# RWAlgorithms/ConjugateGradientOptim.jl

Hardware: AMD Instinct MI355X
Metric: CG iterations/sec at n=1e8 (outer iterations of minimizeobjective, PR-CG) (higher is better)
Workload: dtype f64

## Files before the change

conjugategradientoptim.jl_amd/_lib.py:

```python
from __future__ import annotations

import ctypes as C
import os
import subprocess

_PKG = os.path.dirname(os.path.abspath(__file__))
LIB_PATH = os.environ.get("CGO_LIB_PATH") or os.path.join(_PKG, "lib", "libcgo_hip.so")
CSRC = os.path.join(_PKG, "csrc")

dp = C.POINTER(C.c_double)
i64p = C.POINTER(C.c_int64)


class BetaConfig(C.Structure):
    _fields_ = [("kind", C.c_int32), ("lbfgs_m", C.c_int32), ("mu", C.c_double)]


class CGConfigC(C.Structure):
    _fields_ = [("eps", C.c_double), ("beta", BetaConfig), ("max_iters", C.c_int64),
                ("verbose", C.c_int32), ("trace_enabled", C.c_int32)]


class LSConfigC(C.Structure):
    _fields_ = [("kind", C.c_int32), ("cond_kind", C.c_int32), ("c1", C.c_double),
# ... 123 lines not shown
    "cgo_ctx_set_default_policy": (C.c_int, [_vp, C.POINTER(SolverPolicyC)]),
    "cgo_solver_get_policy": (C.c_int, [_vp, C.POINTER(SolverPolicyC)]),
    "cgo_solver_create_ex": (C.c_int, [_vp, _vp, C.POINTER(CGConfigC), C.POINTER(LSConfigC), C.POINTER(SolverPolicyC), _pp]),
    "cgo_solver_create_sys_ex": (C.c_int, [_vp, _vp, C.POINTER(CGConfigC), C.POINTER(LSSConfigC), C.POINTER(SolverPolicyC), _pp]),
    "cgo_ctx_destroy": (C.c_int, [_vp]),
    "cgo_comm_unique_id": (C.c_int, [_vp]),
    "cgo_ctx_set_comm_rccl": (C.c_int, [_vp, C.c_int32, C.c_int32, _vp]),
    "cgo_ctx_set_comm_callback": (C.c_int, [_vp, C.c_int32, C.c_int32, ALLGATHER_FN, _vp]),
    "cgo_ctx_set_comm_shm": (C.c_int, [_vp, C.c_int32, C.c_int32, C.c_char_p, C.c_int32]),
    "cgo_shm_unlink": (C.c_int, [C.c_char_p]),
    "cgo_ctx_comm_info": (C.c_int, [_vp, C.POINTER(C.c_int32), C.POINTER(C.c_int32), C.POINTER(C.c_int32), C.POINTER(C.c_int32)]),
    "cgo_ctx_exchange_stats": (C.c_int, [_vp, i64p, dp, dp, C.c_int32]),
    "cgo_ctx_comm_connect_devices": (C.c_int, [_vp, C.POINTER(C.c_int32)]),
    "cgo_rccl_available": (C.c_int, []),
    "cgo_objective_create": (C.c_int, [_vp, C.c_int32, C.c_int64, C.c_int64, C.c_int64, _pp]),
    "cgo_objective_create_from_source": (C.c_int, [_vp, C.c_char_p, C.c_int32, C.c_int64, C.c_int64, C.c_int64, _pp]),
    "cgo_objective_create_callback": (C.c_int, [_vp, FDF_FN, _vp, C.c_int64, C.c_int64, C.c_int64, _pp]),
    "cgo_objective_destroy": (C.c_int, [_vp]),
    "cgo_objective_create_from_source_ex": (C.c_int, [_vp, C.c_char_p, C.c_int32, C.c_int64, C.c_int64, C.c_int64, _pp]),
    "cgo_objective_num_params": (C.c_int, [_vp, C.POINTER(C.c_int32)]),
    "cgo_objective_set_param_host": (C.c_int, [_vp, C.c_int32, dp]),
    "cgo_objective_set_param_device": (C.c_int, [_vp, C.c_int32, _vp]),
    "cgo_objective_fill_param": (C.c_int, [_vp, C.c_int32, C.c_int32, C.c_uint64, C.c_double, C.c_double]),
    "cgo_objective_set_scalar": (C.c_int, [_vp, C.c_int32, C.c_double]),
    "cgo_objective_set_cost_class": (C.c_int, [_vp, C.c_int32]),
    "cgo_objective_eval_host": (C.c_int, [_vp, dp, dp, dp]),
    "cgo_solver_create": (C.c_int, [_vp, _vp, C.POINTER(CGConfigC), C.POINTER(LSConfigC), _pp]),
    "cgo_solver_destroy": (C.c_int, [_vp]),
    "cgo_solver_set_x0_host": (C.c_int, [_vp, dp]),
    "cgo_solver_set_x0_fill": (C.c_int, [_vp, C.c_int32, C.c_uint64, C.c_double, C.c_double]),
    "cgo_solver_set_x0_device": (C.c_int, [_vp, _vp]),
    "cgo_solver_results_device": (C.c_int, [_vp, _vp, _vp]),
    "cgo_solver_start": (C.c_int, [_vp]),
    "cgo_solver_iterate": (C.c_int, [_vp, C.c_int64, C.POINTER(C.c_int32)]),
    "cgo_solver_results": (C.c_int, [_vp, C.POINTER(ResultsC)]),
    "cgo_solver_trial_log": (C.c_int, [_vp, C.c_int64, dp, dp, dp, i64p]),
    "cgo_solver_profile_enable": (C.c_int, [_vp, C.c_int32]),
    "cgo_solver_profile_reset": (C.c_int, [_vp]),
    "cgo_solver_profile_get": (C.c_int, [_vp, C.c_int32, i64p, dp, dp]),
    "cgo_kernel_kind_name": (C.c_char_p, [C.c_int32]),
    "cgo_solver_kernel_family": (C.c_char_p, [_vp]),
    "cgo_solver_controller_launches": (C.c_int64, [_vp]),
    "cgo_solver_resident_stats": (C.c_int, [_vp, i64p, i64p, i64p]),
    "cgo_solver_lbfgs_stats": (C.c_int, [_vp, i64p, i64p, i64p]),
    "cgo_num_kernel_kinds": (C.c_int, []),
    "cgo_solver_set_lazy_direction": (C.c_int, [_vp, C.c_int32]),
    "cgo_solver_probe_set_beta_prev": (C.c_int, [_vp, C.c_double]),
    "cgo_solver_set_replay_depth": (C.c_int, [_vp, C.c_int32]),
    "cgo_solver_set_lean_sums": (C.c_int, [_vp, C.c_int32]),
    "cgo_solver_set_path_prediction": (C.c_int, [_vp, C.c_int32]),
    "cgo_solver_path_stats": (C.c_int, [_vp, i64p, i64p, i64p, i64p]),
    "cgo_solver_probe_set_path": (C.c_int, [_vp, C.c_int32]),
    "cgo_solver_debug_set_path_skew": (C.c_int, [_vp, C.c_double]),
    "cgo_solver_probe_set_replay": (C.c_int, [_vp, C.c_int32, dp, dp]),
    "cgo_solver_probe_set_deep_trial": (C.c_int, [_vp, C.c_int32]),
    "cgo_solver_replay_stats": (C.c_int, [_vp, i64p, i64p, i64p, i64p, i64p, i64p, C.POINTER(C.c_int32)]),
    "cgo_solver_kernel_symbol": (C.c_int, [_vp, C.c_int32, C.c_char_p, C.c_int32]),
    "cgo_evalwolfeconditions": (C.c_int, [C.POINTER(LSConfigC), C.c_double, C.c_double, C.c_double, C.c_double,
                                          C.c_double, C.c_double, C.POINTER(C.c_int32), C.POINTER(C.c_int32)]),
    "cgo_evalbacktrackcondition": (C.c_int, [C.POINTER(LSConfigC), C.c_double, C.c_double, C.c_double, C.c_double,
                                             C.POINTER(C.c_int32)]),
    "cgo_check_lss_config": (C.c_int, [C.POINTER(LSSConfigC)]),
    "cgo_lss_default_max_iters": (C.c_int64, [C.c_double]),
    "cgo_solver_create_sys": (C.c_int, [_vp, _vp, C.POINTER(CGConfigC), C.POINTER(LSSConfigC), _pp]),
    "cgo_solvesystem": (C.c_int, [_vp, _vp, dp, C.POINTER(CGConfigC), C.POINTER(LSSConfigC), C.POINTER(ResultsC)]),
    "cgo_minimize": (C.c_int, [_vp, _vp, dp, C.POINTER(CGConfigC), C.POINTER(LSConfigC), C.POINTER(ResultsC)]),
    "cgo_minimize_rerun": (C.c_int, [_vp, _vp, dp, C.POINTER(CGConfigC), C.POINTER(LSConfigC),
                                     C.POINTER(CGConfigC), C.POINTER(LSConfigC), C.c_int32,
                                     C.POINTER(ResultsC), C.POINTER(C.c_int32)]),
    "cgo_minimize_batch": (C.c_int, [_vp, C.c_int32, C.c_int64, C.c_int64, dp, dp, C.POINTER(CGConfigC), C.POINTER(LSConfigC),
                                     C.c_int64, C.POINTER(BatchResultsC)]),
    "cgo_batch_max_n": (C.c_int64, [_vp, C.c_int32]),
    "cgo_minimize_batch_obj": (C.c_int, [_vp, _vp, C.c_int64, dp, C.POINTER(dp), C.c_int32, C.POINTER(CGConfigC), C.POINTER(LSConfigC),
                                         C.c_int64, C.POINTER(BatchResultsC)]),
    "cgo_batch_max_n_obj": (C.c_int64, [_vp]),
    "cgo_batch_open": (C.c_int, [_vp, _vp, C.c_int64, C.POINTER(dp), C.c_int32, C.POINTER(_vp)]),
    "cgo_batch_solve": (C.c_int, [_vp, dp, dp, C.POINTER(C.c_uint8), C.POINTER(CGConfigC), C.POINTER(LSConfigC), C.c_int64,
                                  C.POINTER(BatchResultsC)]),
    "cgo_batch_close": (C.c_int, [_vp]),
    "cgo_batch_policy_init": (None, [C.POINTER(BatchPolicyC)]),
    "cgo_minimize_batch_ex": (C.c_int, [_vp, C.c_int32, C.c_int64, C.c_int64, dp, dp, C.POINTER(CGConfigC), C.POINTER(LSConfigC),
                                        C.c_int64, C.POINTER(BatchPolicyC), C.POINTER(BatchResultsC), C.POINTER(C.c_int32)]),
    "cgo_minimize_batch_obj_ex": (C.c_int, [_vp, _vp, C.c_int64, dp, C.POINTER(dp), C.c_int32, C.POINTER(CGConfigC), C.POINTER(LSConfigC),
                                            C.c_int64, C.POINTER(BatchPolicyC), C.POINTER(BatchResultsC), C.POINTER(C.c_int32)]),
    "cgo_batch_open_ex": (C.c_int, [_vp, _vp, C.c_int64, C.POINTER(dp), C.c_int32, C.POINTER(BatchPolicyC), C.POINTER(_vp)]),
    "cgo_batch_rows": (C.c_int, [_vp, C.POINTER(C.c_int32)]),
    "cgo_batch_max_n_ex": (C.c_int64, [_vp, C.c_int32, C.POINTER(BatchPolicyC)]),
    "cgo_batch_max_n_obj_ex": (C.c_int64, [_vp, C.POINTER(BatchPolicyC)]),
    "cgo_batch_rows_shape": (None, [C.POINTER(C.c_int32), C.POINTER(C.c_int32)]),
    "cgo_minimize_batch_lbfgs": (C.c_int, [_vp, C.c_int32, C.c_int64, C.c_int64, dp, dp, C.POINTER(CGConfigC), C.POINTER(LSConfigC),
                                           C.c_int64, C.POINTER(BatchResultsC)]),
    "cgo_batch_lbfgs_max_m": (C.c_int32, []),
    "cgo_batch_lbfgs_max_n": (C.c_int64, [_vp, C.c_int32]),
    "cgo_batch_lbfgs_shape": (None, [C.POINTER(C.c_int32), C.POINTER(C.c_int32)]),
    "cgo_minimize_batch_lbfgs_obj": (C.c_int, [_vp, _vp, C.c_int64, dp, C.POINTER(dp), C.c_int32, dp, C.POINTER(CGConfigC), C.POINTER(LSConfigC),
                                               C.c_int64, C.POINTER(BatchResultsC)]),
    "cgo_batch_lbfgs_max_n_obj": (C.c_int64, [_vp]),
    "cgo_batch_lbfgs_shape_obj": (None, [C.c_int32, C.POINTER(C.c_int32), C.POINTER(C.c_int32)]),
    "cgo_minimize_batch_lbfgs_ex": (C.c_int, [_vp, C.c_int32, C.c_int64, C.c_int64, dp, dp, C.POINTER(CGConfigC), C.POINTER(LSConfigC),
                                              C.c_int64, C.POINTER(BatchPolicyC), C.POINTER(BatchResultsC), C.POINTER(C.c_int32)]),
    "cgo_minimize_batch_lbfgs_obj_ex": (C.c_int, [_vp, _vp, C.c_int64, dp, C.POINTER(dp), C.c_int32, dp, C.POINTER(CGConfigC),
                                                  C.POINTER(LSConfigC), C.c_int64, C.POINTER(BatchPolicyC), C.POINTER(BatchResultsC),
                                                  C.POINTER(C.c_int32)]),
    "cgo_batch_lbfgs_max_n_ex": (C.c_int64, [_vp, C.c_int32, C.c_int32, C.POINTER(BatchPolicyC)]),
    "cgo_batch_lbfgs_max_n_obj_ex": (C.c_int64, [_vp, C.c_int32, C.POINTER(BatchPolicyC)]),
    "cgo_batch_lbfgs_lds_rows": (C.c_int32, [C.c_int32, C.c_int32]),
# ... 66 lines not shown
```

conjugategradientoptim.jl_amd/api.py:

```python
from __future__ import annotations

import ctypes as C
import math
import re
from dataclasses import dataclass, field
from typing import List, Optional, Sequence, Union

import numpy as np

from . import _lib
from ._lib import BetaConfig, CGConfigC, LSConfigC, LSSConfigC, ResultsC, check, dp, i64p



class TraceTrait:
    pass


class EnableTrace(TraceTrait):
    def __repr__(self):
        return "EnableTrace()"


class DisableTrace(TraceTrait):
# ... 606 lines not shown
        fin = C.c_int32(0)
        check(_lib.lib().cgo_solver_iterate(self._h, iters, C.byref(fin)))
        return bool(fin.value)

    def enable_trial_log(self):
        cnt = C.c_int64()
        check(_lib.lib().cgo_solver_trial_log(self._h, -1, None, None, None, C.byref(cnt)))

    def trial_log(self):
        cnt = C.c_int64()
        check(_lib.lib().cgo_solver_trial_log(self._h, 0, None, None, None, C.byref(cnt)))
        k = cnt.value
        a, p, d = np.zeros(max(k, 1)), np.zeros(max(k, 1)), np.zeros(max(k, 1))
        check(_lib.lib().cgo_solver_trial_log(self._h, k, a.ctypes.data_as(dp), p.ctypes.data_as(dp),
                                              d.ctypes.data_as(dp), C.byref(cnt)))
        return a[:k], p[:k], d[:k]

    def kernel_family(self) -> str:
        return _lib.lib().cgo_solver_kernel_family(self._h).decode()

    def kernel_symbol(self, kind_name: str) -> str:
        L = _lib.lib()
        buf = C.create_string_buffer(200)
        for k in range(L.cgo_num_kernel_kinds()):
            if L.cgo_kernel_kind_name(k).decode() == kind_name:
                check(L.cgo_solver_kernel_symbol(self._h, k, buf, 200))
                return buf.value.decode()
        return ""

    def set_lazy_direction(self, on: bool = True):
        check(_lib.lib().cgo_solver_set_lazy_direction(self._h, int(bool(on))))

    def set_replay_depth(self, d: int):
        check(_lib.lib().cgo_solver_set_replay_depth(self._h, int(d)))

    def replay_stats(self):
        v = [C.c_int64(0) for _ in range(6)]
        mx = C.c_int32(0)
        check(_lib.lib().cgo_solver_replay_stats(self._h, *[C.byref(q) for q in v], C.byref(mx)))
        return dict(zip(("n", "s", "t", "m", "t_deep", "m_deep"), (q.value for q in v)), max_list=mx.value)

    def set_lean_sums(self, on: bool):
        check(_lib.lib().cgo_solver_set_lean_sums(self._h, int(bool(on))))

    def set_path_prediction(self, on: bool):
        check(_lib.lib().cgo_solver_set_path_prediction(self._h, int(bool(on))))

    def path_stats(self):
        by = (C.c_int64 * 8)()
        p, t, m = C.c_int64(0), C.c_int64(0), C.c_int64(0)
        check(_lib.lib().cgo_solver_path_stats(self._h, by, C.byref(p), C.byref(t), C.byref(m)))
        return dict(by_nact={j: int(by[j]) for j in (1, 2, 3, 4, 5, 7)}, predicted=p.value, tree=t.value, misses=m.value)

    def debug_set_path_skew(self, factor: float):
        check(_lib.lib().cgo_solver_debug_set_path_skew(self._h, float(factor)))

    def probe_launch(self, kind_name: str, variant: int, a_acc: float, beta: float, a: Sequence[float], x, u=None, aux=None,
                     beta_prev: Optional[float] = None, replay: Optional[Sequence] = None, path_nact: Optional[int] = None,
                     deep_trial: bool = False):
        L = _lib.lib()
        kk = [L.cgo_kernel_kind_name(k).decode() for k in range(L.cgo_num_kernel_kinds())].index(kind_name)
        if beta_prev is not None:
            check(L.cgo_solver_probe_set_beta_prev(self._h, float(beta_prev)))
        if replay is not None:
            ra = np.ascontiguousarray([p[0] for p in replay], dtype=np.float64)
            rb = np.ascontiguousarray([p[1] for p in replay], dtype=np.float64)
            check(L.cgo_solver_probe_set_replay(self._h, len(replay), ra.ctypes.data_as(dp), rb.ctypes.data_as(dp)))
        if path_nact is not None:
            check(L.cgo_solver_probe_set_path(self._h, int(path_nact)))
        if deep_trial:
            check(L.cgo_solver_probe_set_deep_trial(self._h, 1))
        n = self.obj.n_local
        vec = lambda v: None if v is None else np.ascontiguousarray(v, dtype=np.float64)
        x, u, aux = vec(x), vec(u), vec(aux)
        for v in (x, u, aux):
            if v is not None and v.size != n:
                raise ValueError(f"probe vectors hold n_local = {n} elements")
        av = np.ascontiguousarray(a, dtype=np.float64) if len(a) else np.zeros(1)
        sums, ln = np.full(64, np.nan), C.c_int32(0)
        xo, uo, go = np.empty(n), np.empty(n), np.empty(n)
        sym = C.create_string_buffer(200)
        ptr = lambda v: None if v is None else v.ctypes.data_as(dp)
        check(L.cgo_solver_probe_launch(self._h, kk, int(variant), float(a_acc), float(beta), ptr(av), len(a), ptr(x), ptr(u),
                                        ptr(aux), ptr(sums), 64, C.byref(ln), ptr(xo), ptr(uo), ptr(go), sym, 200))
        return dict(sums=sums[:ln.value].copy(), x=xo, u=uo, g=go, symbol=sym.value.decode())

    LBFGS_PASSES = ("push", "push_gram", "direction_gram", "direction_trial", "push_lite", "loop")

    def probe_lbfgs(self, pass_name: str, x=None, u=None, g=None, gt=None, S=None, Y=None, **kw):
        n = self.obj.n_local
        P = self._cfg_c.beta.lbfgs_m + 1
        vec = lambda v: None if v is None else np.ascontiguousarray(v, dtype=np.float64)
        x, u, g, gt = vec(x), vec(u), vec(g), vec(gt)
        for v in (x, u, g, gt):
            if v is not None and v.size != n:
                raise ValueError(f"probe vectors hold n_local = {n} elements")
        S = None if S is None else np.ascontiguousarray(S, dtype=np.float64).reshape(P, n)
        Y = None if Y is None else np.ascontiguousarray(Y, dtype=np.float64).reshape(P, n)
        p = _lib.LbfgsProbeC()
        p.pass_ = self.LBFGS_PASSES.index(pass_name)
        dots = None
        for key, val in kw.items():
            if key in ("list", "spec_list"):
                getattr(p, key)[:len(val)] = [int(v) for v in val]
                setattr(p, "count" if key == "list" else "spec_count", len(val))
            elif key in ("cy", "cs", "alpha"):
                getattr(p, key)[:len(val)] = [float(v) for v in val]
            elif key == "stats":
                p.M, p.S = float(val[0]), float(val[1])
            elif key == "dots":
                dots = np.ascontiguousarray(val, dtype=np.float64).reshape(-1, 10)
                p.dots, p.dot_count = dots.ctypes.data_as(dp), dots.shape[0]
            else:
                if not hasattr(p, key):
                    raise TypeError(f"probe_lbfgs: no field {key}")
                setattr(p, key, val)
        outs = {k: np.full(n, np.nan) for k in ("x", "xo", "u", "g", "gt")}
        So, Yo = np.full((P, n), np.nan), np.full((P, n), np.nan)
        ptr = lambda v: None if v is None else v.ctypes.data_as(dp)
        check(_lib.lib().cgo_solver_probe_lbfgs(self._h, C.byref(p), ptr(x), ptr(u), ptr(g), ptr(gt), ptr(S), ptr(Y),
                                                *[ptr(outs[k]) for k in ("x", "xo", "u", "g", "gt")], ptr(So), ptr(Yo)))
        sym = p.symbol.decode()
        return dict(sums=np.array(p.sums[:p.sums_len]), S=So, Y=Yo, alpha=np.array(p.alpha[:]), symbols=sym.split(" + ") if sym else [],
                    new_in_list=p.new_in_list, spec_ok=bool(p.spec_ok),
                    gram=np.array(p.gram[:5 + 5 * p.spec_count]) if p.spec_ok else None, **outs)

    def probe_resident(self, script, x, u):
        n = self.obj.n_local
        x, u = np.ascontiguousarray(x, dtype=np.float64), np.ascontiguousarray(u, dtype=np.float64)
        if x.size != n or u.size != n:
            raise ValueError(f"probe vectors hold n_local = {n} elements")
        p = _lib.ResidentProbeC()
        if len(script) > 32:
            raise ValueError("probe_resident: at most 32 passes")
        p.npass = len(script)
        for q, item in enumerate(script):
            c = p.pass_[q]
            if item[0] == "trial":
# ... 1081 lines not shown
```

conjugategradientoptim.jl_amd/csrc/cgo_backend_cg.hip:

```cpp
#include "cgo_backend_internal.hpp"

#include "cgo_kernels.hip.hpp"
#include "cgo_kernels_cg.hip.hpp"
#include "cgo_kernels_cg_path.hip.hpp"
#include "cgo_kernels_chain.hip.hpp"
#include "cgo_kernels_lse.hip.hpp"
#include "cgo_kernels_resident.hip.hpp"

namespace cgo {

using namespace dev;

double bytes_r(int obj_kind, int mode, int64_t n, int n_params) {
    const int p = std::max(obj_kind == CGO_OBJ_QUAD_DIAG ? 1 : 0, n_params);
    return 8.0 * (double)n * (double)r_vectors(mode, p);
}

template <int N> using Pts = std::integral_constant<int, N>;
template <int MAXPTS, class F>
static inline void with_points(int npts, F f) {
    static_assert(MAXPTS == 1 || MAXPTS == 3 || MAXPTS == 5 || MAXPTS == 7, "a launch evaluates 1, 3, 5 or 7 trial points");
    if constexpr (MAXPTS >= 3) { if (npts == 3) return f(Pts<3>{}); }
    if constexpr (MAXPTS >= 5) { if (npts == 5) return f(Pts<5>{}); }
    if constexpr (MAXPTS >= 7) { if (npts != 1) return f(Pts<7>{}); }
    return f(Pts<1>{});
}

template <class Obj, bool BIG>
static int launch_cg(int mode, int npts, const RParams &P, int grid, hipStream_t st) {
#define ROW(MODE, MAXPTS) if (mode == (MODE) && P.tail.ctl) { with_points<MAXPTS>(npts, [&](auto n) { k_cg_armed<Obj, decltype(n)::value><<<grid, BLOCK, 0, st>>>(P); }); return 0; }
    CGO_CG_ARMED_ROWS(ROW)
#undef ROW
    switch (mode) {
#define ROW(MODE, MAXPTS) case (MODE): with_points<MAXPTS>(npts, [&](auto n) { k_cg<Obj, (MODE), decltype(n)::value, BIG><<<grid, BLOCK, 0, st>>>(P); }); return 0;
    CGO_CG_ROWS(ROW)
#undef ROW
    default: break;
    }
    if constexpr (BIG) {
        switch (mode) {
#define ROW(MODE, MAXPTS) case (MODE): with_points<MAXPTS>(npts, [&](auto n) { k_cg<Obj, (MODE), decltype(n)::value, true><<<grid, BLOCK, 0, st>>>(P); }); return 0;
        CGO_CG_LAG_ROWS(ROW)
        CGO_CG_REPLAY_ROWS(ROW)
        CGO_CG_LEAN_ROWS(ROW)
#undef ROW
        default: break;
        }
    }
    return -1;
}

template <class Obj>
static int launch_cg_path(int mode, int nact, const RParams &P, const RDeep &Q, int grid, hipStream_t st) {
#define ROW(MODE, NACT) if (mode == (MODE) && nact == (NACT)) { k_cg_path<Obj, (MODE), (NACT), true><<<grid, BLOCK, 0, st>>>(P, Q); return 0; }
    CGO_CG_PATH_ROWS(ROW)
#undef ROW
    return -1;
}
template <class Obj>
static int launch_cg_deep_t(int npts, const RParams &P, const RDeep &Q, int grid, hipStream_t st) {
#define ROW(NPTS) if (npts == (NPTS)) { k_cg_trial_deep<Obj, (NPTS), true><<<grid, BLOCK, 0, st>>>(P, Q); return 0; }
    CGO_CG_DEEP_T_ROWS(ROW)
#undef ROW
    return -1;
}
static inline bool path_row(int mode, int nact) {
#define ROW(MODE, NACT) if (mode == (MODE) && nact == (NACT)) return true;
    CGO_CG_PATH_ROWS(ROW)
#undef ROW
    return false;
}
static inline bool path_objective(int kind) {
#define ROW(KIND, T) if (kind == KIND) return true;
    CGO_OBJ_CURV_ROWS(ROW)
#undef ROW
    return false;
}
bool HipBackend::deep_trial(int mode) const {
    return mode == (R_REPLAY | R_TRIAL) && !path_nact_ && path_objective(obj_->kind) && (rep_n_ > RMAX || deep_t_);
}
bool HipBackend::path_rows() const {
    if (!path_on_ || !path_objective(obj_->kind) || replay_depth_ < 2 || !lazy_eligible()) return false;
    const int mode_n = r_mode_of(KK_ACCEPT_TRIAL_NOSTORE), mode_s = R_REPLAY | R_ADT;
    return path_row(mode_n | lean_for(mode_n), MAXP) && path_row(mode_s | lean_for(mode_s), MAXP);
}

static inline bool lean_row(int mode) {
#define ROW(MODE, MAXPTS) if (mode == (MODE)) return true;
    CGO_CG_LEAN_ROWS(ROW)
#undef ROW
    return false;
}
int HipBackend::lean_for(int mode) const { return (lean_bits_ && lean_row(mode | lean_bits_)) ? lean_bits_ : 0; }

void unpack_r(const double *s, int k, Scal *out, bool dir, int npts) {
    if (npts == 0) npts = npts_for(k);
    for (int j = 0; j < k; ++j) {
        const double *q = s + RS_PER_POINT * j;
        out[j].f = q[RS_F]; out[j].gtu = q[RS_GTU]; out[j].gtgt = q[RS_GTGT]; out[j].gtg = q[RS_GTG];
        out[j].yy = q[RS_YY]; out[j].uy = q[RS_UY]; out[j].ygt = q[RS_YGT];
    }
    if (dir) { out[0].gu = s[RS_PER_POINT * npts]; out[0].uu = s[RS_PER_POINT * npts + 1]; }
}

static inline int chain_npts(int mode, int npts) { return ((mode & R_TRIAL) && npts >= 3) ? 3 : 1; }

RPlan HipBackend::r_plan(int mode, int npts) const {
    const double bytes = bytes_r(obj_->kind, mode, obj_->n_local, obj_->nparams());
    const bool big = r_big_only(mode) || bytes > big_bytes(r_read_only(mode));
    return {big, big ? GRID_BIG : grid_cg(obj_->n_local, chain() ? 1 : npts), chain() ? chain_npts(mode, npts) : npts, bytes};
}
bool HipBackend::adt_is_big() const { return bytes_r(obj_->kind, R_ADT, obj_->n_local, obj_->nparams()) > big_bytes(false); }

int HipBackend::launch_r(int kk, int mode, double a_acc, double beta, const double *a, int k, bool fetch,
                         double *sums) {
    if (int rc = pipe_drain()) return rc;
    pipe_streak_ = 0;
    if (u_lag_ && !(mode & R_ULAG)) {
        if (r_reads_u(mode)) { if (int rc = materialize_u()) return rc; }
        else if (mode & (R_INIT | R_RESET)) u_lag_ = false;
    }
    if (rep_n_ > 0 && !(mode & R_REPLAY)) { if (int rc = materialize_lag()) return rc; }
    if (rep_n_ > RMAX && (mode & R_REPLAY) && r_base(mode) != R_REPLAY && !path_nact_ && !deep_trial(mode)) { if (int rc = materialize_lag()) return rc; }
    RPlan plan;
    const int npts = path_nact_ ? MAXP : npts_for(k);
    if (int rc = launch_r_kernel(kk, mode, a_acc, beta, a, k, npts, nullptr, &plan)) return rc;
    const int grid = plan.grid;
    total_launches_++;
    const bool has_sums = r_has_sums(mode);
    const bool fused = has_sums && tail_fused(grid);
    if (has_sums && chain()) {
        const bool three = plan.npts == 3;
        const int W = three ? NRC3 : NRC, edge = three ? RC3_EDGE : RC_EDGE, nsums = three ? NR : NR1;
        if (!fused) { if (int rc = finalize_rows(ctx_, grid, W, true)) return rc; }
        const int Wd = ctx_->world(), me = ctx_->rank();
        std::vector<double> raw((size_t)W * Wd);
        double all[NRC3];
        if (int rc = fetch_sums(ctx_, all, MERGE_SUM, W, raw.data())) return rc;
        if (sums) std::memcpy(sums, all, sizeof(double) * nsums);
        if (me > 0) {
            const double *e = raw.data() + (size_t)(me - 1) * W + edge + 4;
            halo_xl_[0] = e[0]; halo_xl_[1] = e[1]; halo_ul_[0] = e[2]; halo_ul_[1] = e[3];
        }
        if (me < Wd - 1) {
            const double *e = raw.data() + (size_t)(me + 1) * W + edge;
            halo_xr_[0] = e[0]; halo_xr_[1] = e[1]; halo_ur_[0] = e[2]; halo_ur_[1] = e[3];
        }
        if (probe_) { std::memcpy(probe_row_, all, sizeof(double) * W); probe_len_ = W; }
    } else if (has_sums) {
        if (!fused) { if (int rc = finalize_rows(ctx_, grid, rows_for(npts), true)) return rc; }
        if (fetch) {
            if (int rc = fetch_sums(ctx_, sums, MERGE_SUM, rows_for(npts))) return rc;
        }
        if (probe_ && fetch) { std::memcpy(probe_row_, sums, sizeof(double) * rows_for(npts)); probe_len_ = rows_for(npts); }
    }
    if (prof_on_) prof_commit(kk, plan.bytes);
    return CGO_OK;
}

bool HipBackend::lazy_eligible() const {
    if (!lazy_on_ || !rmode_ || chain() || sys_on_ || probe_ || pingpong_ == 1) return false;
    bool aot = false;
#define ROW(KIND, T) aot = aot || obj_->kind == KIND;
    CGO_OBJ_ROWS(ROW)
#undef ROW
    if (!aot) return false;
    if (const char *e = getenv("CGO_PINGPONG")) { if (e[0] == '1') return false; }
    if (ctl_depth() > 0) return false;
    return adt_is_big() && r_plan(R_TRIAL, 1).big;
}

int HipBackend::materialize_u() {
    if (!u_lag_) return CGO_OK;
    const int64_t asked = total_launches_;
    const int nact = path_nact_;
    path_nact_ = 0;
    const int rc = launch_rk(KK_MATERIALIZE_U, 0.0, 0.0, nullptr, 0, false, nullptr);
    path_nact_ = nact;
    total_launches_ = asked;
    if (rc) return rc;
    u_lag_ = false;
    return CGO_OK;
}

int HipBackend::materialize_lag() {
    if (int rc = materialize_u()) return rc;
    const int64_t asked = total_launches_;
    const int nact = path_nact_;
    path_nact_ = 0;
    int rc = CGO_OK;
    while (rep_n_ > 0 && rc == CGO_OK) {
        const int all = rep_n_, take = std::min(all, (int)RMAX);
        rep_n_ = take;
        rc = launch_rk(KK_MATERIALIZE_XU, 0.0, 0.0, nullptr, 0, false, nullptr);
        rep_n_ = all;
        if (rc) break;
        rstats_.m++;
        if (all > RMAX) rstats_.m_deep++;
        for (int j = take; j < all; ++j) { rep_a_[j - take] = rep_a_[j]; rep_b_[j - take] = rep_b_[j]; }
        rep_n_ = all - take;
    }
    path_nact_ = nact;
    total_launches_ = asked;
    return rc;
}

int HipBackend::set_replay_depth_now(int d) {
    if (d < 1 || d > RCAP + 1) { set_error("replay depth: 1 … 16"); return CGO_EINVAL; }
    if (d != replay_depth_) { if (int rc = materialize_lag()) return rc; }
    replay_depth_ = d;
    return CGO_OK;
}

void HipBackend::set_probe_replay(int nrep, const double *a, const double *beta) {
    probe_rep_n_ = std::max(0, std::min(nrep, (int)RCAP));
    for (int j = 0; j < probe_rep_n_; ++j) { probe_rep_a_[j] = a[j]; probe_rep_b_[j] = beta[j]; }
}

int HipBackend::accept_dir_trial_r(double a_acc, double beta, const double *a, int k, double *s) {
    if (!lazy_eligible()) return launch_rk(KK_ACCEPT_DIR_TRIAL, a_acc, beta, a, k, true, s);
    if (replay_depth_ >= 2) {
        if (int rc = materialize_u()) return rc;
        if (rep_n_ < replay_depth_ - 1 && rep_n_ < (path_nact_ ? RCAP : RMAX)) {
            const int mode_n = r_mode_of(KK_ACCEPT_TRIAL_NOSTORE);
            if (int rc = launch_r(KK_ACCEPT_TRIAL_NOSTORE, mode_n | lean_for(mode_n), a_acc, beta, a, k, true, s)) return rc;
            if (path_nact_) { path_last_n_ = path_nact_; path_count_[path_nact_]++; }
            rep_a_[rep_n_] = a_acc; rep_b_[rep_n_] = beta; rep_n_++;
            rstats_.n++;
            return CGO_OK;
        }
        const int mode_s = R_REPLAY | R_ADT;
        if (int rc = launch_r(KK_ACCEPT_DIR_TRIAL, mode_s | lean_for(mode_s), a_acc, beta, a, k, true, s)) return rc;
        if (path_nact_) { path_last_s_ = path_nact_; path_count_[path_nact_]++; }
        rep_n_ = 0;
        rstats_.s++;
        return CGO_OK;
    }
    if (!u_lag_) {
        if (int rc = launch_rk(KK_ACCEPT_TRIAL_LAZY, a_acc, beta, a, k, true, s)) return rc;
        u_lag_ = true; beta_lag_ = beta;
        return CGO_OK;
    }
    if (int rc = launch_r(KK_ACCEPT_DIR_TRIAL, R_ULAG | R_ADT, a_acc, beta, a, k, true, s)) return rc;
    u_lag_ = false;
    return CGO_OK;
}
int HipBackend::trial_r(const double *a, int k, double *s) {
    if (rep_n_ > 0 && lazy_eligible()) {
        rstats_.t++;
        if (rep_n_ > RMAX) rstats_.t_deep++;
        return launch_r(KK_TRIAL, R_REPLAY | R_TRIAL, 0, 0, a, k, true, s);
    }
    if (u_lag_ && lazy_eligible()) return launch_r(KK_TRIAL, R_ULAG | R_TRIAL, 0, 0, a, k, true, s);
    return launch_rk(KK_TRIAL, 0, 0, a, k, true, s);
}

bool HipBackend::pipe_fused(int grid) const {
    return tail_fused(grid) && obj_->kind != CGO_OBJ_USER && !chain() && ctl_fused_;
}
bool HipBackend::tail_fused(int grid) const {
    static const int cap = [] { const char *e = getenv("CGO_FUSED_TAIL_MAX_GRID"); int v = e ? atoi(e) : 0; return v > 0 ? v : 1024; }();
    return ctx_->fused_tail && grid <= cap && grid <= TAIL_GROUP * TAIL_GROUP;
}
Tail HipBackend::make_tail(bool on) {
    Tail t{};
    if (!on) return t;
    ctx_->seq++;
    t.partials2 = ctx_->partials2_f; t.tickets = ctx_->tickets; t.out = ctx_->out_dev;
    t.strict = ctx_->tail_strict ? 1 : 0;
    ctx_->pub_target(&t.host_out, &t.host_seq);
    ctx_->pub_checked = (t.host_out != nullptr) && !ctx_->tail_strict;
    t.seq = ctx_->seq;
    return t;
}

int HipBackend::launch_r_kernel(int kk, int mode, double a_acc, double beta, const double *a, int k, int npts,
                                const CtlArgs *ctl, RPlan *plan_out) {
    HIPCHK(hipSetDevice(ctx_->device));
    if (obj_->unset_slot() >= 0) return param_unset_error(obj_->unset_slot());
    const int64_t n = obj_->n_local;
    if (mode & (R_GRAD | R_GRADT)) { if (int rc = ensure_ga()) return rc; }
    const bool has_sums = r_has_sums(mode);
    const RPlan plan = *plan_out = r_plan(mode, npts);
    const bool big = plan.big; const int grid = plan.grid;
    const bool deep_t = deep_trial(mode);
    last_mode_ = mode; last_npts_ = plan.npts; last_big_ = big; last_nact_ = deep_t ? -1 : path_nact_;
    if (path_nact_ && (chain() || !big || ctl || !path_row(mode, path_nact_) || !path_objective(obj_->kind))) { set_error("internal: not a path row"); return CGO_EINVAL; }
    if (chain()) {
        if (int rc = prof_begin(kk)) return rc;
        if (int rc = launch_chain_kernel(mode, a_acc, beta, a, k, plan.npts, big, grid, make_tail(has_sums && !ctl && tail_fused(grid)))) return rc;
        return prof_end();
    }
    RParams P;
    P.x = xc_; P.u = uc_; P.gout = ga_.p; obj_->param_args(P); P.n = n;
    P.xo = xc_; P.uo = uc_;
    P.a_acc = a_acc; P.beta = beta; P.s0 = obj_->s0; P.partials = ctx_->partials;
    P.beta_prev = beta_lag_;
    const int nrep = (mode & R_REPLAY) ? rep_n_ : 0;
    if (nrep > RCAP || (nrep > RMAX && !path_nact_ && !deep_t)) { set_error("internal: more replayed steps than the launch takes"); return CGO_ESTATE; }
    P.nrep = std::min(nrep, (int)RMAX);
    for (int j = 0; j < RMAX; ++j) { P.ra[j] = j < P.nrep ? rep_a_[j] : 0.0; P.rb[j] = j < P.nrep ? rep_b_[j] : 0.0; }
    RDeep Q;
    Q.nrep2 = nrep - P.nrep;
    for (int j = 0; j < RDEEP; ++j) { Q.ra2[j] = j < Q.nrep2 ? rep_a_[RMAX + j] : 0.0; Q.rb2[j] = j < Q.nrep2 ? rep_b_[RMAX + j] : 0.0; }
    rstats_.max_list = std::max(rstats_.max_list, nrep);
    P.ctl = ctl;
    P.x2 = xn_;
    for (int j = 0; j < MAXP; ++j) P.a[j] = (a && j < k) ? a[j] : ((a && k > 0) ? a[k - 1] : 0.0);
    P.tail = make_tail(has_sums && !ctl && tail_fused(grid));
    if (ctl && pipe_fused(grid)) {
        P.tail.partials2 = ctx_->partials2_f; P.tail.tickets = ctx_->tickets; P.tail.out = ctx_->out_dev;
        P.tail.strict = ctx_->tail_strict ? 1 : 0;
        P.tail.ctl = ctl_dev_; P.tail.ctl_rec = ctl_rec_; P.tail.ctl_seq = ctl_seq_;
        if (!ctx_->single()) {
            P.tail.xw = ctx_->world(); P.tail.xme = ctx_->rank(); P.tail.xseq0 = epoch_ << 40;
            for (int r = 0; r < P.tail.xw && r < 8; ++r) P.tail.xmail[r] = ctx_->comm->dev_mailbox(r);
        }
    }
    if (P.tail.tickets) P.partials = ctx_->partials_f;
    const bool wr_x = r_writes_x(mode), wr_u = r_writes_u(mode);
    const bool pp = big && !ctl && (wr_x || wr_u) && !(mode & R_PROJ) && pingpong_ready();
    if (pp && wr_x) P.xo = xalt_;
    if (pp && wr_u) P.uo = ualt_;
    if (mode == R_PROJ && !xn_) { set_error("internal: no second iterate buffer"); return CGO_ESTATE; }
    hipStream_t st = ctx_->stream;
    if (int rc = prof_begin(kk)) return rc;
    int r = -2;
    if (path_nact_) {
        switch (obj_->kind) {
#define ROW(KIND, T) case KIND: r = launch_cg_path<T>(mode, path_nact_, P, Q, grid, st); break;
        CGO_OBJ_CURV_ROWS(ROW)
#undef ROW
        default: break;
        }
    } else if (deep_t) {
        if (!big) { set_error("internal: not a deep trial row"); return CGO_EINVAL; }
        switch (obj_->kind) {
#define ROW(KIND, T) case KIND: r = launch_cg_deep_t<T>(plan.npts, P, Q, grid, st); break;
        CGO_OBJ_CURV_ROWS(ROW)
#undef ROW
        default: break;
        }
    } else switch (obj_->kind) {
#define ROW(KIND, T) case KIND: r = big ? launch_cg<T, true>(mode, npts, P, grid, st) : launch_cg<T, false>(mode, npts, P, grid, st); break;
    CGO_OBJ_ROWS(ROW)
#undef ROW
    case CGO_OBJ_USER:
        if (!obj_->rtc) { set_error("user objective has no compiled module"); return CGO_EINVAL; }
        if (r_big_only(mode)) break;
        if (int rc = launch_module(obj_->rtc->cg(mode, npts, big), &P, grid, st)) return rc;
        r = 0;
        break;
    default: break;
    }
    if (r) { set_error("internal: CG kernel mode not instantiated"); return CGO_EINVAL; }
    HIPCHK(hipGetLastError());
    if (pp && wr_x) std::swap(xc_, xalt_);
    if (pp && wr_u) std::swap(uc_, ualt_);
    return prof_end();
}

template <bool BIG>
static int launch_chain(int mode, int npts, const ChainParams &P, int grid, hipStream_t st) {
    switch (mode) {
#define ROW(MODE, MAXPTS) case (MODE): with_points<MAXPTS>(npts, [&](auto n) { k_chain<(MODE), decltype(n)::value, BIG><<<grid, BLOCK, 0, st>>>(P); }); return 0;
    CGO_CHAIN_ROWS(ROW)
#undef ROW
    default: return -1;
    }
}

int HipBackend::launch_chain_kernel(int mode, double a_acc, double beta, const double *a, int k, int npts, bool big, int grid, const Tail &tail) {
    ChainParams P;
    P.tail = tail;
    for (int j = 0; j < 3; ++j) P.a[j] = (a && j < k) ? a[j] : ((a && k > 0) ? a[k - 1] : 0.0);
    P.x = xc_; P.u = uc_; P.xo = xc_; P.uo = uc_; P.gout = ga_.p;
    P.odd = (int)(obj_->n_local & 1);
    P.n = obj_->n_local + P.odd; P.a_acc = a_acc; P.beta = beta; P.partials = tail.tickets ? ctx_->partials_f : ctx_->partials;
    for (int j = 0; j < 2; ++j) { P.hxl[j] = halo_xl_[j]; P.hul[j] = halo_ul_[j]; P.hxr[j] = halo_xr_[j]; P.hur[j] = halo_ur_[j]; }
    P.has_left = obj_->offset > 0 ? 1 : 0;
    P.has_right = obj_->offset + obj_->n_local < obj_->n_global ? 1 : 0;
    const bool wr_x = r_writes_x(mode), wr_u = r_writes_u(mode);
    if (wr_x) P.xo = xalt_;
    if (wr_u) P.uo = ualt_;
    const int r = big ? launch_chain<true>(mode, npts, P, grid, ctx_->stream) : launch_chain<false>(mode, npts, P, grid, ctx_->stream);
    if (r) { set_error("internal: chain kernel mode not instantiated"); return CGO_EINVAL; }
    HIPCHK(hipGetLastError());
    if (wr_x) std::swap(xc_, xalt_);
    if (wr_u) std::swap(uc_, ualt_);
    return CGO_OK;
}

std::string HipBackend::r_symbol(int mode, int npts, bool big, int nact) const {
    char buf[160];
    if (chain()) snprintf(buf, sizeof buf, "k_chain<%d, %d, %s>", mode, npts, big ? "true" : "false");
    else if (nact < 0) snprintf(buf, sizeof buf, "k_cg_trial_deep<%s, %d, true>", obj_tname(), npts);
    else if (nact) snprintf(buf, sizeof buf, "k_cg_path<%s, %d, %d, true>", obj_tname(), mode, nact);
    else snprintf(buf, sizeof buf, "k_cg<%s, %d, %d, %s>", obj_tname(), mode, npts, big ? "true" : "false");
    return buf;
}

std::string HipBackend::kernel_symbol(int kk) const {
    if (!rmode_) {
        if (obj_->two_phase() || kk == KK_LBFGS_PUSH || kk == KK_LBFGS_LOOP || kk == KK_LBFGS_FINAL) return lbfgs_symbol(kk);
        const int mode = fused_mode(kk);
        return mode < 0 ? "" : fused_symbol(obj_tname(), mode, is_big(obj_->kind, mode, obj_->n_local, obj_->nparams(), pol_.hbm_stream_bytes));
    }
    const RKind *rk = r_kind(kk);
    if (!rk) return "";
    int mode = rk->mode;
    const bool lazy = lazy_eligible();
    switch (kk) {
    case KK_ACCEPT_DIR_TRIAL: if (lazy) mode |= replay_depth_ >= 2 ? R_REPLAY : R_ULAG; break;
    case KK_ACCEPT_TRIAL_LAZY: case KK_MATERIALIZE_U: if (!lazy || replay_depth_ >= 2) return ""; break;
    case KK_ACCEPT_TRIAL_NOSTORE: case KK_MATERIALIZE_XU: if (!lazy || replay_depth_ < 2) return ""; break;
    default: break;
    }
    if (kk == KK_TRIAL && lazy && rep_n_ > RMAX) mode |= R_REPLAY;
    const RPlan plan = r_plan(mode, rk->pts == PTS_ONE ? 1 : npts_for(rk->pts == PTS_MAX ? max_points() : std::min(max_points(), 3)));
    if ((mode & R_REPLAY) && (mode & R_ACCEPT)) mode |= lean_for(mode);
    if ((mode & R_REPLAY) && (mode & R_ACCEPT) && path_rows()) {
        const int last = kk == KK_ACCEPT_TRIAL_NOSTORE ? path_last_n_ : path_last_s_;
        return r_symbol(mode, plan.npts, plan.big, last ? last : MAXP);
    }
    if (kk == KK_TRIAL && deep_trial(mode)) return r_symbol(mode, plan.npts, plan.big, -1);
    return r_symbol(mode, plan.npts, plan.big);
}


__global__ void k_ctl_init(CtlDev *d, const CtlConfig cfg, const CtlState st, unsigned long long round) {
    d->cfg = cfg;
    d->st = st;
    d->round = round;
    d->args = ctl_args_of(st);
}



template <int N, int THREADS>
__global__ __launch_bounds__(THREADS) void k_finalize_ctl(const double *partials, int rows, double *out, CtlDev *d,
                                                          CtlRecord *rec_ring, unsigned long long *seq_ring) {
    constexpr int G = BLOCK / N;
    constexpr int WD = sizeof(CtlDev) / 8, WR = sizeof(CtlRecord) / 8;
    __shared__ double sm[G][N];
    __shared__ double fin[CTL_NSUMS];
    __shared__ CtlDev sd;
    __shared__ CtlRecord sr;
    const int tid = threadIdx.x;
    if (tid < WD) ((unsigned long long *)&sd)[tid] = ((const unsigned long long *)d)[tid];
    if (tid < CTL_NSUMS) fin[tid] = 0.0;
    __syncthreads();
    const bool go = sd.st.go != 0;
    const unsigned long long round = sd.round, seq = round + 1;
    CtlRecord *rec_host = rec_ring + (round % PIPE_RING);
    unsigned long long *seq_host = seq_ring + (round % PIPE_RING);
    if (go) {
        if (tid < G * N) {
            double t = 0.0;
            const long long total = (long long)rows * N;
            for (long long i = tid; i < total; i += G * N) t += partials[i];
            sm[tid / N][tid % N] = t;
        }
        __syncthreads();
        if (tid < N) {
            double v = 0.0;
#pragma unroll
            for (int g = 0; g < G; ++g) v += sm[g][tid];
            out[tid] = v;
            fin[tid] = v;
        }
        __syncthreads();
    }
    if (tid == 0) {
        if (go) {
            ctl_step(sd.cfg, sd.st, fin, sr);
            sd.args = ctl_args_of(sd.st);
// ... 242 lines not shown
        if (b == &x2_ || b == &u2_) { if (pingpong_ != 1) continue; }
        if (int rc = b->alloc(np)) return rc;
        HIPCHK(hipMemsetAsync(b->p, 0, na * sizeof(double), ctx_->stream));
        HIPCHK(hipMemsetD32Async((hipDeviceptr_t)(b->p + na), (int)PROBE_NAN32, (np - na) * 2, ctx_->stream));
    }
    for (int j = 0; j < obj_->nparams(); ++j) {
        if (!obj_->p_set[j]) continue;
        DevBuf p;
        if (int rc = p.alloc(np)) return rc;
        HIPCHK(hipMemcpyAsync(p.p, obj_->p[j].p, n * sizeof(double), hipMemcpyDeviceToDevice, ctx_->stream));
        HIPCHK(hipMemsetD32Async((hipDeviceptr_t)(p.p + n), (int)PROBE_NAN32, (np - n) * 2, ctx_->stream));
        HIPCHK(hipStreamSynchronize(ctx_->stream));
        std::swap(p.p, obj_->p[j].p); std::swap(p.n, obj_->p[j].n);
    }
    HIPCHK(hipStreamSynchronize(ctx_->stream));
    xc_ = x_.p; uc_ = u_.p; xalt_ = x2_.p; ualt_ = u2_.p;
    g_ = ga_.p; gt_ = gb_.p; xn_ = gb_.p;
    lse_have_ = false;
    probe_ = true;
    return CGO_OK;
}

int HipBackend::probe_slack_intact() {
    const size_t n = (size_t)obj_->n_local, na = n + (chain() ? (n & 1) : 0);
    struct { const DevBuf *b; const char *name; size_t used; int slot; } v[] = {
        {&x_, "x", na, -1}, {&u_, "u", na, -1}, {&x2_, "x (ping-pong)", na, -1}, {&u2_, "u (ping-pong)", na, -1},
        {&ga_, "gradient A", na, -1}, {&gb_, "gradient B / x2", na, -1}, {&obj_->p[0], "parameter vector", n, 0},
        {&obj_->p[1], "parameter vector 1", n, 1}, {&obj_->p[2], "parameter vector 2", n, 2}, {&obj_->p[3], "parameter vector 3", n, 3}};
    std::vector<unsigned> h;
    for (const auto &e : v) {
        if (!e.b->p || (e.slot >= 0 && !(e.slot < obj_->nparams() && obj_->p_set[e.slot]))) continue;
        const size_t words = (e.b->n - e.used) * 2;
        h.assign(words, 0u);
        HIPCHK(hipMemcpyAsync(h.data(), e.b->p + e.used, words * 4, hipMemcpyDeviceToHost, ctx_->stream));
        HIPCHK(hipStreamSynchronize(ctx_->stream));
        for (size_t w = 0; w < words; ++w)
            if (h[w] != PROBE_NAN32) {
                set_error(std::string("probe: the launch wrote past the ") + std::to_string(e.used) + " elements of " + e.name +
                          " (element " + std::to_string(e.used + w / 2) + ")");
                return CGO_ESTATE;
            }
    }
    return CGO_OK;
}

int HipBackend::probe_launch(int kk, int variant, double a_acc, double beta, const double *a, int k, const double *x,
                             const double *u, const double *aux, double *sums, int sums_cap, int *sums_len, double *x_out,
                             double *u_out, double *g_out, std::string &symbol) {
    *sums_len = 0;
    const int want_nact = probe_nact_;
    probe_nact_ = 0;
    const bool want_deep = probe_deep_t_;
    probe_deep_t_ = false;
    const bool lse = obj_->two_phase();
    if (k < 0 || k > MAXP || (k > 0 && !a)) { set_error("probe: 0 ≤ k ≤ 7 trial steps"); return CGO_EINVAL; }
    if (!rmode_ && !lse) return probe_launch_stored(kk, variant, a_acc, beta, a, k, x, u, aux, sums, sums_cap, sums_len, x_out, u_out, g_out, symbol);
    int mode = -1;
    if (lse) {
        if (kk == KK_LSE_STATS && (variant == 0 || variant == LM_NOU || variant == (LM_ACCEPT | LM_DIR))) mode = variant;
        if (kk == KK_LSE_GRAD && variant >= 0 && variant <= 2) mode = variant;
        if (kk == KK_LSE_STATS && mode != LM_NOU && k < 1) mode = -1;
        if (kk == KK_LSE_GRAD && mode != 2 && k < 1) mode = -1;
    } else {
        static constexpr RKind norm_passes{KK_SCALED_NORM, R_GRAD, PTS_ONE, {R_GRADT, 0}};
        const RKind *rk = kk == KK_SCALED_NORM ? &norm_passes : r_kind(kk);
        if (rk && (variant & R_LEAN)) {
            const int full = kk == KK_ACCEPT_DIR_TRIAL ? (R_REPLAY | R_ADT) : (kk == KK_ACCEPT_TRIAL_NOSTORE ? rk->mode : -1);
            if (lean_row(variant) && (variant & ~R_LEAN) == full) mode = variant;
        } else if (rk) {
            const int m = variant ? variant : rk->mode;
            if (r_kind_allows(*rk, m) || (kk == KK_INIT && chain() && m == R_EDGES)) mode = m;
        }
        if (mode > 0 && (mode & (R_TRIAL | R_GRADT | R_PROJ)) && k < 1) mode = -1;
        if (mode > 0 && chain() && k > 3) mode = -1;
        if (mode > 0 && r_big_only(mode) && (chain() || obj_->kind == CGO_OBJ_USER)) mode = -1;
    }
    if (mode < 0) { set_error("probe: kernel kind / variant / trial steps not a launch this solver's engine issues"); return CGO_EINVAL; }
    if (int rc = probe_prepare()) return rc;
    HIPCHK(hipSetDevice(ctx_->device));
    hipStream_t st = ctx_->stream;
    const size_t n = (size_t)obj_->n_local, nb = n * sizeof(double);
    double *ub = lse ? u_.p : uc_;
    double *gb = lse ? gt_ : ga_.p;
    double *auxb = lse ? g_ : xn_;
    auto put = [&](double *dst, const double *src) -> int {
        if (src) HIPCHK(hipMemcpyAsync(dst, src, nb, hipMemcpyHostToDevice, st));
        else HIPCHK(hipMemsetD32Async((hipDeviceptr_t)dst, (int)PROBE_NAN32, n * 2, st));
        return CGO_OK;
    };
    if (int rc = put(xc_, x)) return rc;
    if (int rc = put(ub, u)) return rc;
    if (int rc = put(auxb, aux)) return rc;
    if (gb != auxb) { if (int rc = put(gb, nullptr)) return rc; }
    if (!lse && pingpong_ == 1) {
        if (int rc = put(xalt_, nullptr)) return rc;
        if (int rc = put(ualt_, nullptr)) return rc;
    }
    HIPCHK(hipStreamSynchronize(st));
    probe_len_ = 0;
    last_mode_ = -1;
    beta_lag_ = probe_beta_prev_;
    rep_n_ = (!lse && (mode & R_REPLAY)) ? probe_rep_n_ : 0;
    for (int j = 0; j < rep_n_; ++j) { rep_a_[j] = probe_rep_a_[j]; rep_b_[j] = probe_rep_b_[j]; }
    int rc = CGO_OK;
    char buf[160];
    if (lse) {
        Scal o;
        if (kk == KK_LSE_STATS) {
            lse_have_ = false;
            rc = lse_stats(mode, a_acc, beta, k ? a[0] : 0.0, o, mode == (LM_ACCEPT | LM_DIR));
            snprintf(buf, sizeof buf, "k_lse_stats<%d, %s, %s>", last_mode_, last_big_ ? "true" : "false", last_npts_ ? "true" : "false");
        } else {
            const bool nb0 = need_beta_;
            need_beta_ = mode == 1;
            rc = lse_grad(mode == 2, k ? a[0] : 0.0, o);
            need_beta_ = nb0;
            snprintf(buf, sizeof buf, "k_lse_grad<%s, %s, %s>", last_mode_ == 1 ? "true" : "false", last_mode_ == 2 ? "true" : "false",
                     last_big_ ? "true" : "false");
        }
        if (rc) return rc;
        symbol = buf;
    } else {
        double s[64];
        if (want_deep && (mode != (R_REPLAY | R_TRIAL) || want_nact || !path_objective(obj_->kind))) { rep_n_ = 0; set_error("probe: not a deep trial launch of this solver"); return CGO_EINVAL; }
        if (rep_n_ > RMAX && !want_nact && !(mode == (R_REPLAY | R_TRIAL) && path_objective(obj_->kind))) {
            rep_n_ = 0; set_error("probe: more than 7 replayed steps: path rows and the deep trial launch only"); return CGO_EINVAL;
        }
        deep_t_ = want_deep;
        if (want_nact) {
            if (!path_row(mode, want_nact) || !path_objective(obj_->kind) || k > want_nact) { rep_n_ = 0; set_error("probe: not a path row of this solver, or more steps than it evaluates"); return CGO_EINVAL; }
            path_nact_ = want_nact;
        }
        rc = launch_r(kk, mode, a_acc, beta, a, k, true, s);
        path_nact_ = 0;
        deep_t_ = false;
        rep_n_ = 0;
        if (rc) return rc;
        symbol = r_symbol(last_mode_, last_npts_, last_big_, last_nact_);
    }
    HIPCHK(hipStreamSynchronize(st));
    if (x_out) HIPCHK(hipMemcpyAsync(x_out, xc_, nb, hipMemcpyDeviceToHost, st));
    if (u_out) HIPCHK(hipMemcpyAsync(u_out, lse ? u_.p : uc_, nb, hipMemcpyDeviceToHost, st));
    if (g_out) HIPCHK(hipMemcpyAsync(g_out, mode == R_PROJ && !lse ? xn_ : gb, nb, hipMemcpyDeviceToHost, st));
    HIPCHK(hipStreamSynchronize(st));
    if (int rc2 = probe_slack_intact()) return rc2;
    *sums_len = probe_len_;
    if (probe_len_ > sums_cap) { set_error("probe: sums_cap smaller than the launch's row"); return CGO_EINVAL; }
    if (probe_len_) std::memcpy(sums, probe_row_, sizeof(double) * probe_len_);
    return CGO_OK;
}

void HipBackend::probe_append(const double *row, int len) {
    if (probe_len_ + len > (int)(sizeof probe_row_ / sizeof probe_row_[0])) return;
    std::memcpy(probe_row_ + probe_len_, row, sizeof(double) * len);
    probe_len_ += len;
}

int HipBackend::probe_launch_stored(int kk, int variant, double a_acc, double beta, const double *a, int k, const double *x,
                                    const double *u, const double *aux, double *sums, int sums_cap, int *sums_len, double *x_out,
                                    double *u_out, double *g_out, std::string &symbol) {
    if (ctx_->world() != 1) { set_error("probe: a single-rank solver"); return CGO_EINVAL; }
    const bool host = obj_->host_closure();
    int mode = -1;
    if (const MKind *mk = m_kind(kk)) {
        const int m = variant ? variant : (host ? mk->host : fused_mode(kk));
        if (host ? m == mk->host : (m == mk->mode || (mk->alt && m == mk->alt))) mode = m;
    } else if (kk == KK_SCALED_NORM) {
        mode = (variant == 0 || variant == 1 || variant == 3 || variant == 4) ? variant : -1;
    }
    const bool trial_step = kk == KK_TRIAL || kk == KK_ACCEPT_DIR_TRIAL;
    if (mode >= 0 && trial_step && k != 1) mode = -1;
    if (mode < 0) { set_error("probe: kernel kind / variant / trial steps not a launch this solver's engine issues"); return CGO_EINVAL; }
    if (int rc = probe_prepare()) return rc;
    HIPCHK(hipSetDevice(ctx_->device));
    hipStream_t st = ctx_->stream;
    const size_t n = (size_t)obj_->n_local, nb = n * sizeof(double);
    auto put = [&](double *dst, const double *src) -> int {
        if (src) HIPCHK(hipMemcpyAsync(dst, src, nb, hipMemcpyHostToDevice, st));
        else HIPCHK(hipMemsetD32Async((hipDeviceptr_t)dst, (int)PROBE_NAN32, n * 2, st));
        return CGO_OK;
    };
    const bool norm = kk == KK_SCALED_NORM;
    const bool gt_in_x = norm && (mode == 1 || mode == 4);
    const bool swaps = kk == KK_ACCEPT_DIR_TRIAL || kk == KK_ACCEPT_DIR || kk == KK_ACCEPT_ONLY;
    if (int rc = put(xc_, gt_in_x ? nullptr : x)) return rc;
    if (int rc = put(u_.p, u)) return rc;
    if (int rc = put(swaps ? gt_ : g_, aux)) return rc;
    if (int rc = put(swaps ? g_ : gt_, gt_in_x ? x : nullptr)) return rc;
    HIPCHK(hipStreamSynchronize(st));
    probe_len_ = 0;
    probe_syms_.clear();
// ... 459 lines not shown
```

conjugategradientoptim.jl_amd/csrc/cgo_capi.hip:

```cpp
#include <sys/mman.h>

#include <cmath>
#include <cstdio>
#include <cstdlib>
#include <cstring>
#include <new>
#include <vector>

#include "cgo_capi_internal.hpp"
#include "cgo_build_id.inc"

using namespace cgo;

extern "C" {

int cgo_version(void) { return CGO_VERSION; }
const char *cgo_build_id(void) { return CGO_BUILD_ID; }
const char *cgo_last_error(void) { return get_error(); }
const char *cgo_status_name(int32_t s) { return status_name(s); }
const char *cgo_kernel_kind_name(int32_t k) {
    if (k == 100) return "dir";
    if (k == 101) return "beta_partials";
    return kernel_kind_name(k);
}
// ... 424 lines not shown
    int rc = s->be->alloc();
    if (rc) { delete s; obj_unref(obj); return rc; }
    const bool cheap = obj->o.kind == CGO_OBJ_QUAD_DIAG || obj->o.kind == CGO_OBJ_BOOTH ||
                       (obj->o.kind == CGO_OBJ_USER && obj->o.user_cheap);
    s->be->set_multi_min_n(0);
    s->be->set_multi5_min_n(cheap ? 0 : INT64_MAX);
    s->be->set_multi7_min_n(cheap ? 0 : INT64_MAX);
    s->be->set_three_point_band(0, 0);
    const char *mm = getenv("CGO_MULTI_MIN_N"), *m5 = getenv("CGO_MULTI5_MIN_N"), *m7 = getenv("CGO_MULTI7_MIN_N");
    if (chain) m5 = m7 = nullptr;
    if (mm || m5 || m7) s->be->set_three_point_band(0, 0);
    if (mm) s->be->set_multi_min_n(atoll(mm));
    if (m5) s->be->set_multi5_min_n(atoll(m5));
    if (m7) s->be->set_multi7_min_n(atoll(m7));
    if (pol.points) {
        const int pts = chain ? std::min(pol.points, 3) : pol.points;
        s->be->set_three_point_band(0, 0);
        s->be->set_multi_min_n(pts >= 3 ? 0 : INT64_MAX);
        s->be->set_multi5_min_n(pts >= 5 ? 0 : INT64_MAX);
        s->be->set_multi7_min_n(pts >= 7 ? 0 : INT64_MAX);
    }
    s->be->set_ctl_depth((ls && !cheap && !chain && s->be->policy_points() <= 3 && (ctx->c.world() == 1 || ctx->c.dev_exchange()) && obj->o.n_local <= 100000) ? 4 : 0);
    if (pol.controller_depth >= 0) s->be->set_ctl_depth(chain ? 0 : pol.controller_depth);
    s->be->set_ctl_graph(pol.controller_graph != 0);
    {
        bool lazy = obj->o.kind == CGO_OBJ_QUAD_DIAG;
        const int forced = env_tri("CGO_LAZY_DIR");
        if (forced >= 0) lazy = forced != 0;
        s->be->set_lazy_direction(lazy);
    }
    {
        int depth = 1;
        if (obj->o.kind == CGO_OBJ_QUAD_DIAG && 8.0 * (double)obj->o.n_local * 5.0 > 1.4e9) depth = kReplayDepth;
        if (const char *e = getenv("CGO_REPLAY_DEPTH")) { const int v = atoi(e); if (v >= 1 && v <= 16) depth = v; }
        s->be->set_replay_depth(depth);
    }
    {
        bool lean = kLeanSums && obj->o.kind == CGO_OBJ_QUAD_DIAG && 8.0 * (double)obj->o.n_local * 5.0 > 1.4e9;
        const int forced = env_tri("CGO_LEAN_SUMS");
        if (forced >= 0) lean = forced != 0;
        s->be->set_beta_unread(beta_unread_sums(cfg->beta.kind));
        s->be->set_lean_sums(lean);
    }
    {
        bool predict = kPathPredict && kLeanSums && obj->o.kind == CGO_OBJ_QUAD_DIAG && 8.0 * (double)obj->o.n_local * 5.0 > 1.4e9;
        const int forced = env_tri("CGO_PATH_PREDICT");
        if (forced >= 0) predict = forced != 0;
        s->be->set_path_prediction(predict && path_applies(obj, cfg, ls));
    }
    if (int prc = s->be->place()) { delete s; obj_unref(obj); return prc; }
    if (pol.resident >= 0) s->be->set_resident(pol.resident != 0);
    if (int prc = s->be->prepare_controller()) { delete s; obj_unref(obj); return prc; }
    s->sv = ls ? new Solver(s->be, *cfg, *ls) : new Solver(s->be, *cfg, *lss);
    *out = s;
    return CGO_OK;
}

int cgo_solver_create(cgo_ctx *ctx, cgo_objective *obj, const cgo_cg_config *cfg,
                      const cgo_ls_config *ls, cgo_solver **out) {
    API_GUARD_BEGIN
    REQUIRE(ctx && obj && cfg && ls && out, "null argument");
    return make_solver(ctx, obj, cfg, ls, nullptr, nullptr, out);
    API_GUARD_END
}

int cgo_solver_create_ex(cgo_ctx *ctx, cgo_objective *obj, const cgo_cg_config *cfg, const cgo_ls_config *ls,
                         const cgo_solver_policy *policy, cgo_solver **out) {
    API_GUARD_BEGIN
    REQUIRE(ctx && obj && cfg && ls && out, "null argument");
    return make_solver(ctx, obj, cfg, ls, nullptr, policy, out);
    API_GUARD_END
}

int cgo_solver_create_sys(cgo_ctx *ctx, cgo_objective *obj, const cgo_cg_config *cfg,
                          const cgo_lss_config *ls, cgo_solver **out) {
    API_GUARD_BEGIN
    REQUIRE(ctx && obj && cfg && ls && out, "null argument");
    return make_solver(ctx, obj, cfg, nullptr, ls, nullptr, out);
    API_GUARD_END
}

int cgo_solver_create_sys_ex(cgo_ctx *ctx, cgo_objective *obj, const cgo_cg_config *cfg, const cgo_lss_config *ls,
                             const cgo_solver_policy *policy, cgo_solver **out) {
    API_GUARD_BEGIN
    REQUIRE(ctx && obj && cfg && ls && out, "null argument");
    return make_solver(ctx, obj, cfg, nullptr, ls, policy, out);
    API_GUARD_END
}

int cgo_check_lss_config(const cgo_lss_config *ls) {
    API_GUARD_BEGIN
    std::string why;
    if (int rc = check_lss_config(ls, why)) { set_error(why); return rc; }
    return CGO_OK;
    API_GUARD_END
}

int64_t cgo_lss_default_max_iters(double rho) { return lss_default_max_iters(rho); }

int cgo_solver_destroy(cgo_solver *s) {
    API_GUARD_BEGIN
    if (s) {
        (void)hipSetDevice(s->ctx->c.device);
        cgo_objective *o = s->obj;
        delete s;
        obj_unref(o);
// ... 154 lines not shown
}

int cgo_solver_set_replay_depth(cgo_solver *s, int32_t d) {
    API_GUARD_BEGIN
    REQUIRE(s, "null argument");
    REQUIRE(d >= 1 && d <= 16, "replay depth: 1 … 16");
    return s->be->set_replay_depth_now(d);
    API_GUARD_END
}

int cgo_solver_replay_stats(cgo_solver *s, int64_t *n, int64_t *s_launches, int64_t *t, int64_t *m, int64_t *t_deep, int64_t *m_deep,
                            int32_t *max_list) {
    API_GUARD_BEGIN
    REQUIRE(s, "null argument");
    const auto &r = s->be->replay_stats();
    if (n) *n = r.n;
    if (s_launches) *s_launches = r.s;
    if (t) *t = r.t;
    if (m) *m = r.m;
    if (t_deep) *t_deep = r.t_deep;
    if (m_deep) *m_deep = r.m_deep;
    if (max_list) *max_list = r.max_list;
    return CGO_OK;
    API_GUARD_END
}

int cgo_solver_set_lean_sums(cgo_solver *s, int32_t on) {
    API_GUARD_BEGIN
    REQUIRE(s, "null argument");
    s->be->set_lean_sums(on != 0);
    return CGO_OK;
    API_GUARD_END
}

int cgo_solver_set_path_prediction(cgo_solver *s, int32_t on) {
    API_GUARD_BEGIN
    REQUIRE(s, "null argument");
    const bool applies = s->sv && !s->sv->is_sys() && path_applies(s->obj, &s->sv->config(), &s->sv->linesearch());
    s->be->set_path_prediction(on != 0 && applies);
    return CGO_OK;
    API_GUARD_END
}

int cgo_solver_path_stats(cgo_solver *s, int64_t *by_nact, int64_t *predicted, int64_t *tree, int64_t *misses) {
    API_GUARD_BEGIN
    REQUIRE(s && s->sv, "null argument");
    if (by_nact) for (int j = 0; j < 8; ++j) by_nact[j] = s->be->path_launches(j);
    int64_t p = 0, t = 0, m = 0;
    s->sv->path_stats(p, t, m);
    if (predicted) *predicted = p;
    if (tree) *tree = t;
    if (misses) *misses = m;
    return CGO_OK;
    API_GUARD_END
}

int cgo_solver_debug_set_path_skew(cgo_solver *s, double factor) {
    API_GUARD_BEGIN
    REQUIRE(s && s->sv, "null argument");
    REQUIRE(factor > 0.0 && std::isfinite(factor), "path skew: a positive factor");
    s->sv->set_path_skew(factor);
    return CGO_OK;
    API_GUARD_END
}

int cgo_solver_probe_set_path(cgo_solver *s, int32_t nact) {
    API_GUARD_BEGIN
    REQUIRE(s, "null argument");
    REQUIRE(nact >= 0 && nact <= 7, "probe path row: 0 … 7 active points");
    s->be->set_probe_path(nact);
    return CGO_OK;
    API_GUARD_END
}

int cgo_solver_probe_set_replay(cgo_solver *s, int32_t nrep, const double *a, const double *beta) {
    API_GUARD_BEGIN
    REQUIRE(s, "null argument");
    REQUIRE(nrep >= 0 && nrep <= 15 && (nrep == 0 || (a && beta)), "probe replay list: 0 … 15 (a*, β) pairs (more than 7: path rows and the deep trial launch)");
    s->be->set_probe_replay(nrep, a, beta);
    return CGO_OK;
    API_GUARD_END
}

int cgo_solver_probe_set_deep_trial(cgo_solver *s, int32_t on) {
    API_GUARD_BEGIN
    REQUIRE(s, "null argument");
    s->be->set_probe_deep_trial(on != 0);
    return CGO_OK;
    API_GUARD_END
}

int cgo_solver_probe_set_beta_prev(cgo_solver *s, double beta_prev) {
    API_GUARD_BEGIN
    REQUIRE(s, "null argument");
    s->be->set_probe_beta_prev(beta_prev);
    return CGO_OK;
    API_GUARD_END
}

int cgo_solver_profile_enable(cgo_solver *s, int32_t on) {
    API_GUARD_BEGIN
    REQUIRE(s, "null argument");
    s->be->profile_enable(on != 0);
    return CGO_OK;
    API_GUARD_END
}
// ... 247 lines not shown
```

conjugategradientoptim.jl_amd/csrc/cgo_engine.cpp:

```cpp
#include "cgo_engine.hpp"

#include <algorithm>
#include <cstring>

namespace cgo {

static const char *kStatusNames[CGO_NUM_STATUS] = {
    "incomplete",
    "success",
    "increasing_objective",
    "non_finite_objective_or_gradient_proposed",
    "max_iters_reached",
    "non_descent_search_direction",
    "linesearch_a_max_overflow",
    "linesearch_max_iters_reached",
    "zoom_max_iters_reached",
    "accepted_non_finite_iterate",
    "cannot_find_initial_feasible_step",
    "max_step_length_reached",
    "cannot_find_feasible_step",
    "step_bracket_precision_issue",
    "bisection_lower_bound_larger_than_proposed_step",
    "feasible",
    "infeasible",
    "non_finite_step_proposed",
    "proposed_step_same_as_current_step",
    "linesearch_failed",
};

const char *status_name(int s) {
    return (s >= 0 && s < CGO_NUM_STATUS) ? kStatusNames[s] : "unknown";
}

static const char *kKernelNames[KK_COUNT] = {
    "init", "trial", "accept_dir_trial", "accept_dir", "accept_only",
    "reset_dir", "upg_norm", "lbfgs_push", "lbfgs_loop", "lbfgs_final", "lse_stats", "lse_grad",
    "scaled_norm", "dir_trial", "sys_project", "resident", "accept_trial_nostore", "materialize_xu",
    "accept_trial_lazy", "materialize_u",
};

const char *kernel_kind_name(int k) { return (k >= 0 && k < KK_COUNT) ? kKernelNames[k] : "unknown"; }

int check_cg_config(const cgo_cg_config *c, std::string &why) {
    if (!c) { why = "null CGConfig"; return CGO_EINVAL; }
    if (!(0.0 < c->eps && c->eps < 1.0)) {
        why = "AssertionError: zero(T) < ϵ < one(T)  (types.jl:187)";
        return CGO_EINVAL;
    }
    if (c->beta.kind < 0 || c->beta.kind > CGO_BETA_BROYDEN_FAMILY) { why = "unknown β_config kind"; return CGO_EINVAL; }
    if (c->beta.kind == CGO_BETA_BROYDEN_FAMILY && !(0.0 <= c->beta.mu)) {
        why = "AssertionError: zero(T) <= θ  (qn_flavours.jl:57)"; return CGO_EINVAL;
    }
    if (c->beta.kind == CGO_BETA_LBFGS && (c->beta.lbfgs_m < 1 || c->beta.lbfgs_m > 64)) {
        why = "LBFGS history length m must be in 1..64"; return CGO_EINVAL;
    }
    if (c->max_iters < 0) { why = "max_iters must be ≥ 0"; return CGO_EINVAL; }
    return CGO_OK;
}

int check_ls_config(const cgo_ls_config *l, std::string &why) {
    if (!l) { why = "null LineSearchConfig"; return CGO_EINVAL; }
    if (l->kind == CGO_LS_STRONG_WOLFE_BISECTION) {
        if (!(0.0 < l->c1 && l->c1 < l->c2 && l->c2 < 1.0)) {
            why = "AssertionError: zero(T) < c1 < c2 < one(T)  (nocedal.jl:22)"; return CGO_EINVAL;
        }
        if (!(l->max_iters >= 0)) { why = "AssertionError: max_iters >= 0  (nocedal.jl:24)"; return CGO_EINVAL; }
        if (!(l->zoom_max_iters >= 0)) { why = "AssertionError: zoom_max_iters >= 0  (nocedal.jl:25)"; return CGO_EINVAL; }
        if (!(l->a_max_growth_factor > 1.0)) { why = "AssertionError: a_max_growth_factor > 1  (nocedal.jl:26)"; return CGO_EINVAL; }
        return CGO_OK;
    }
    if (l->kind == CGO_LS_WOLFE_BISECTION) {
        if (l->cond_kind == CGO_COND_WOLFE) {
            if (!(0.0 < l->c1 && l->c1 < l->c2 && l->c2 < 1.0)) {
                why = "AssertionError: zero(T) < c1 < c2 < one(T)  (wolfe.jl:278)"; return CGO_EINVAL;
            }
        } else if (l->cond_kind == CGO_COND_YUAN_WEI_LU) {
            if (!(0.0 < l->delta1 && l->delta1 < l->c1 && l->c1 < l->c2 && l->c2 < 1.0)) {
                why = "AssertionError: zero(T) < δ1 < c1 < c2 < one(T)  (wolfe.jl:233)"; return CGO_EINVAL;
            }
        } else { why = "unknown Wolfe condition kind"; return CGO_EINVAL; }
        return CGO_OK;
    }
    if (l->kind == CGO_LS_BACKTRACKING) {
        if (l->cond_kind != CGO_COND_ARMIJO) { why = "Backtracking needs the Armijo condition"; return CGO_EINVAL; }
        if (!(0.0 < l->c1 && l->c1 < 1.0)) {
            why = "AssertionError: zero(T) < c1 < one(T)  (geometric.jl:169)"; return CGO_EINVAL;
        }
        if (!(l->discount_factor > 0.0 && std::isfinite(l->discount_factor))) { why = "discount_factor must be positive"; return CGO_EINVAL; }
        return CGO_OK;
    }
    why = "unknown LineSearchConfig kind";
// ... 15 lines not shown
double beta_from_scalars(const cgo_beta_config &b, const Scal &t, double gu_old, double gg_old,
                         double uu_old) {
    const TrialSums ts = trial_sums(t);
    return beta_from_sums(b.kind, b.mu, ts, gu_old, gg_old, uu_old, beta_norms_fast(ts, uu_old));
}

int Solver::robust_norm(double sumsq, int which, double &out) {
    if (sumsq >= 1e-280 && sumsq <= 1e300) { out = std::sqrt(sumsq); return CGO_OK; }
    double m = 0, ss = 0;
    bool has_nan = false;
    if (int rc = be_->scaled_norm_parts(which, last_eval_a_, m, ss, has_nan)) return rc;
    if (has_nan) out = NAN;
    else if (m == 0.0 || std::isinf(m)) out = m;
    else out = m * std::sqrt(ss);
    return CGO_OK;
}

Solver::Solver(VecBackend *be, const cgo_cg_config &cfg, const cgo_ls_config &ls)
    : be_(be), cfg_(cfg), ls_(ls) {}

Solver::Solver(VecBackend *be, const cgo_cg_config &cfg, const cgo_lss_config &lss)
    : be_(be), cfg_(cfg), ls_{}, sys_(true), lss_(lss) {}

int Solver::start() {
    Scal s;
    if (cfg_.beta.kind == CGO_BETA_LBFGS) {
        const int P = cfg_.beta.lbfgs_m + 1;
        int rc = be_->lbfgs_alloc(P);
        if (rc) return rc;
        qn_rho_.assign(P, 0.0);
        qn_list_.clear(); qn_free_ = 0; qn_gamma_ = 1.0;
        qn_gram_ = be_->lbfgs_gram_max_pairs() >= cfg_.beta.lbfgs_m;
        qn_SY_.assign((size_t)P * P, 0.0); qn_YY_.assign((size_t)P * P, 0.0);
        qn_sg_.assign(P, 0.0); qn_yg_.assign(P, 0.0);
    }
    if (sys_ && (cfg_.beta.kind >= CGO_BETA_LBFGS || !be_->sys_supported())) return CGO_EINVAL;
    int rc = be_->init_eval(s);
    if (rc) return rc;
    if (sys_ && (rc = be_->sys_begin())) return rc;
    total_evals_ = 1;
    f_x_ = s.f;
    f_x0_ = f_x_;
    gg_ = s.gtgt;
    if ((rc = robust_norm(gg_, 0, norm_df_x_))) return rc;
    dphi0_ = -gg_;
    uu_ = gg_;
    dir_is_neg_grad_ = true;
    a_initial_ = NAN;
    it_ = 0; iters_ran_ = 0; status_ = CGO_INCOMPLETE;
    ncache_ = 0; finished_ = false; started_ = true;
    qn_trial_done_ = false;
    res_fail_streak_ = 0; res_backoff_ = 0;
    tr_f_.clear(); tr_g_.clear(); tr_a_.clear(); tr_e_.clear(); log_.clear();
    path_part_ = false; path_reset_ = false;
    path_pred_ = 0; path_tree_ = 0; path_miss_ = 0;
    return CGO_OK;
}

void Solver::finish(int64_t iters, int status) {
    iters_ran_ = iters;
    status_ = status;
    finished_ = true;
    ncache_ = 0;
    path_part_ = false;
    qn_trial_done_ = false;
    be_->discard_pending();
    if (cfg_.trace_enabled) {
        tr_f_.resize((size_t)iters); tr_g_.resize((size_t)iters);
        tr_a_.resize((size_t)iters); tr_e_.resize((size_t)iters);
    }
}

double Solver::first_step(double a_initial) const { return ls_first_step(ls_, a_initial); }

void Solver::first_hints(double a0, double (&h)[2]) const { ls_first_hints(ls_, a0, h[0], h[1]); }

int Solver::eval(double a, double &phi, double &dphi, double h1, double h2, double h3, double h4) {
    const double hs[4] = {h1, h2, h3, h4};
    return evaln(a, phi, dphi, hs, 4);
}

int Solver::evaln(double a, double &phi, double &dphi, const double *hs, int nh) {
    int hit = -1;
    for (int j = 0; j < ncache_; ++j)
        if (std::memcmp(&a, &cache_[j].a, sizeof(double)) == 0) { hit = j; break; }
    int in_tree = -1;
    if (hit < 0 && path_part_)
        for (int j = 0; j < ntree_; ++j)
            if (std::memcmp(&a, &tree_[j], sizeof(double)) == 0) { in_tree = j; break; }
    if (hit >= 0) {
        last_ = cache_[hit].s;
    } else if (in_tree >= 0) {
        Scal out[7];
        if (int rc = be_->trial(tree_, ntree_, out)) return rc;
        ncache_ = ntree_;
        for (int j = 0; j < ntree_; ++j) cache_[j] = {tree_[j], out[j]};
        last_ = out[in_tree];
        path_part_ = false;
        path_miss_++;
    } else {
        double pts[7] = {a, 0, 0, 0, 0, 0, 0};
        int k = 1;
        const int mp = sys_ ? be_->max_points() : std::min(be_->max_points(), 3);
        for (int q = 0; q < nh && k < mp; ++q) {
            const double h = hs[q];
            bool ok = std::isfinite(h) && h > 0.0;
            for (int j = 0; ok && j < k; ++j) ok = (h != pts[j]);
            if (ok) pts[k++] = h;
        }
        Scal out[7];
        if (int rc = be_->trial(pts, k, out)) return rc;
        ncache_ = k;
        for (int j = 0; j < k; ++j) cache_[j] = {pts[j], out[j]};
        last_ = out[0];
    }
    last_eval_a_ = a;
    total_evals_++;
    phi = last_.f;
    dphi = last_.gtu;
    if (log_on_) log_.push_back({a, phi, dphi});
    return CGO_OK;
}

int Solver::ls_strong_wolfe(double a_initial, LSOut &o) {
    auto ev = [this](double a, double &phi, double &dphi, double h1, double h2, double h3, double h4) {
        return eval(a, phi, dphi, h1, h2, h3, h4);
    };
    return ls_strong_wolfe_t(ls_, f_x_, dphi0_, a_initial, ev, o);
}

int Solver::find_feasible(double &a, double lb, int64_t &evals, double &phi, double &dphi,
                          int &flag, double h1, double h2, double h3, double h4) {
    auto ev = [this](double a_, double &phi_, double &dphi_, double g1, double g2, double g3, double g4) {
        return eval(a_, phi_, dphi_, g1, g2, g3, g4);
    };
    return ls_find_feasible_t(ls_, a, lb, evals, phi, dphi, flag, ev, h1, h2, h3, h4);
}

int Solver::ls_wolfe_bisection(double a_initial, LSOut &o) {
    auto ev = [this](double a, double &phi, double &dphi, double h1, double h2, double h3, double h4) {
        return eval(a, phi, dphi, h1, h2, h3, h4);
    };
    struct Bk {
        Solver *s;
        int is_neg_grad(bool &yes) {
            yes = s->dir_is_neg_grad_;
            if (!yes) {
                double ss = 0;
                if (int rc = s->be_->upg_sumsq(ss)) return rc;
                yes = (std::sqrt(ss) == 0.0);
            }
            return 0;
        }
        int reset_dir(double &uu) {
            Scal sc;
            if (int rc = s->be_->reset_dir(sc)) return rc;
            s->ncache_ = 0;
            uu = sc.uu;
            s->dphi0_ = sc.gu;
            s->dir_is_neg_grad_ = true;
            s->path_part_ = false; s->path_reset_ = true;
            return 0;
// ... 225 lines not shown
                        qn_SY_[(size_t)slot * P + pj] = G.yjsn[j];
                        qn_YY_[(size_t)pj * P + slot] = qn_YY_[(size_t)slot * P + pj] = G.yjyn[j];
                    }
                }
                if (sy > 0.0) {
                    qn_SY_[(size_t)slot * P + slot] = sy; qn_YY_[(size_t)slot * P + slot] = yy;
                    qn_sg_[slot] = G.sgn; qn_yg_[slot] = G.ygn;
                }
            } else {
                if ((rc = be_->lbfgs_push(a_xp, o.a, slot, sy, yy))) return rc;
            }
            if (sy > 0.0) {
                qn_rho_[slot] = 1.0 / sy;
                qn_gamma_ = sy / yy;
                qn_commit(slot);
            }
            if (!will_stop) {
                const double a0 = first_step(a_initial_);
                Scal t0;
                if ((rc = qn_direction(s, ls_.kind == CGO_LS_BACKTRACKING ? NAN : a0, &t0))) return rc;
                dphi0_ = s.gu; uu_ = s.uu;
                dir_is_neg_grad_ = qn_list_.empty();
                if (qn_trial_done_) { ncache_ = 1; cache_[0] = {a0, t0}; }
            }
        } else if (will_stop) {
            if ((rc = be_->accept_only(a_xp))) return rc;
        } else if (!std::isfinite(first_step(a_initial_))) {
            if ((rc = be_->accept_dir(a_xp, beta, s))) return rc;
            dphi0_ = s.gu; uu_ = s.uu;
            dir_is_neg_grad_ = (beta == 0.0);
        } else {
            double pts[7] = {0, 0, 0, 0, 0, 0, 0};
            int k;
            if (be_->max_points() >= 5) {
                k = ls_trial_points_n(ls_, first_step(a_initial_), be_->max_points() >= 7 ? 7 : 5, pts);
            } else {
                double p3[3];
                k = ls_trial_points(ls_, first_step(a_initial_), be_->max_points() >= 3, p3);
                for (int j = 0; j < 3; ++j) pts[j] = p3[j];
            }
            Scal out[7];
            if (be_->ctl_depth() > 0 && !be_->two_phase() && ls_.kind != CGO_LS_BACKTRACKING) {
                CtlConfig cc;
                cc.ls = ls_; cc.eps = cfg_.eps; cc.mu = cfg_.beta.mu;
                cc.beta_kind = cfg_.beta.kind; cc.maxp = be_->max_points();
                cc.max_iters = cfg_.max_iters;
                CtlState cs;
                cs.f_x = f_x_; cs.gg = gg_; cs.a_acc = a_xp; cs.beta = beta;
                for (int j = 0; j < CTL_MAXP; ++j) cs.a[j] = pts[j < k ? j : k - 1];
                cs.npts = k; cs.go = 1; cs.it = it_;
                rc = be_->accept_dir_trial_ctl(cc, cs, budget, out);
            } else if (be_->path_rows() && k >= 6) {
                k = path_points(a_xp, beta, pts, k);
                rc = be_->accept_dir_trial_path(a_xp, beta, pts, k, out);
            } else {
                rc = be_->accept_dir_trial(a_xp, beta, pts, k, out);
            }
            if (rc) return rc;
            dphi0_ = out[0].gu; uu_ = out[0].uu;
            dir_is_neg_grad_ = (beta == 0.0);
            ncache_ = k;
            for (int j = 0; j < k; ++j) cache_[j] = {pts[j], out[j]};
        }
    }
    finished = finished_;
    return CGO_OK;
}

int Solver::path_points(double a_xp, double beta, double (&pts)[7], int k) {
    ntree_ = k;
    for (int j = 0; j < 7; ++j) tree_[j] = pts[j];
    path_part_ = false;
    int kp = 0;
    double pp[7] = {0, 0, 0, 0, 0, 0, 0};
    if (cfg_.beta.kind == CGO_BETA_POLAK_RIBIERE && !path_reset_ && std::isfinite(last_.curv) && std::isfinite(beta) &&
        std::isfinite(a_xp) && a_xp > 0.0 && std::isfinite(dphi0_) && std::isfinite(last_.gtu) && std::isfinite(last_.gtgt) &&
        std::isfinite(last_.ygt) && std::isfinite(f_x_)) {
        const double c_k = (last_.gtu - dphi0_) / a_xp;
        const double d1 = -last_.gtgt + beta * last_.gtu;
        const double c1 = (last_.curv - 2.0 * beta * last_.ygt / a_xp + beta * beta * c_k) * path_skew_;
        kp = ls_predicted_path(ls_, f_x_, d1, c1, a_initial_, pp);
    }
    int ka = 0;
    for (int j = 0; j < kp; ++j) {
        bool held = false;
        for (int q = 0; q < k; ++q) held = held || std::memcmp(&pp[j], &tree_[q], sizeof(double)) == 0;
        if (!held) break;
        pp[ka++] = pp[j];
    }
    if (ka == 0 || std::memcmp(&pp[0], &tree_[0], sizeof(double)) != 0) { path_tree_++; return k; }
    for (int j = 0; j < 7; ++j) pts[j] = j < ka ? pp[j] : 0.0;
    path_part_ = ka < k;
    path_pred_++;
    return ka;
}

int check_batch_config(const cgo_cg_config &cfg, const cgo_ls_config &ls, std::string &why) {
    if (cfg.beta.kind == CGO_BETA_LBFGS) { why = "batched solves: β = L-BFGS is not supported (CG flavours only)"; return CGO_EINVAL; }
    if (cfg.beta.kind == CGO_BETA_BROYDEN_FAMILY) { why = "batched solves: β = Broyden family is not supported (CG flavours only)"; return CGO_EINVAL; }
    if (ls.kind == CGO_LS_BACKTRACKING) { why = "batched solves: the Backtracking line search is not supported (StrongWolfeBisection or WolfeBisection)"; return CGO_EINVAL; }
    return CGO_OK;
}

int run_batch(VecBackend *be, const cgo_cg_config &cfg, const cgo_ls_config &ls, int64_t batch, int64_t slice_iters, BatchRun &out) {
    ResConfig c{};
    c.ls = ls; c.eps = cfg.eps; c.mu = cfg.beta.mu; c.beta_kind = cfg.beta.kind;
    c.npts = 3; c.max_iters = cfg.max_iters; c.log_on = 0;
    const int64_t budget = slice_iters > 0 ? slice_iters : 64;
    out.evals.assign((size_t)batch, 0);
    out.launches = 0;
    std::vector<char> live((size_t)batch, 1);
    for (;;) {
        if (int rc = be->batch_launch(c, budget, out.st, out.f_x0)) return rc;
        out.launches++;
        if ((int64_t)out.st.size() != batch || (int64_t)out.f_x0.size() != batch) return CGO_ESTATE;
        bool any = false;
        for (int64_t b = 0; b < batch; ++b) {
            if (!live[(size_t)b]) continue;
            const ResState &s = out.st[(size_t)b];
            out.evals[(size_t)b] += s.evals;
            if (s.reason == RES_STOP || s.reason == RES_HOST) live[(size_t)b] = 0;
            else if (s.reason == RES_BUDGET && s.done > 0) any = true;
            else return CGO_ESTATE;
        }
        if (!any) break;
    }
    return CGO_OK;
}

int Solver::iterate_sys(int64_t iters, bool &finished) {
    for (int64_t budget = iters; budget > 0 && !finished_; --budget) {
        const int64_t n = it_ + 1;
        if (n > cfg_.max_iters) { finish(cfg_.max_iters, CGO_MAX_ITERS_REACHED); break; }
        if (norm_df_x_ < cfg_.eps) { finish(n - 1, CGO_SUCCESS); break; }
        const double s0 = lss_.s, rho = lss_.rho;
        double a = NAN, phi = NAN, dphi = NAN, nrm = NAN;
        int64_t hit = -1;
        int rc;
        for (int64_t i = 0; i < lss_.max_iters; ++i) {
            a = s0 * std::pow(rho, (double)i);
            double nxt[6];
            for (int q = 0; q < 6; ++q) nxt[q] = (i + 1 + q < lss_.max_iters) ? s0 * std::pow(rho, (double)(i + 1 + q)) : NAN;
            if ((rc = evaln(a, phi, dphi, nxt, 6))) return rc;
// ... 59 lines not shown
```

conjugategradientoptim.jl_amd/csrc/cgo_engine.hpp:

```cpp
#pragma once

#include <cmath>
#include <cstdint>
#include <memory>
#include <string>
#include <vector>

#include "../../include/cgo.h"
#include "cgo_ctl.hpp"
#include "cgo_path.hpp"
#include "cgo_resident.hpp"

namespace cgo {

struct Scal {
    double f = 0;
    double gtu = 0;
    double gtgt = 0;
    double gtg = 0;
    double yy = 0;
    double uy = 0;
    double ygt = 0;
    double gu = 0;
    double uu = 0;
    double curv = NAN;
};

enum KernelKind : int {
    KK_INIT = 0,
    KK_TRIAL,
    KK_ACCEPT_DIR_TRIAL,
    KK_ACCEPT_DIR,
    KK_ACCEPT_ONLY,
    KK_RESET_DIR,
    KK_UPG_NORM,
    KK_LBFGS_PUSH,
    KK_LBFGS_LOOP,
    KK_LBFGS_FINAL,
    KK_LSE_STATS,
    KK_LSE_GRAD,
    KK_SCALED_NORM,
    KK_DIR_TRIAL,
    KK_SYS_PROJECT,
    KK_RESIDENT,
    KK_ACCEPT_TRIAL_NOSTORE,
    KK_MATERIALIZE_XU,
    KK_ACCEPT_TRIAL_LAZY,
    KK_MATERIALIZE_U,
    KK_COUNT
};

struct Comm {
    int rank = 0, world = 1;
    virtual ~Comm() {}
    virtual int allgather_host(const double *send, double *recv, int count) = 0;
    virtual int allgather_device(const double *, double *, int, void * ) { return -1; }
    virtual int kind() const { return 3; }
    virtual int ranks_seen() { return world; }
    virtual double *shm_slot_host(int , int ) { return nullptr; }
    virtual double *shm_slot_dev(int , int ) { return nullptr; }
    virtual int connect_devices() { return 0; }
    virtual double *dev_mailbox(int ) { return nullptr; }
};

struct VecBackend {
    virtual ~VecBackend() {}
    virtual int64_t n_local() const = 0;
    virtual int set_x0_host(const double *x0) = 0;
    virtual int set_x0_fill(int kind, uint64_t seed, double lo, double hi) = 0;
    virtual int init_eval(Scal &out) = 0;
    virtual int max_points() const { return 1; }
    virtual int trial(const double *a, int k, Scal *out) = 0;
    virtual int accept_dir_trial(double a_acc, double beta, const double *a, int k, Scal *out) = 0;
    virtual bool path_rows() const { return false; }
    virtual int accept_dir_trial_path(double a_acc, double beta, const double *a, int k, Scal *out) { return accept_dir_trial(a_acc, beta, a, k, out); }
    virtual int ctl_depth() const { return 0; }
    virtual int accept_dir_trial_ctl(const CtlConfig &, const CtlState &s, int64_t , Scal *out) {
        return accept_dir_trial(s.a_acc, s.beta, s.a, s.npts, out);
    }
    virtual bool resident_ready(const cgo_cg_config &, const cgo_ls_config &) const { return false; }
    virtual int resident_run(const ResConfig &, ResState &, int64_t , std::vector<ResRecord> &, std::vector<ResLog> &) { return CGO_EINVAL; }
    virtual int batch_launch(const ResConfig &, int64_t , std::vector<ResState> & , std::vector<double> & ) { return CGO_EINVAL; }
    virtual bool sys_supported() const { return false; }
    virtual int sys_begin() { return CGO_EINVAL; }
    virtual int sys_project(double , double , Scal &) { return CGO_EINVAL; }
    virtual int sys_commit() { return CGO_EINVAL; }
    virtual int dir_trial(double , const double * , int , Scal *) { return CGO_EINVAL; }
    virtual int accept_dir(double a_acc, double beta, Scal &out) = 0;
    virtual int accept_only(double a_acc) = 0;
    virtual int reset_dir(Scal &out) = 0;
    virtual int upg_sumsq(double &out) = 0;
    virtual int lbfgs_push(double a_x, double a_s, int slot, double &sy, double &yy) = 0;
    virtual int lbfgs_direction(const int *slots, const double *rho, int count, double gamma,
                                Scal &out) = 0;
    virtual int lbfgs_alloc(int slots) = 0;
    virtual int lbfgs_gram_max_pairs() const { return 0; }
    struct GramOut {
        double sy, yy, sgn, ygn;
        double sjg[16], yjg[16], sjyn[16], yjsn[16], yjyn[16];
        bool materialized = false;
        bool y_based = false;
        double gtgt = 0.0;
    };
    virtual int lbfgs_push_gram(double, double, int, const int *, int, GramOut &) { return CGO_EINVAL; }
    virtual bool lbfgs_push_materializes(double ) { return false; }
    virtual int lbfgs_push_commit(bool ) { return CGO_OK; }
    virtual bool lbfgs_push_spec(double , double , int , const int * , int , GramOut &) { return false; }
    virtual int lbfgs_direction_gram(const int *, const double *, const double *, int, double, Scal &) { return CGO_EINVAL; }
    virtual bool lbfgs_direction_gram_can_fuse_trial() const { return false; }
    virtual int lbfgs_direction_gram_trial(const int *, const double *, const double *, int, double, double , Scal & , Scal & ) { return CGO_EINVAL; }
    virtual bool two_phase() const { return false; }
    virtual void discard_pending() {}
    virtual int materialize(Scal &) { return 0; }
    virtual int download(double *x, double *g) = 0;
    virtual int scaled_norm_parts(int which, double a_trial, double &maxabs, double &scaled_ss, bool &has_nan) = 0;
    virtual void profile_enable(bool) {}
    virtual void profile_reset() {}
    virtual void profile_get(int, int64_t *launches, double *ms, double *bytes) {
        *launches = 0; *ms = 0; *bytes = 0;
    }
    virtual int64_t launches() const { return 0; }
};

const char *status_name(int s);
const char *kernel_kind_name(int k);
int check_cg_config(const cgo_cg_config *c, std::string &why);
int check_ls_config(const cgo_ls_config *l, std::string &why);
int check_lss_config(const cgo_lss_config *l, std::string &why);
int64_t lss_default_max_iters(double rho);

double beta_from_scalars(const cgo_beta_config &b, const Scal &t, double gu_old, double gg_old,
                         double uu_old);

struct TrialRecord { double a, phi, dphi; };

class Solver {
  public:
    Solver(VecBackend *be, const cgo_cg_config &cfg, const cgo_ls_config &ls);
    Solver(VecBackend *be, const cgo_cg_config &cfg, const cgo_lss_config &lss);
    int start();
    int iterate(int64_t iters, bool &finished);
    double objective() const { return f_x_; }
    int64_t iters_ran() const { return iters_ran_; }
    int status() const { return status_; }
    bool finished() const { return finished_; }
    int64_t total_evals() const { return total_evals_; }
    const std::vector<double> &trace_objective() const { return tr_f_; }
    const std::vector<double> &trace_grad_norm() const { return tr_g_; }
    const std::vector<double> &trace_step_size() const { return tr_a_; }
    const std::vector<int64_t> &trace_evals() const { return tr_e_; }
    const std::vector<TrialRecord> &trial_log() const { return log_; }
    void set_log_enabled(bool on) { log_on_ = on; }
    VecBackend *backend() { return be_; }
    const cgo_cg_config &config() const { return cfg_; }
    const cgo_ls_config &linesearch() const { return ls_; }
    bool is_sys() const { return sys_; }
    void path_stats(int64_t &predicted, int64_t &tree, int64_t &misses) const { predicted = path_pred_; tree = path_tree_; misses = path_miss_; }
    void set_path_skew(double f) { path_skew_ = f; }
    void resume(double f_x0, int64_t evals, const ResState &s, const ResRecord *recs);

  private:
    void adopt(const ResState &s, const ResRecord *recs, const ResLog *log);
    int eval(double a, double &phi, double &dphi, double h1 = NAN, double h2 = NAN, double h3 = NAN, double h4 = NAN);
    int evaln(double a, double &phi, double &dphi, const double *hints, int nh);
    void first_hints(double a0, double (&h)[2]) const;
    int ls_strong_wolfe(double a_initial, LSOut &o);
    int ls_wolfe_bisection(double a_initial, LSOut &o);
    int ls_backtracking(double a_initial, LSOut &o);
    int find_feasible(double &a, double lb, int64_t &evals, double &phi, double &dphi,
                      int &flag, double h1 = NAN, double h2 = NAN, double h3 = NAN, double h4 = NAN);
    double first_step(double a_initial) const;
    int robust_norm(double sumsq, int which, double &out);
    void finish(int64_t iters, int status);
    int iterate_sys(int64_t iters, bool &finished);
    int run_resident(int64_t cap, int64_t &done, int &reason);
    std::vector<ResRecord> res_recs_;
    int res_fail_streak_ = 0;
    int64_t res_backoff_ = 0;
    std::vector<ResLog> res_log_;

    VecBackend *be_;
    cgo_cg_config cfg_;
    cgo_ls_config ls_;
    bool sys_ = false;
    cgo_lss_config lss_{};
    bool started_ = false, finished_ = false;
    double f_x_ = NAN, f_x0_ = NAN, norm_df_x_ = NAN, gg_ = NAN;
    double a_initial_ = NAN;
    int64_t it_ = 0;
    int64_t iters_ran_ = 0;
    int status_ = CGO_INCOMPLETE;
    double dphi0_ = NAN, uu_ = NAN;
    bool dir_is_neg_grad_ = true;
    struct Cached { double a; Scal s; };
    Cached cache_[7];
    int ncache_ = 0;
    Scal last_;
    double last_eval_a_ = NAN;
    int64_t total_evals_ = 0;
    std::vector<int> qn_list_;
    int qn_free_ = 0;
    std::vector<double> qn_rho_;
    double qn_gamma_ = 1.0;
    bool qn_gram_ = false;
    std::vector<double> qn_SY_, qn_YY_, qn_sg_, qn_yg_;
    int qn_direction(Scal &s, double a_trial = NAN, Scal *trial = nullptr);
    bool qn_trial_done_ = false;
    void qn_commit(int slot);
    std::vector<double> tr_f_, tr_g_, tr_a_;
    std::vector<int64_t> tr_e_;
    std::vector<TrialRecord> log_;
    bool log_on_ = false;
    double tree_[7] = {};
    int ntree_ = 0;
    bool path_part_ = false, path_reset_ = false;
    double path_skew_ = 1.0;
    int64_t path_pred_ = 0, path_tree_ = 0, path_miss_ = 0;
    int path_points(double a_xp, double beta, double (&pts)[7], int k);
};

struct BatchRun {
    std::vector<ResState> st;
    std::vector<double> f_x0;
    std::vector<int64_t> evals;
    int64_t launches = 0;
};
int check_batch_config(const cgo_cg_config &cfg, const cgo_ls_config &ls, std::string &why);
int run_batch(VecBackend *be, const cgo_cg_config &cfg, const cgo_ls_config &ls, int64_t batch, int64_t slice_iters, BatchRun &out);

}
```

conjugategradientoptim.jl_amd/csrc/cgo_hip_backend.hip:

```cpp
#include "cgo_backend_internal.hpp"

#include "cgo_kernels.hip.hpp"
#include "cgo_kernels_lse.hip.hpp"
#include "cgo_kernels_cg.hip.hpp"
#include "cgo_kernels_chain.hip.hpp"

namespace cgo {

using namespace dev;

static double wait_timeout_ns() {
    static const double t = [] { const char *e = getenv("CGO_WAIT_TIMEOUT_S"); double v = e ? atof(e) : 0.0; return (v > 0.0 ? v : 120.0) * 1e9; }();
    return t;
}

static thread_local std::string g_err;
void set_error(const std::string &msg) { g_err = msg; }
const char *get_error() { return g_err.c_str(); }


int DevBuf::alloc(size_t count) {
    release();
    if (count == 0) count = 1;
    HIPCHK(hipMalloc((void **)&p, count * sizeof(double)));
    n = count;
    return CGO_OK;
}
void DevBuf::release() {
    if (p) (void)hipFree(p);
    p = nullptr;
    n = 0;
}

HipObjective::~HipObjective() {
    if (host_x) (void)hipHostFree(host_x);
    if (host_g) (void)hipHostFree(host_g);
}

int HipCtx::init(int dev_id) {
    int count = 0;
    hipError_t e = hipGetDeviceCount(&count);
    if (e != hipSuccess || count <= 0) {
        set_error("no HIP device visible: this engine has no CPU fallback (needs an MI355X / gfx950)");
        return CGO_ENODEV;
    }
    if (dev_id < 0 || dev_id >= count) { set_error("device index out of range"); return CGO_EINVAL; }
    HIPCHK(hipSetDevice(dev_id));
    device = dev_id;
    hipDeviceProp_t prop;
    HIPCHK(hipGetDeviceProperties(&prop, dev_id));
    arch = prop.gcnArchName;
    num_cu = prop.multiProcessorCount;
    if (arch.find("gfx950") == std::string::npos) {
        set_error("device is " + arch + "; this library carries gfx950 code objects only");
        return CGO_ENODEV;
    }
    HIPCHK(hipStreamCreateWithFlags(&stream, hipStreamNonBlocking));
    HIPCHK(hipMalloc((void **)&partials, sizeof(double) * MAX_GRID * NG));
    HIPCHK(hipMalloc((void **)&partials2, sizeof(double) * (MAX_GRID / 64) * NG));
    HIPCHK(hipMalloc((void **)&out_dev, sizeof(double) * NG));
    HIPCHK(hipMalloc((void **)&tickets, sizeof(unsigned int) * (TAIL_GROUP + 2)));
    HIPCHK(hipMemset(tickets, 0, sizeof(unsigned int) * (TAIL_GROUP + 2)));
    HIPCHK(hipMalloc((void **)&partials_f, sizeof(double) * MAX_GRID * NR7));
    HIPCHK(hipMalloc((void **)&partials2_f, sizeof(double) * TAIL_GROUP * NG));
    static_assert((TAIL_EMPTY >> 32) == (TAIL_EMPTY & 0xFFFFFFFFull), "filled with a 32-bit pattern");
    HIPCHK(hipMemsetD32((hipDeviceptr_t)partials_f, (int)(TAIL_EMPTY & 0xFFFFFFFFull), (size_t)MAX_GRID * NR7 * 2));
    HIPCHK(hipMemsetD32((hipDeviceptr_t)partials2_f, (int)(TAIL_EMPTY & 0xFFFFFFFFull), (size_t)TAIL_GROUP * NG * 2));
    HIPCHK(hipDeviceSynchronize());
    if (const char *e = getenv("CGO_FUSED_TAIL")) fused_tail = (e[0] != '0');
    if (const char *e = getenv("CGO_TAIL_STRICT")) tail_strict = (e[0] == '1');
    HIPCHK(hipHostMalloc((void **)&host_pinned, sizeof(double) * NG * 64, hipHostMallocDefault));
    HIPCHK(hipHostMalloc((void **)&host_seq, 64, hipHostMallocDefault));
    *host_seq = 0;
    if (const char *e = getenv("CGO_HOST_PUBLISH")) host_publish = (e[0] != '0');
    if (const char *e = getenv("CGO_FORCE_GATHER")) force_gather = (e[0] == '1');
    HIPCHK(hipEventCreate(&ev0));
    HIPCHK(hipEventCreate(&ev1));
    return CGO_OK;
}

void HipCtx::xch_collect() {
    if (!xev_pending) return;
    float ms = 0;
    if (hipEventQuery(xev1) == hipSuccess && hipEventElapsedTime(&ms, xev0, xev1) == hipSuccess) {
        xch_dev_ms += ms; xch_dev_n++;
        xev_pending = false;
    }
}

int HipCtx::ensure_gather() {
    if (gather_dev) return CGO_OK;
    if (world() > 64) { set_error("world size > 64 unsupported"); return CGO_EINVAL; }
    HIPCHK(hipSetDevice(device));
    HIPCHK(hipMalloc((void **)&gather_dev, sizeof(double) * NG * world()));
    return CGO_OK;
}

HipCtx::~HipCtx() {
    if (device < 0) return;
    (void)hipSetDevice(device);
    comm.reset();
    if (stream) (void)hipStreamSynchronize(stream);
    if (partials) (void)hipFree(partials);
    if (partials2) (void)hipFree(partials2);
    if (out_dev) (void)hipFree(out_dev);
    if (tickets) (void)hipFree(tickets);
    if (partials_f) (void)hipFree(partials_f);
    if (partials2_f) (void)hipFree(partials2_f);
    if (gather_dev) (void)hipFree(gather_dev);
    if (host_pinned) (void)hipHostFree(host_pinned);
    if (host_seq) (void)hipHostFree(host_seq);
    if (ev0) (void)hipEventDestroy(ev0);
    if (ev1) (void)hipEventDestroy(ev1);
    if (xev0) (void)hipEventDestroy(xev0);
    if (xev1) (void)hipEventDestroy(xev1);
    if (stream) (void)hipStreamDestroy(stream);
}

double big_bytes_for(double forced, bool read_only) {
    if (forced > 0.0) return forced;
    return read_only ? 4.5e8 : 1.4e9;
}
double env_big_bytes() {
    static const double forced = [] { const char *e = getenv("CGO_BIG_BYTES"); double t = e ? atof(e) : 0.0; return t > 0.0 ? t : 0.0; }();
    return forced;
}
double HipBackend::big_bytes(bool read_only) const { return big_bytes_for(pol_.hbm_stream_bytes, read_only); }
int param_unset_error(int slot) {
    set_error("objective parameter vector (slot " + std::to_string(slot) + ") was never set");
    return CGO_ESTATE;
}
bool is_big(int obj_kind, int mode, int64_t n, int hp, double forced) {
    return bytes_for(obj_kind, mode, n, hp) > big_bytes_for(forced, m_read_only(mode));
}
std::string fused_symbol(const char *obj_tname, int mode, bool big) {
    char buf[160];
    snprintf(buf, sizeof buf, "k_fused<%s, %d, %s>", m_evaluates(mode) ? obj_tname : "ObjQuadDiag", mode, big ? "true" : "false");
    return buf;
}

static int grid_capped(int64_t n, int cap) {
    static const int forced = [] { const char *e = getenv("CGO_GRID_SMALL"); int v = e ? atoi(e) : 0; return (v >= 1 && v <= MAX_GRID) ? v : 0; }();
    static const int per = [] { const char *e = getenv("CGO_GROUPS_PER_LANE"); int v = e ? atoi(e) : 2; return (v >= 1 && v <= 64) ? v : 2; }();
    if (forced) cap = forced;
    const int64_t n2 = n >> 1;
    int64_t blocks = (n2 + (int64_t)BLOCK * per - 1) / ((int64_t)BLOCK * per);
    if (blocks < 1) blocks = 1;
    if (blocks > cap) blocks = cap;
    return (int)blocks;
}

int grid_for(int64_t n) { return grid_capped(n, GRID_SMALL); }

int grid_cg(int64_t n, int npts) {
    static const int cap57 = [] { const char *e = getenv("CGO_GRID_CG7"); int v = e ? atoi(e) : 0; return (v >= 1 && v <= MAX_GRID) ? v : 0; }();
    if (npts >= 5) return grid_capped(n, cap57 ? cap57 : (n <= 2000000 ? 256 : 512));
    return grid_capped(n, n <= 16000000 ? 256 : 512);
// ... 222 lines not shown
        if (timed_x) {
            if (!ctx->xev0) { HIPCHK(hipEventCreate(&ctx->xev0)); HIPCHK(hipEventCreate(&ctx->xev1)); }
            HIPCHK(hipEventRecord(ctx->xev0, ctx->stream));
        }
        dr = ctx->comm->allgather_device(ctx->out_dev, ctx->gather_dev, ns, (void *)ctx->stream);
        ctx->xch_count++;
    }
    if (dr == 2) {
    } else if (dr == 0 && ctx->host_publish) {
        ctx->seq++;
        k_publish<<<1, 64, 0, ctx->stream>>>(ctx->gather_dev, ns * W, h, ctx->host_seq, ctx->seq);
        HIPCHK(hipGetLastError());
        if (timed_x) { HIPCHK(hipEventRecord(ctx->xev1, ctx->stream)); ctx->xev_pending = true; }
        if (int rc = wait_seq(ctx, ctx->seq)) return rc;
    } else if (dr == 0) {
        HIPCHK(hipMemcpyAsync(h, ctx->gather_dev, sizeof(double) * ns * W, hipMemcpyDeviceToHost, ctx->stream));
        HIPCHK(hipStreamSynchronize(ctx->stream));
    } else if (dr < 0) {
        double local[NG];
        HIPCHK(hipMemcpyAsync(h, ctx->out_dev, sizeof(double) * ns, hipMemcpyDeviceToHost, ctx->stream));
        HIPCHK(hipStreamSynchronize(ctx->stream));
        std::memcpy(local, h, sizeof(double) * ns);
        if (ctx->comm->allgather_host(local, h, ns) != 0) {
            set_error("allgather callback failed");
            return CGO_ECOMM;
        }
    } else {
        return CGO_ECOMM;
    }
    if (raw) std::memcpy(raw, h, sizeof(double) * (size_t)ns * W);
    for (int s = 0; s < ns; ++s) {
        double t = 0.0;
        for (int r = 0; r < W; ++r) t += h[r * ns + s];
        sums[s] = t;
    }
    if (merge == MERGE_MAX0) {
        double m = h[0];
        for (int r = 1; r < W; ++r) if (h[r * ns] > m) m = h[r * ns];
        sums[0] = m;
    }
    if (merge == MERGE_LSE) {
        double m = h[L_M], S = h[L_S], T = h[L_T];
        for (int r = 1; r < W; ++r) lse_merge(m, S, T, h[r * ns + L_M], h[r * ns + L_S], h[r * ns + L_T]);
        sums[L_M] = m; sums[L_S] = S; sums[L_T] = T;
    }
    return CGO_OK;
}

static inline bool two_stage_rows(long long rows, int ns) {
    static const long long thr = [] { const char *e = getenv("CGO_FINALIZE_2STAGE_BYTES"); long long v = e ? atoll(e) : 0; return v > 0 ? v : 131072LL; }();
    return rows * ns * 8 > thr;
}

int finalize_rows(HipCtx *ctx, int rows, int ns, bool canon) {
    hipStream_t st = ctx->stream;
    ctx->seq++;
    double *hp; unsigned long long *hs;
    ctx->pub_target(&hp, &hs);
    if (ctx->fused_tail && rows > TAIL_GROUP && rows <= TAIL_GROUP * TAIL_GROUP && (canon || two_stage_rows(rows, ns))) {
        Tail t{};
        t.partials2 = ctx->partials2_f; t.tickets = ctx->tickets; t.out = ctx->out_dev;
        t.host_out = hp; t.host_seq = hs; t.seq = ctx->seq; t.strict = ctx->tail_strict ? 1 : 0;
        ctx->pub_checked = (hp != nullptr) && !ctx->tail_strict;
        const int nb = (rows + TAIL_GROUP - 1) / TAIL_GROUP;
        const bool ok = with_width<NG, NR, NR5, NR7, NRC3, NS>(ns, false, [&](auto w) { k_finalize_one<decltype(w)::value><<<nb, BLOCK, 0, st>>>(ctx->partials, rows, t); });
        if (!ok) { set_error("internal: no single-launch reduction for this row width"); return CGO_EINVAL; }
        HIPCHK(hipGetLastError());
        return CGO_OK;
    }
    const double *src = ctx->partials;
    int nrows = rows;
    if (canon) {
        if (rows > TAIL_GROUP * TAIL_GROUP) { set_error("internal: more partial rows than two levels of 64 reduce"); return CGO_EINVAL; }
        if (rows > TAIL_GROUP) {
            const int nb = (rows + TAIL_GROUP - 1) / TAIL_GROUP;
            with_width<NR, NR5, NR7, NRC3, NS>(ns, true, [&](auto w) { k_finalize_t<decltype(w)::value, BLOCK><<<nb, BLOCK, 0, st>>>(ctx->partials, TAIL_GROUP, rows, ctx->partials2, nullptr, nullptr, 0); });
            HIPCHK(hipGetLastError());
            src = ctx->partials2;
            nrows = nb;
        }
        with_width<NR, NR5, NR7, NRC3, NS>(ns, true, [&](auto w) { k_finalize_t<decltype(w)::value, BLOCK><<<1, BLOCK, 0, st>>>(src, nrows, nrows, ctx->out_dev, hp, hs, ctx->seq); });
        HIPCHK(hipGetLastError());
        return CGO_OK;
    }
    if (two_stage_rows(rows, ns)) {
        const int nb = (rows + 63) / 64;
        with_width<NG, NS>(ns, true, [&](auto w) { constexpr int N = decltype(w)::value, T = N == NG ? 768 : BLOCK; k_finalize_t<N, T><<<nb, T, 0, st>>>(ctx->partials, 64, rows, ctx->partials2, nullptr, nullptr, 0); });
        HIPCHK(hipGetLastError());
        src = ctx->partials2;
        nrows = nb;
    }
    with_width<NG, NS>(ns, true, [&](auto w) { constexpr int N = decltype(w)::value, T = N == NG ? 768 : BLOCK; k_finalize_t<N, T><<<1, T, 0, st>>>(src, nrows, nrows, ctx->out_dev, hp, hs, ctx->seq); });
    HIPCHK(hipGetLastError());
    return CGO_OK;
}

int finalize_launch(HipCtx *ctx, int grid, bool lse) {
    if (!lse) return finalize_rows(ctx, grid, NS);
    ctx->seq++;
    double *hp; unsigned long long *hs;
    ctx->pub_target(&hp, &hs);
    if (grid > 1024) {
        const int nb = (grid + 63) / 64;
        k_finalize_lse<<<nb, BLOCK, 0, ctx->stream>>>(ctx->partials, 64, grid, ctx->partials2, nullptr, nullptr, 0);
        k_finalize_lse<<<1, BLOCK, 0, ctx->stream>>>(ctx->partials2, nb, nb, ctx->out_dev, hp, hs, ctx->seq);
    } else {
        k_finalize_lse<<<1, BLOCK, 0, ctx->stream>>>(ctx->partials, grid, grid, ctx->out_dev, hp, hs, ctx->seq);
    }
    HIPCHK(hipGetLastError());
    return CGO_OK;
}

HipBackend::HipBackend(HipCtx *ctx, HipObjective *obj) : ctx_(ctx), obj_(obj) {
    cgo_solver_policy_init(&pol_);
    epoch_ = ++ctx->solver_epoch;
}
void HipBackend::set_policy(const cgo_solver_policy &p) {
    pol_ = p;
    ctl_fused_ = p.controller_fused != 0;
    if (p.fused_tail >= 0) ctx_->fused_tail = p.fused_tail != 0;
    if (p.strict_tail >= 0) ctx_->tail_strict = p.strict_tail != 0;
}
HipBackend::~HipBackend() {
    if (pipe_done_ < pipe_enq_ && ctx_->stream) (void)hipStreamSynchronize(ctx_->stream);
    if (placed_ && x_.p && u_.p && !ctx_->placed_x.p && !ctx_->placed_u.p) {
        if (ctx_->stream) (void)hipStreamSynchronize(ctx_->stream);
        std::swap(x_.p, ctx_->placed_x.p); std::swap(x_.n, ctx_->placed_x.n);
        std::swap(u_.p, ctx_->placed_u.p); std::swap(u_.n, ctx_->placed_u.n);
        ctx_->placed_n = obj_->n_local;
        ctx_->placed_first_us = place_first_us_; ctx_->placed_best_us = place_best_us_; ctx_->placed_candidates = place_candidates_;
    }
    for (auto &g : graphs_) if (g.exec) (void)hipGraphExecDestroy((hipGraphExec_t)g.exec);
    if (ctl_dev_) (void)hipFree(ctl_dev_);
    if (ctl_rec_) (void)hipHostFree(ctl_rec_);
    if (ctl_seq_) (void)hipHostFree(ctl_seq_);
    if (qn_alpha_dev_) (void)hipFree(qn_alpha_dev_);
    if (res_state_ || res_xbuf_) { if (ctx_->stream) (void)hipStreamSynchronize(ctx_->stream); }
    if (res_state_) (void)hipHostFree(res_state_);
    if (res_recs_) (void)hipHostFree(res_recs_);
    if (res_log_) (void)hipHostFree(res_log_);
// ... 10 lines not shown
    if (bat_fx0_) (void)hipFree(bat_fx0_);
    if (bat_S_) (void)hipFree(bat_S_);
    if (bat_Y_) (void)hipFree(bat_Y_);
    if (bat_qn_) (void)hipFree(bat_qn_);
    if (bat_s0v_) (void)hipFree(bat_s0v_);
    for (auto &r : ring_) { if (r.e0) (void)hipEventDestroy(r.e0); if (r.e1) (void)hipEventDestroy(r.e1); }
}

int HipBackend::alloc() {
    HIPCHK(hipSetDevice(ctx_->device));
    const size_t n = (size_t)obj_->n_local + (chain() ? (size_t)(obj_->n_local & 1) : 0);
    if (ctx_->placed_n != obj_->n_local && (ctx_->placed_x.p || ctx_->placed_u.p)) {
        ctx_->placed_x.release(); ctx_->placed_u.release(); ctx_->placed_n = 0;
    }
    if (int rc = x_.alloc(n)) return rc;
    if (int rc = u_.alloc(n)) return rc;
    if (chain()) {
        HIPCHK(hipMemsetAsync(x_.p, 0, n * sizeof(double), ctx_->stream));
        HIPCHK(hipMemsetAsync(u_.p, 0, n * sizeof(double), ctx_->stream));
    }
    xc_ = x_.p; uc_ = u_.p;
    if (chain()) {
        if (int rc = x2_.alloc(n)) return rc;
        if (int rc = u2_.alloc(n)) return rc;
        HIPCHK(hipMemsetAsync(x2_.p, 0, n * sizeof(double), ctx_->stream));
        HIPCHK(hipMemsetAsync(u2_.p, 0, n * sizeof(double), ctx_->stream));
        xalt_ = x2_.p; ualt_ = u2_.p;
        pingpong_ = 1;
    }
    if (!rmode_) {
        if (int rc = ensure_ga()) return rc;
        if (int rc = ensure_gb()) return rc;
    }
    return CGO_OK;
}

int HipBackend::ensure_ga() {
    if (!ga_.p) { if (int rc = ga_.alloc((size_t)obj_->n_local + (size_t)(obj_->n_local & 1))) return rc; }
    if (!g_) g_ = ga_.p;
    return CGO_OK;
}
int HipBackend::ensure_gb() {
    if (!gb_.p) { if (int rc = gb_.alloc((size_t)obj_->n_local)) return rc; }
    if (!gt_) gt_ = gb_.p;
    xn_ = (xc_ == gb_.p) ? x_.p : gb_.p;
    return CGO_OK;
}

int HipBackend::set_x0_host(const double *x0) {
    if (int rc = pipe_drain()) return rc;
    discard_pending();
    u_lag_ = false;
    rep_n_ = 0;
    HIPCHK(hipSetDevice(ctx_->device));
    xc_ = x_.p; xn_ = gb_.p;
    if (pingpong_ == 1) xalt_ = x2_.p;
    HIPCHK(hipMemcpyAsync(xc_, x0, sizeof(double) * (size_t)obj_->n_local, hipMemcpyHostToDevice, ctx_->stream));
    HIPCHK(hipStreamSynchronize(ctx_->stream));
    return CGO_OK;
}

int HipBackend::set_x0_device(const double *x0_dev) {
    if (int rc = pipe_drain()) return rc;
    discard_pending();
    u_lag_ = false;
    rep_n_ = 0;
    HIPCHK(hipSetDevice(ctx_->device));
    xc_ = x_.p; xn_ = gb_.p;
    if (pingpong_ == 1) xalt_ = x2_.p;
    HIPCHK(hipMemcpyAsync(xc_, x0_dev, sizeof(double) * (size_t)obj_->n_local, hipMemcpyDeviceToDevice, ctx_->stream));
    HIPCHK(hipStreamSynchronize(ctx_->stream));
    return CGO_OK;
}

int fill_device(HipCtx *ctx, double *v, int64_t n, int64_t offset, int kind, uint64_t seed, double lo,
                double hi) {
    HIPCHK(hipSetDevice(ctx->device));
    int grid = (int)std::min<int64_t>((n + BLOCK - 1) / BLOCK, GRID_SMALL);
    if (grid < 1) grid = 1;
    k_fill<<<grid, BLOCK, 0, ctx->stream>>>(v, n, offset, kind, seed, lo, hi);
    HIPCHK(hipGetLastError());
    return CGO_OK;
}

int HipBackend::set_x0_fill(int kind, uint64_t seed, double lo, double hi) {
    if (int rc = pipe_drain()) return rc;
    discard_pending();
    u_lag_ = false;
    rep_n_ = 0;
    xc_ = x_.p; xn_ = gb_.p;
    if (pingpong_ == 1) xalt_ = x2_.p;
    return fill_device(ctx_, xc_, obj_->n_local, obj_->offset, kind, seed, lo, hi);
}

int HipBackend::prof_slot(hipEvent_t *e0, hipEvent_t *e1) {
    if (ring_.empty()) {
        ring_.resize(1024);
        for (auto &r : ring_) { HIPCHK(hipEventCreate(&r.e0)); HIPCHK(hipEventCreate(&r.e1)); r.kk = -1; }
    }
    if (ring_used_ == (int)ring_.size()) prof_flush();
    ProfSlot &r = ring_[ring_used_++];
    r.kk = -1;
    *e0 = r.e0; *e1 = r.e1;
    return CGO_OK;
}
void HipBackend::profile_enable(bool on) {
    prof_on_ = on;
    if (on && ring_.empty() && hipSetDevice(ctx_->device) == hipSuccess) {
        ring_.resize(1024);
        for (auto &r : ring_) { if (hipEventCreate(&r.e0) != hipSuccess || hipEventCreate(&r.e1) != hipSuccess) { (void)hipGetLastError(); } r.kk = -1; }
    }
}

bool HipBackend::prof_pick(int kk) {
    const int every = obj_->n_local >= 30000000 ? 1 : prof_every_;
    if (capturing_) { prof_cur_ = false; return false; }
    prof_cur_ = prof_on_ && (prof_tick_[kk]++ % every) == 0;
    return prof_cur_;
}
int HipBackend::prof_begin(int kk) {
    if (!prof_pick(kk)) return CGO_OK;
    hipEvent_t e0, e1;
    if (int rc = prof_slot(&e0, &e1)) return rc;
    HIPCHK(hipEventRecord(e0, ctx_->stream));
    return CGO_OK;
}
int HipBackend::prof_end() {
    if (!prof_cur_ || ring_used_ == 0) return CGO_OK;
    HIPCHK(hipEventRecord(ring_[ring_used_ - 1].e1, ctx_->stream));
    return CGO_OK;
}
void HipBackend::prof_commit(int kk, double bytes) {
    prof_cnt_[kk]++;
    prof_bytes_[kk] = bytes;
    if (!prof_cur_ || ring_used_ == 0) return;
    ring_[ring_used_ - 1].kk = kk;
    ring_[ring_used_ - 1].bytes = bytes;
    prof_cur_ = false;
}
void HipBackend::prof_flush() {
    if (ring_used_ == 0) return;
    (void)hipStreamSynchronize(ctx_->stream);
// ... 39 lines not shown
    }
    if (probe_stored_) {
        probe_note(nullptr, 0, "%s", fused_symbol(obj_tname(), mode, is_big(obj_->kind, mode, obj_->n_local, obj_->nparams(), pol_.hbm_stream_bytes)).c_str());
        if (fetch) probe_append(sums, NS);
    }
    if (prof_on_) prof_commit(kk, bytes_for(obj_->kind, mode, obj_->n_local, obj_->nparams()));
    return CGO_OK;
}

static void unpack(const double *s, Scal &o, bool trial, bool dir) {
    if (trial) {
        o.f = s[S_F]; o.gtu = s[S_GTU]; o.gtgt = s[S_GTGT]; o.gtg = s[S_GTG];
        o.yy = s[S_YY]; o.uy = s[S_UY]; o.ygt = s[S_YGT];
    }
    if (dir) { o.gu = s[S_GU]; o.uu = s[S_UU]; }
}

int HipBackend::init_eval(Scal &out) {
    if (int rc = flush_lite()) return rc;
    if (rmode_) {
        double s[NR7];
        if (chain() && !ctx_->single()) {
            if (int rc = launch_r(KK_INIT, R_EDGES, 0, 0, nullptr, 0, true, s)) return rc;
        }
        if (int rc = launch_rk(KK_INIT, 0, 0, nullptr, 0, true, s)) return rc;
        out = Scal();
        out.f = s[RS_F]; out.gtgt = s[RS_GTGT];
        return CGO_OK;
    }
    if (obj_->host_closure()) return host_trial(0.0, true, out);
    if (obj_->two_phase()) {
        out = Scal();
        if (int rc = lse_stats(LM_NOU, 0, 0, 0, out, false)) return rc;
        const double f = out.f;
        if (int rc = lse_grad(true, 0.0, out)) return rc;
        out.f = f;
        std::swap(g_, gt_);
        return CGO_OK;
    }
    double s[NS];
    if (int rc = launch_k(KK_INIT, 0, 0, 0, true, s)) return rc;
    std::swap(g_, gt_);
    out = Scal();
    out.f = s[S_F];
    out.gtgt = s[S_GTGT];
    return CGO_OK;
}

int HipBackend::trial(const double *a, int k, Scal *out) {
    if (rmode_) {
        double s[NR7];
        if (int rc = trial_r(a, k, s)) return rc;
        unpack_r(s, k, out, false);
        return CGO_OK;
    }
    if (obj_->host_closure()) return host_trial(a[0], false, out[0]);
    if (obj_->two_phase()) return lse_stats(0, 0, 0, a[0], out[0], false);
    if (int rc = flush_lite()) return rc;
    spec_valid_ = false; spec_unmat_ = false;
    double s[NS];
    if (int rc = launch_k(KK_TRIAL, 0, 0, a[0], true, s)) return rc;
    unpack(s, out[0], true, false);
    return CGO_OK;
}

int HipBackend::accept_dir_trial(double a_acc, double beta, const double *a, int k, Scal *out) {
    if (rmode_) {
        double s[NR7];
        if (int rc = accept_dir_trial_r(a_acc, beta, a, k, s)) return rc;
        unpack_r(s, k, out, true);
        return CGO_OK;
    }
    double s[NS];
    if (obj_->host_closure()) {
        Scal d;
        if (int rc = accept_dir(a_acc, beta, d)) return rc;
        if (int rc = host_trial(a[0], false, out[0])) return rc;
        out[0].gu = d.gu; out[0].uu = d.uu;
        return CGO_OK;
    }
    std::swap(g_, gt_);
    if (obj_->two_phase()) return lse_stats(LM_ACCEPT | LM_DIR, a_acc, beta, a[0], out[0], true);
    if (int rc = launch_k(KK_ACCEPT_DIR_TRIAL, a_acc, beta, a[0], true, s)) return rc;
    unpack(s, out[0], true, true);
    return CGO_OK;
}

int HipBackend::accept_dir_trial_path(double a_acc, double beta, const double *a, int k, Scal *out) {
    if (!path_rows()) return accept_dir_trial(a_acc, beta, a, k, out);
    double s[NR7];
    path_nact_ = k <= 5 ? std::max(k, 1) : MAXP;
    const int rc = accept_dir_trial_r(a_acc, beta, a, k, s);
    path_nact_ = 0;
    if (rc) return rc;
    unpack_r(s, k, out, true, MAXP);
    for (int j = 0; j < k; ++j) { out[j].curv = out[j].yy; out[j].yy = 0.0; }
    return CGO_OK;
}

int HipBackend::accept_dir(double a_acc, double beta, Scal &out) {
    if (rmode_) {
        double s[NR7];
        if (int rc = launch_rk(KK_ACCEPT_DIR, a_acc, beta, nullptr, 0, true, s)) return rc;
        out.gu = s[RS_PER_POINT]; out.uu = s[RS_PER_POINT + 1];
        return CGO_OK;
    }
    double s[NS];
    std::swap(g_, gt_);
    if (int rc = launch_k(KK_ACCEPT_DIR, a_acc, beta, 0, true, s)) return rc;
    unpack(s, out, false, true);
    return CGO_OK;
}

int HipBackend::accept_only(double a_acc) {
    if (rmode_) return launch_rk(KK_ACCEPT_ONLY, a_acc, 0, nullptr, 0, false, nullptr);
    std::swap(g_, gt_);
    return launch_k(KK_ACCEPT_ONLY, a_acc, 0, 0, false, nullptr);
}

int HipBackend::reset_dir(Scal &out) {
    if (int rc = flush_lite()) return rc;
    if (rmode_) {
        double s[NR7];
        if (int rc = launch_rk(KK_RESET_DIR, 0, 0, nullptr, 0, true, s)) return rc;
        out.gu = s[RS_PER_POINT]; out.uu = s[RS_PER_POINT + 1];
        return CGO_OK;
    }
    double s[NS];
    if (int rc = launch_k(KK_RESET_DIR, 0, 0, 0, true, s)) return rc;
    unpack(s, out, false, true);
    return CGO_OK;
}

int HipBackend::upg_sumsq(double &out) {
    if (rmode_) {
        double s[NR7];
        if (int rc = launch_rk(KK_UPG_NORM, 0, 0, nullptr, 0, true, s)) return rc;
        out = s[RS_PER_POINT + 1];
        return CGO_OK;
    }
    double s[NS];
    if (int rc = launch_k(KK_UPG_NORM, 0, 0, 0, true, s)) return rc;
    out = s[S_UU];
    return CGO_OK;
}

int HipBackend::sys_begin() {
    if (!rmode_) { set_error("solvesystem needs an element-wise objective (k_cg kernel family)"); return CGO_EINVAL; }
    if (int rc = pipe_drain()) return rc;
// ... 344 lines not shown
```

conjugategradientoptim.jl_amd/csrc/cgo_hip_backend.hpp:

```cpp
#pragma once

#include <hip/hip_runtime.h>

#include <memory>
#include <string>
#include <vector>

#include "cgo_engine.hpp"
#include "cgo_launch_kinds.hpp"
#include "cgo_rtc.hpp"

namespace cgo {

enum class BatchTier : int { LDS = 0, ROWS = 1, LBFGS = 2, LBFGS_LDS = 3 };
constexpr int BATCH_TIERS = 4;
struct BatchTierRow;

namespace dev { struct CtlArgs; struct Tail; struct LoopParams; struct ResParams; struct BatchParams; struct BatchLbfgsParams; }

void set_error(const std::string &msg);
const char *get_error();

struct DevBuf {
    double *p = nullptr;
    size_t n = 0;
    DevBuf() {}
    DevBuf(const DevBuf &) = delete;
    DevBuf &operator=(const DevBuf &) = delete;
    ~DevBuf() { release(); }
    int alloc(size_t count);
    void release();
};

struct HipCtx {
    int device = -1;
    hipStream_t stream = nullptr;
    std::unique_ptr<Comm> comm;
    double *partials = nullptr;
    double *partials2 = nullptr;
    double *out_dev = nullptr;
    unsigned int *tickets = nullptr;
    double *partials_f = nullptr;
    double *partials2_f = nullptr;
    bool pub_checked = false;
    bool tail_strict = false;
    bool fused_tail = true;
    double *gather_dev = nullptr;
    double *host_pinned = nullptr;
    unsigned long long *host_seq = nullptr;
    unsigned long long seq = 0;
    bool host_publish = true;
    long long xch_count = 0;
    double xch_peer_wait_ns = 0;
    hipEvent_t xev0 = nullptr, xev1 = nullptr;
    bool xev_pending = false;
    double xch_dev_ms = 0; long long xch_dev_n = 0;
    void xch_collect();
    bool force_gather = false;
    unsigned long long solver_epoch = 0;
    bool dev_exchange() const { return comm && world() > 1 && comm->dev_mailbox(0) != nullptr; }
    bool single() const { return world() == 1 && !force_gather; }
    bool shm() const { return comm && comm->shm_slot_host(0, 0) != nullptr; }
    void pub_target(double **out, unsigned long long **seqw);
    hipEvent_t ev0 = nullptr, ev1 = nullptr;
    DevBuf placed_x, placed_u;
    int64_t placed_n = 0;
    double placed_first_us = 0.0, placed_best_us = 0.0;
    int placed_candidates = 0;
    std::string arch;
    int num_cu = 0;
    ~HipCtx();
    int init(int device);
    int ensure_gather();
    int rank() const { return comm ? comm->rank : 0; }
    int world() const { return comm ? comm->world : 1; }
};

struct HipObjective {
    HipCtx *ctx = nullptr;
    int kind = 0;
    int64_t n_global = 0, offset = 0, n_local = 0;
    DevBuf p[CGO_MAX_PARAM_SLOTS];
    bool p_set[CGO_MAX_PARAM_SLOTS] = {};
    double s0 = 0.0;
    std::shared_ptr<RtcModule> rtc;
    int user_nparams = 0;
    bool user_cheap = false;
    int users = 0;
    cgo_fdf_fn host_fn = nullptr;
    void *host_user = nullptr;
    double *host_x = nullptr, *host_g = nullptr;
    bool host_closure() const { return kind == CGO_OBJ_HOST; }
// ... 91 lines not shown
    int accept_only(double a_acc) override;
    int reset_dir(Scal &out) override;
    int upg_sumsq(double &out) override;
    int lbfgs_alloc(int slots) override;
    int lbfgs_gram_max_pairs() const override { return gram_on_ ? 12 : 0; }
    int lbfgs_push_gram(double a_x, double a_s, int slot, const int *prev, int count, GramOut &out) override;
    bool lbfgs_push_materializes(double a_x) override;
    bool lbfgs_push_spec(double a_x, double a_s, int slot, const int *prev, int count, GramOut &out) override;
    int lbfgs_push_commit(bool direction_follows) override;
    int lbfgs_direction_gram(const int *slots, const double *cy, const double *cs, int count, double cg,
                             Scal &out) override;
    bool lbfgs_direction_gram_can_fuse_trial() const override;
    int lbfgs_direction_gram_trial(const int *slots, const double *cy, const double *cs, int count, double cg, double a_trial,
                                   Scal &dir, Scal &trial) override;
    int lbfgs_push(double a_x, double a_s, int slot, double &sy, double &yy) override;
    int lbfgs_direction(const int *slots, const double *rho, int count, double gamma,
                        Scal &out) override;
    bool two_phase() const override { return obj_->two_phase(); }
    int materialize(Scal &out) override;
    void discard_pending() override { push_pending_ = false; push_lite_pending_ = false; lite_deferred_ = false; spec_valid_ = false; spec_unmat_ = false; }
    int download(double *x, double *g) override;
    int scaled_norm_parts(int which, double a_trial, double &maxabs, double &scaled_ss, bool &has_nan) override;
    void profile_enable(bool on) override;
    void profile_reset() override;
    void profile_get(int kind, int64_t *launches, double *ms, double *bytes) override;
    int64_t launches() const override { return total_launches_; }
    void set_need_beta(bool b) { need_beta_ = b; }
    void set_rmode(bool on) { rmode_ = on; }
    void set_multi_min_n(int64_t n) { multi_min_n_ = n; }
    void set_multi5_min_n(int64_t n) { multi5_min_n_ = n; }
    void set_multi7_min_n(int64_t n) { multi7_min_n_ = n; }
    void set_three_point_band(int64_t lo, int64_t hi) { band3_lo_ = lo; band3_hi_ = hi; }
    bool rmode() const { return rmode_; }
    void set_lazy_direction(bool on) { lazy_on_ = on; }
    bool lazy_direction() const { return lazy_on_; }
    int set_lazy_direction_now(bool on) { if (!on) { if (int rc = materialize_lag()) return rc; } lazy_on_ = on; return 0; }
    void set_probe_beta_prev(double b) { probe_beta_prev_ = b; }
    void set_replay_depth(int d) { replay_depth_ = d < 1 ? 1 : (d > 16 ? 16 : d); }
    int replay_depth() const { return replay_depth_; }
    int set_replay_depth_now(int d);
    void set_probe_replay(int nrep, const double *a, const double *beta);
    void set_probe_deep_trial(bool on) { probe_deep_t_ = on; }
    struct ReplayStats { int64_t n = 0, s = 0, t = 0, m = 0, t_deep = 0, m_deep = 0; int max_list = 0; };
    const ReplayStats &replay_stats() const { return rstats_; }
    void set_beta_unread(int bits) { lean_mask_ = bits; if (lean_bits_) lean_bits_ = bits; }
    void set_lean_sums(bool on) { lean_bits_ = on ? lean_mask_ : 0; }
    bool lean_sums() const { return lean_bits_ != 0; }
    void set_path_prediction(bool on) { path_on_ = on; }
    bool path_prediction() const { return path_on_; }
    bool path_rows() const override;
    int accept_dir_trial_path(double a_acc, double beta, const double *a, int k, Scal *out) override;
    int64_t path_launches(int nact) const { return (nact >= 1 && nact <= 7) ? path_count_[nact] : 0; }
    void set_probe_path(int nact) { probe_nact_ = nact; }
    std::string kernel_symbol(int kernel_kind) const;
    int probe_launch(int kernel_kind, int variant, double a_acc, double beta, const double *a, int k, const double *x,
                     const double *u, const double *aux, double *sums, int sums_cap, int *sums_len, double *x_out,
                     double *u_out, double *g_out, std::string &symbol);
    bool probed() const { return probe_; }
    int probe_launch_stored(int kernel_kind, int variant, double a_acc, double beta, const double *a, int k, const double *x,
                            const double *u, const double *aux, double *sums, int sums_cap, int *sums_len, double *x_out,
                            double *u_out, double *g_out, std::string &symbol);
    int probe_lbfgs(int m, cgo_lbfgs_probe &p, const double *x, const double *u, const double *g, const double *gt, const double *S,
                    const double *Y, double *x_out, double *xo_out, double *u_out, double *g_out, double *gt_out, double *S_out,
                    double *Y_out);

    int probe_resident(const cgo_cg_config &cfg, const cgo_ls_config &ls, cgo_resident_probe &p, const double *x, const double *u,
                       double *rows, int64_t rows_cap, double *x_out, double *u_out);

    int probe_armed(const cgo_cg_config &cfg, const cgo_ls_config &ls, cgo_armed_probe &p, const double *x, const double *u,
                    double *x_out, double *u_out);

    static int run_dir(HipCtx *ctx, double *u_host, const double *g_host, double beta, int64_t n,
                       double *out2);
    static int run_beta_partials(HipCtx *ctx, const double *gn, const double *g, const double *u,
                                 int64_t n, double *out9);
    static int run_trial(HipObjective *obj, const double *x, const double *u, double a,
                         double *gn_out, double *out2);
    static int run_eval(HipObjective *obj, const double *x, double *g_out, double *f);
    static int bench_kernel(HipCtx *ctx, HipObjective *obj, int kernel_kind, int64_t n, int reps,
                            double *ms, double *bytes);
    static int bench_stream_mix(HipCtx *ctx, int64_t n, int reps, double *median_us, double *best_us);

  private:
    int launch(int kk, int mode, double a_acc, double beta, double a_trial, bool fetch,
               double *sums );
    int launch_k(int kk, double a_acc, double beta, double a_trial, bool fetch, double *sums) { return launch(kk, fused_mode(kk), a_acc, beta, a_trial, fetch, sums); }
    HipCtx *ctx_;
    HipObjective *obj_;
    DevBuf x_, u_, ga_, gb_;
    DevBuf x2_, u2_;
    double *uc_ = nullptr;
    double *xalt_ = nullptr, *ualt_ = nullptr;
    int pingpong_ = -1;
    bool sys_on_ = false;
    bool chain() const { return obj_->kind == CGO_OBJ_ROSENBROCK_CHAINED; }
    bool probe_ = false;
    double probe_row_[64] = {};
    int probe_len_ = 0;
    int last_mode_ = -1, last_npts_ = 0;
    bool last_big_ = false;
    int probe_prepare();
    int probe_slack_intact();
    std::string r_symbol(int mode, int npts, bool big, int nact = 0) const;
    std::string probe_syms_;
    void probe_note(const double *row, int len, const char *fmt, ...);
    int probe_ring_slack_intact();
    bool probe_stored_ = false;
    void probe_append(const double *row, int len);
    const char *obj_tname() const;
    int launch_loop(const dev::LoopParams &P, int kk, double nvec, bool big, int grid);
    double halo_xl_[2] = {0, 0}, halo_ul_[2] = {0, 0}, halo_xr_[2] = {0, 0}, halo_ur_[2] = {0, 0};
    int launch_chain_kernel(int mode, double a_acc, double beta, const double *a, int k, int npts, bool big, int grid, const dev::Tail &tail);
    bool tail_fused(int grid) const;
    bool pipe_fused(int grid) const;
    dev::Tail make_tail(bool on);
    bool pingpong_ready();
    int tune_placement();
    double place_first_us_ = 0.0, place_best_us_ = 0.0;
    int place_candidates_ = 0;
    double place_cap_bytes_ = 0.0;
    bool placed_ = false;
    int ensure_ga();
    int ensure_gb();
    double *xc_ = nullptr, *xn_ = nullptr;
    double *g_ = nullptr, *gt_ = nullptr;
    bool need_beta_ = true;
    bool rmode_ = false;
    int64_t multi_min_n_ = 3000000;
    int64_t multi5_min_n_ = INT64_MAX;
    int64_t multi7_min_n_ = INT64_MAX;
    int64_t band3_lo_ = 0, band3_hi_ = 0;
    int launch_r(int kk, int mode, double a_acc, double beta, const double *a, int k, bool fetch, double *sums);
    int launch_rk(int kk, double a_acc, double beta, const double *a, int k, bool fetch, double *sums) { return launch_r(kk, r_mode_of(kk), a_acc, beta, a, k, fetch, sums); }
    RPlan r_plan(int mode, int npts) const;
    bool adt_is_big() const;
    int fused_mode(int kk) const { const MKind *mk = m_kind(kk); return !mk ? -1 : ((kk == KK_TRIAL && !need_beta_) ? mk->alt : mk->mode); }
    std::string lbfgs_symbol(int kk) const;
    bool lazy_on_ = false, u_lag_ = false;
    double beta_lag_ = 0.0, probe_beta_prev_ = 0.0;
    bool lazy_eligible() const;
    int materialize_u();
    int replay_depth_ = 1, rep_n_ = 0, probe_rep_n_ = 0;
    double rep_a_[15] = {}, rep_b_[15] = {}, probe_rep_a_[15] = {}, probe_rep_b_[15] = {};
    bool probe_deep_t_ = false, deep_t_ = false;
    bool deep_trial(int mode) const;
    ReplayStats rstats_;
    int materialize_lag();
    int lean_mask_ = 0, lean_bits_ = 0;
    int lean_for(int mode) const;
    bool path_on_ = false;
    int path_nact_ = 0, last_nact_ = 0, probe_nact_ = 0;
    int path_last_n_ = 0, path_last_s_ = 0;
    int64_t path_count_[8] = {};
    int accept_dir_trial_r(double a_acc, double beta, const double *a, int k, double *s);
    int trial_r(const double *a, int k, double *s);
    int launch_r_kernel(int kk, int mode, double a_acc, double beta, const double *a, int k, int npts,
                        const struct dev::CtlArgs *ctl, RPlan *plan_out);
    int ctl_depth_ = 0;
    unsigned long long epoch_ = 0;
    void *ctl_dev_ = nullptr;
    void *ctl_rec_ = nullptr;
    unsigned long long *ctl_seq_ = nullptr;
    unsigned long long pipe_enq_ = 0, pipe_done_ = 0;
    bool pipe_stopped_ = false;
    bool pipe_checked_ = false;
    bool ctl_fused_ = true;
    cgo_solver_policy pol_;
    int pipe_npts_ = 1;
    int64_t pipe_streak_ = 0;
    int64_t pipe_served_ = 0;
    std::vector<std::pair<int, unsigned>> pipe_prof_;
    unsigned prof_gen_ = 0;
    int pipe_alloc();
    int pipe_round_kernels();
    int pipe_finalize_ctl(const double *src, int nrows, int ns);
    int pipe_enqueue_round();
    int pipe_launch_graph(int rounds);
    int pipe_enqueue(int64_t count);
    struct PipeGraph { void *exec; int rounds, npts; double *x, *u; const double *p0; int64_t n; std::string syms; };
    std::vector<PipeGraph> graphs_;
    bool graph_on_ = false;
    bool capturing_ = false;
    unsigned long long pipe_batches_ = 0;
    int64_t graph_rounds_ = 0;
    int pipe_wait(unsigned long long id, CtlRecord &rec);
    int pipe_drain();
    int accept_dir_trial_keep_streak(const CtlState &s0, Scal *out);
    bool res_on_ = true;
    int res_grid_ = 0, res_npts_ = 3;
    int64_t res_chunk_ = 0;
    size_t res_lds_ = 0;
    int res_plan();
    int res_alloc();
    void res_out_buffers(double *&xo, double *&uo) const;
    void res_fill_params(dev::ResParams &P, double *xo, double *uo);
    void res_swap_in(double *xo, double *uo);
    int res_error_reset();
    ResState *res_state_ = nullptr;
    ResRecord *res_recs_ = nullptr;
    ResLog *res_log_ = nullptr;
    ResRecord *res_recs_dev_ = nullptr;
    ResLog *res_log_dev_ = nullptr;
    double *res_xbuf_ = nullptr;
    unsigned int *res_err_ = nullptr;
    DevBuf res_xo_, res_uo_;
    double *res_xin_ = nullptr, *res_uin_ = nullptr;
// ... 28 lines not shown
    struct ProfSlot { hipEvent_t e0 = nullptr, e1 = nullptr; int kk = -1; double bytes = 0; };
    std::vector<ProfSlot> ring_;
    int ring_used_ = 0;
    int prof_slot(hipEvent_t *e0, hipEvent_t *e1);
    int prof_begin(int kk);
    int prof_end();
    void prof_commit(int kk, double bytes);
    void prof_flush();
    bool prof_pick(int kk);
    int prof_every_ = 4;
    int64_t prof_tick_[KK_COUNT] = {};
    bool prof_cur_ = false;
    int64_t prof_cnt_[KK_COUNT] = {};
    int64_t prof_n_[KK_COUNT] = {};
    double prof_ms_[KK_COUNT] = {};
    double prof_bytes_[KK_COUNT] = {};
    int64_t total_launches_ = 0;
    int qn_m_ = 0;
    bool gram_on_ = true;
    DevBuf qn_S_, qn_Y_;
    double *qn_alpha_dev_ = nullptr;
    double qn_sgt_ = 0.0;
    int qn_sgt_slot_ = -1;
    bool push_pending_ = false, fuse_grad_ = true;
    double *push_xo_ = nullptr;
    bool spec_on_ = false, spec_valid_ = false, push_lite_pending_ = false;
    bool spec_fuse_push_ = true, lite_deferred_ = false, spec_unmat_ = false;
    int flush_lite();
    double spec_s_[64] = {}, spec_Mr_ = 0.0, spec_Sr_ = 1.0, spec_a_ = 0.0, spec_dphi_ = 0.0;
    int64_t spec_refreshed_ = 0;
    int spec_count_ = 0, spec_slots_[16] = {};
    double lite_a_ = 0.0, lite_as_ = 0.0, lite_M_ = 0.0, lite_S_ = 1.0;
    int lite_slot_ = 0;
    int64_t push_counts_[3] = {0, 0, 0};
    int lbfgs_direction_spec(const int *slots, const double *cy, const double *cs, int count, double cg, double a_trial, Scal &dir, Scal &trial);
    int lbfgs_push_lite();
    int chain_sums(int grid, int slot, const double **dot_ptr, int *dot_count, double *dot_host);
    double lse_a_ = 0.0, lse_M_ = 0.0, lse_S_ = 1.0;
    bool lse_have_ = false;
    int lse_stats(int mode, double a_acc, double beta, double a_trial, Scal &out, bool dir);
    int lse_grad(bool init, double a, Scal &out);
    int host_trial(double a, bool init, Scal &out);
};

int launch_fused(HipCtx *ctx, int obj_kind, int mode, const void *kparams, int64_t n,
                 bool timed = false, const HipObjective *obj = nullptr, hipEvent_t e0 = nullptr,
                 hipEvent_t e1 = nullptr, double big_forced = -1.0 );
int grid_for(int64_t n);
double bytes_for(int obj_kind, int mode, int64_t n, int n_params = 0);
int param_unset_error(int slot);
enum MergeKind { MERGE_SUM = 0, MERGE_LSE = 1, MERGE_MAX0 = 2 };
int fetch_sums(HipCtx *ctx, double *sums, int merge = MERGE_SUM, int ns = 10, double *raw = nullptr);
int finalize_launch(HipCtx *ctx, int grid, bool lse);
int finalize_rows(HipCtx *ctx, int rows, int ns, bool canon = false);
int fill_device(HipCtx *ctx, double *v, int64_t n, int64_t offset, int kind, uint64_t seed, double lo,
                double hi);

Comm *make_rccl_comm(HipCtx *ctx, int rank, int world, const void *unique_id128);
Comm *make_callback_comm(int rank, int world, cgo_allgather_fn fn, void *user);
Comm *make_shm_comm(HipCtx *ctx, int rank, int world, const char *name, int create);
int rccl_unique_id(void *out128);
bool rccl_available();

}
```

conjugategradientoptim.jl_amd/csrc/cgo_kernels_cg_path.hip.hpp:

```cpp
#pragma once

#include "cgo_kernels_cg.hip.hpp"

namespace cgo {
namespace dev {

template <class Obj> struct ObjCurv { static constexpr bool declared = false; };
template <> struct ObjCurv<ObjQuadDiag> {
    static constexpr bool declared = true;
    __device__ static inline d2 apply2(d2 v, const PV<ObjQuadDiag> &p) { return d2{p.v[0].x * v.x, p.v[0].y * v.y}; }
    __device__ static inline double apply1(double v, const PS<ObjQuadDiag> &p) { return p.v[0] * v; }
};

constexpr bool path_mode(int mode) {
    return (r_base(mode) == (R_REPLAY | R_ACCEPT | R_DIR | R_TRIAL | R_NOWU | R_NOWX) || r_base(mode) == (R_REPLAY | R_ACCEPT | R_DIR | R_TRIAL)) &&
           (mode & R_NOYY) != 0;
}

constexpr int RDEEP = 8;
constexpr int RCAP = RMAX + RDEEP;
struct RDeep {
    int nrep2;
    double ra2[RDEEP], rb2[RDEEP];
};
// ... 192 lines not shown
    static_assert(NPTS == 1 || NPTS == 3 || NPTS == 5 || NPTS == 7, "a launch evaluates 1, 3, 5 or 7 trial points");
    constexpr int W = RW<NPTS>::W;
    double acc[W];
#pragma unroll
    for (int s = 0; s < W; ++s) acc[s] = 0.0;
    __shared__ RDeepLds L;
    rdeep_stage(Q, L);
    const long long n2 = P.n >> 1;
    const long long per = big_chunk_pairs(n2, gridDim.x);
    long long i = per * blockIdx.x + threadIdx.x;
    const long long hi = (per * blockIdx.x + per < n2) ? per * blockIdx.x + per : n2;
    const long long step = BLOCK;
    for (; i + step < hi; i += 2 * step) {
        d2 xa = ldg2<true>(P.x, i), xb = ldg2<true>(P.x, i + step);
        d2 ua = ldg2<true>(P.u, i), ub = ldg2<true>(P.u, i + step);
        const PV<Obj> pa = pv_load<Obj, true>(P, i), pb = pv_load<Obj, true>(P, i + step);
        replay_pair<Obj>(P, Q, L, xa, ua, pa);
        cg_trial_points2<Obj, NPTS>(P, xa, ua, pa, acc);
        replay_pair<Obj>(P, Q, L, xb, ub, pb);
        cg_trial_points2<Obj, NPTS>(P, xb, ub, pb, acc);
    }
    if (i < hi) {
        d2 xa = ldg2<true>(P.x, i);
        d2 ua = ldg2<true>(P.u, i);
        const PV<Obj> pa = pv_load<Obj, true>(P, i);
        replay_pair<Obj>(P, Q, L, xa, ua, pa);
        cg_trial_points2<Obj, NPTS>(P, xa, ua, pa, acc);
    }
    if ((P.n & 1) && blockIdx.x == 0 && threadIdx.x == 0) {
        const long long e = P.n - 1;
        double x = P.x[e];
        double u = P.u[e];
        const PS<Obj> p = ps_load<Obj>(P, e);
        replay_single<Obj>(P, Q, L, x, u, p);
        double g = 0.0, f0 = 0.0;
        obj_eval1<Obj>(x, p, P.s0, f0, g);
#pragma unroll
        for (int j = 0; j < NPTS; ++j) {
            const int b = RS_PER_POINT * j;
            const double xp = x + P.a[j] * u;
            double gt;
            obj_term1<Obj, false>(xp, p, P.s0, acc[b + RS_F], gt);
            const double y = gt - g;
            acc[b + RS_GTU] = dsum(acc[b + RS_GTU], gt, u); acc[b + RS_GTGT] = dsum(acc[b + RS_GTGT], gt, gt);
            acc[b + RS_GTG] = dsum(acc[b + RS_GTG], gt, g);
            acc[b + RS_YY] = dsum(acc[b + RS_YY], y, y);
            acc[b + RS_UY] = dsum(acc[b + RS_UY], u, y);
            acc[b + RS_YGT] = dsum(acc[b + RS_YGT], y, gt);
        }
    }
    store_partials_n<W, false>(acc, P.partials, P.tail);
}

}
}
```

conjugategradientoptim.jl_amd/csrc/cgo_path.hpp:

```cpp
#pragma once

#include "cgo_ctl.hpp"

namespace cgo {

struct PathModelEval {
    double f, d0, c;
    double a[CTL_MAXP];
    int n; bool over;
    CGO_HD int operator()(double step, double &phi, double &dphi, double, double, double, double) {
        bool seen = false;
        for (int j = 0; j < CTL_MAXP; ++j) if (j < n && a[j] == step) seen = true;
        if (!seen) {
            if (n >= CTL_MAXP) { over = true; return 1; }
            for (int j = 0; j < CTL_MAXP; ++j) if (j == n) a[j] = step;
            ++n;
        }
        phi = f + step * d0 + 0.5 * (step * step) * c;
        dphi = d0 + step * c;
        return 0;
    }
};

CGO_HD inline int ls_predicted_path(const cgo_ls_config &ls, double f, double dphi0, double c, double a_initial, double (&pts)[7]) {
    for (int j = 0; j < 7; ++j) pts[j] = 0.0;
    if (!(hd_isfinite(f) && hd_isfinite(dphi0) && hd_isfinite(c))) return 0;
    if (!(c > 0.0) || !(dphi0 < 0.0)) return 0;
    if (ls.kind != CGO_LS_STRONG_WOLFE_BISECTION && ls.kind != CGO_LS_WOLFE_BISECTION) return 0;
    if (ls.kind == CGO_LS_WOLFE_BISECTION && ls.cond_kind != CGO_COND_WOLFE) return 0;
    PathModelEval ev;
    ev.f = f; ev.d0 = dphi0; ev.c = c; ev.n = 0; ev.over = false;
    for (int j = 0; j < CTL_MAXP; ++j) ev.a[j] = 0.0;
    LSOut o = ls_out(0.0, 0.0, 0, CGO_INCOMPLETE);
    if (ls.kind == CGO_LS_STRONG_WOLFE_BISECTION) {
        (void)ls_strong_wolfe_t(ls, f, dphi0, a_initial, ev, o);
    } else {
        CtlNoBackend bk;
        double uu = 0.0;
        (void)ls_wolfe_bisection_t(ls, f, dphi0, uu, a_initial, ev, bk, o);
    }
    for (int j = 0; j < 7; ++j) pts[j] = ev.a[j];
    for (int j = 0; j < 7; ++j) if (j < ev.n && !(hd_isfinite(pts[j]) && pts[j] > 0.0)) return 0;
    return ev.n;
}

}
```

include/cgo.h:

```cpp
#ifndef CGO_H
#define CGO_H

#include <stdint.h>

#ifdef __cplusplus
extern "C" {
#endif

#define CGO_VERSION 100

enum {
    CGO_OK = 0,
    CGO_EINVAL = 1,
    CGO_EHIP = 2,
    CGO_ECOMM = 3,
    CGO_ENODEV = 4,
    CGO_ESTATE = 5,
    CGO_ENOMEM = 6
};

enum {
    CGO_INCOMPLETE = 0,
    CGO_SUCCESS = 1,
    CGO_INCREASING_OBJECTIVE = 2,
// ... 300 lines not shown
                                    const cgo_cg_config *cfg, const cgo_ls_config *ls, int64_t slice_iters,
                                    const cgo_batch_policy *policy, cgo_batch_results *out, int32_t *rows_used);
int64_t cgo_batch_lbfgs_max_n_ex(cgo_ctx *ctx, int32_t obj_kind, int32_t m, const cgo_batch_policy *policy);
int64_t cgo_batch_lbfgs_max_n_obj_ex(cgo_objective *model, int32_t m, const cgo_batch_policy *policy);
int32_t cgo_batch_lbfgs_lds_rows(int32_t n_params, int32_t m);
void cgo_batch_lbfgs_lds_shape(int32_t n_params, int32_t *block, int32_t *pairs_per_trip);
int cgo_batch_lbfgs_open(cgo_ctx *ctx, cgo_objective *model, int64_t batch, const double *const *params, int32_t n_params,
                         int32_t m_max, const cgo_batch_policy *policy , cgo_batch **handle);
int cgo_batch_lbfgs_solve(cgo_batch *handle, const double *x0 , const double *scalars ,
                          const unsigned char *active , const cgo_cg_config *cfg, const cgo_ls_config *ls,
                          int64_t slice_iters , cgo_batch_results *out);
int cgo_batch_lbfgs_m(const cgo_batch *handle, int32_t *m_max);
#define CGO_BATCH_PROBE_MAX_PASSES 32
typedef struct cgo_batch_pass {
    int32_t kind, k;
    double a[7];
    double a_acc, beta;
    int32_t co_set, co_count;
    double co_gamma, co_cy[10], co_cs[10];
} cgo_batch_pass;
typedef struct cgo_batch_pass_out {
    double ts[7][7];
    double gu, uu;
    int64_t width, stored;
} cgo_batch_pass_out;
typedef struct cgo_batch_probe_args {
    int32_t tier, obj_kind, m, n_params;
    cgo_objective *model;
    int64_t n, batch;
    const double *x, *u;
    const double *params[4];
    const double *scalars;
    const unsigned char *skip;
    const double *S, *Y;
    const void *qn;
    int32_t npass, reserved;
    cgo_batch_pass pass[CGO_BATCH_PROBE_MAX_PASSES];
    double *rows;
    cgo_batch_pass_out *out;
    double *x_out, *u_out, *g_out, *S_out, *Y_out;
    void *qn_out;
    int32_t *reason;
    int64_t *done, *passes;
    int32_t points, reserved2;
    int64_t ld;
    char symbol[128];
} cgo_batch_probe_args;
int cgo_batch_probe(cgo_ctx *ctx, cgo_batch_probe_args *p);
int64_t cgo_batch_probe_qn_bytes(void);
int cgo_solver_set_path_prediction(cgo_solver *s, int32_t on);
int cgo_solver_path_stats(cgo_solver *s, int64_t *by_nact, int64_t *predicted, int64_t *tree, int64_t *misses);
int cgo_solver_probe_set_path(cgo_solver *s, int32_t nact);
int cgo_solver_debug_set_path_skew(cgo_solver *s, double factor);
int32_t cgo_stop_status(int64_t it, int64_t max_iters, double f_x, double grad_norm, double eps, double f_x0, int64_t *iters_ran);

int cgo_kernel_dir(cgo_ctx *ctx, double *u, const double *g, double beta, int64_t n,
                   double *out2);
int cgo_kernel_beta_partials(cgo_ctx *ctx, const double *g_next, const double *g,
                             const double *u, int64_t n, double *out9);
int cgo_getbeta(cgo_ctx *ctx, const cgo_beta_config *b, const double *g_next, const double *g,
                const double *u, int64_t n, double *beta);
int cgo_kernel_trial(cgo_objective *obj, const double *x, const double *u, double a,
                     double *g_next_out, double *out2);
int cgo_solver_probe_set_beta_prev(cgo_solver *s, double beta_prev);
int cgo_solver_probe_set_replay(cgo_solver *s, int32_t nrep, const double *a, const double *beta);
int cgo_solver_probe_set_deep_trial(cgo_solver *s, int32_t on);
int cgo_solver_probe_launch(cgo_solver *s, int32_t kernel_kind, int32_t variant, double a_acc, double beta,
                            const double *a, int32_t k,
                            const double *x, const double *u, const double *aux,
                            double *sums, int32_t sums_cap, int32_t *sums_len,
                            double *x_out, double *u_out, double *g_out,
                            char *symbol, int32_t symbol_cap);
typedef struct cgo_lbfgs_probe {
    int32_t pass, slot, count, list[16];
    double a, a_s, a_trial, cg, M, S;
    double cy[16], cs[16];
    int32_t deferred_push, lite_slot;
    double a_lite, a_s_lite, M_lite, S_lite;
    int32_t loop_mode, final_step, apply_scale, k, q_from_g, v_ring, v_slot, w_ring, w_slot, dot_count;
    double rho, scale, dot_host;
    const double *dots;
    double alpha[64];
    int32_t spec_check, spec_slot, spec_count, spec_list[16];
    double spec_a_x, spec_a_s;
    int32_t spec_ok, new_in_list, sums_len, reserved;
    double gram[85];
    double sums[64];
    char symbol[256];
} cgo_lbfgs_probe;
int cgo_solver_probe_lbfgs(cgo_solver *s, cgo_lbfgs_probe *p,
                           const double *x, const double *u, const double *g, const double *gt, const double *S, const double *Y,
                           double *x_out, double *xo_out, double *u_out, double *g_out, double *gt_out, double *S_out, double *Y_out);
#define CGO_RESIDENT_PROBE_MAX_PASSES 32
typedef struct cgo_resident_pass {
    int32_t kind, k;
    double a[7];
    double a_acc, beta;
} cgo_resident_pass;
typedef struct cgo_resident_pass_out {
    double ts[7][7];
    double gu, uu;
    int64_t width;
} cgo_resident_pass_out;
typedef struct cgo_resident_probe {
    int32_t npass, reserved;
    cgo_resident_pass pass[CGO_RESIDENT_PROBE_MAX_PASSES];
// ... 50 lines not shown
```

Baseline: 2358.

## Carry predicted next-iteration trial sums inside path launches

Adds a 'path carry' mode. The fused accept/trial path kernel also evaluates the curvature sums for the next iteration's predicted line-search trial points and stores per-block partials. A later trial with matching step sizes is then served by a small finalize/reduction instead of a full HBM streaming pass over x, u and the parameters. It is on by default and can be disabled with the CGO_PATH_CARRY env var. In exchange the path kernel does extra per-element arithmetic and uses more registers, and a misprediction leaves the carried work unused.

```diff
diff --git a/conjugategradientoptim.jl_amd/_lib.py b/conjugategradientoptim.jl_amd/_lib.py
--- a/conjugategradientoptim.jl_amd/_lib.py
+++ b/conjugategradientoptim.jl_amd/_lib.py
@@ -199,6 +199,10 @@
     "cgo_solver_path_stats": (C.c_int, [_vp, i64p, i64p, i64p, i64p]),
     "cgo_solver_probe_set_path": (C.c_int, [_vp, C.c_int32]),
     "cgo_solver_debug_set_path_skew": (C.c_int, [_vp, C.c_double]),
+    "cgo_solver_set_path_carry": (C.c_int, [_vp, C.c_int32]),
+    "cgo_solver_path_carry_stats": (C.c_int, [_vp, i64p, i64p, i64p]),
+    "cgo_solver_probe_set_carry": (C.c_int, [_vp, C.c_int32, dp]),
+    "cgo_solver_probe_carried": (C.c_int, [_vp, dp, C.c_int32, dp, C.c_int32, C.POINTER(C.c_int32)]),
     "cgo_solver_probe_set_replay": (C.c_int, [_vp, C.c_int32, dp, dp]),
     "cgo_solver_probe_set_deep_trial": (C.c_int, [_vp, C.c_int32]),
     "cgo_solver_replay_stats": (C.c_int, [_vp, i64p, i64p, i64p, i64p, i64p, i64p, C.POINTER(C.c_int32)]),
diff --git a/conjugategradientoptim.jl_amd/api.py b/conjugategradientoptim.jl_amd/api.py
--- a/conjugategradientoptim.jl_amd/api.py
+++ b/conjugategradientoptim.jl_amd/api.py
@@ -682,12 +682,20 @@
         check(_lib.lib().cgo_solver_path_stats(self._h, by, C.byref(p), C.byref(t), C.byref(m)))
         return dict(by_nact={j: int(by[j]) for j in (1, 2, 3, 4, 5, 7)}, predicted=p.value, tree=t.value, misses=m.value)
 
+    def set_path_carry(self, on: bool):
+        check(_lib.lib().cgo_solver_set_path_carry(self._h, int(bool(on))))
+
+    def path_carry_stats(self):
+        v = [C.c_int64(0) for _ in range(3)]
+        check(_lib.lib().cgo_solver_path_carry_stats(self._h, *[C.byref(q) for q in v]))
+        return dict(zip(("launches", "served", "unused"), (q.value for q in v)))
+
     def debug_set_path_skew(self, factor: float):
         check(_lib.lib().cgo_solver_debug_set_path_skew(self._h, float(factor)))
 
     def probe_launch(self, kind_name: str, variant: int, a_acc: float, beta: float, a: Sequence[float], x, u=None, aux=None,
                      beta_prev: Optional[float] = None, replay: Optional[Sequence] = None, path_nact: Optional[int] = None,
-                     deep_trial: bool = False):
+                     deep_trial: bool = False, carry: Optional[Sequence[float]] = None):
         L = _lib.lib()
         kk = [L.cgo_kernel_kind_name(k).decode() for k in range(L.cgo_num_kernel_kinds())].index(kind_name)
         if beta_prev is not None:
@@ -698,6 +706,9 @@
             check(L.cgo_solver_probe_set_replay(self._h, len(replay), ra.ctypes.data_as(dp), rb.ctypes.data_as(dp)))
         if path_nact is not None:
             check(L.cgo_solver_probe_set_path(self._h, int(path_nact)))
+        if carry is not None:
+            cv = np.ascontiguousarray(carry, dtype=np.float64)
+            check(L.cgo_solver_probe_set_carry(self._h, len(cv), cv.ctypes.data_as(dp)))
         if deep_trial:
             check(L.cgo_solver_probe_set_deep_trial(self._h, 1))
         n = self.obj.n_local
@@ -713,7 +724,12 @@
         ptr = lambda v: None if v is None else v.ctypes.data_as(dp)
         check(L.cgo_solver_probe_launch(self._h, kk, int(variant), float(a_acc), float(beta), ptr(av), len(a), ptr(x), ptr(u),
                                         ptr(aux), ptr(sums), 64, C.byref(ln), ptr(xo), ptr(uo), ptr(go), sym, 200))
-        return dict(sums=sums[:ln.value].copy(), x=xo, u=uo, g=go, symbol=sym.value.decode())
+        out = dict(sums=sums[:ln.value].copy(), x=xo, u=uo, g=go, symbol=sym.value.decode())
+        if carry is not None:
+            row, rl = np.full(64, np.nan), C.c_int32(0)
+            check(L.cgo_solver_probe_carried(self._h, cv.ctypes.data_as(dp), len(cv), ptr(row), 64, C.byref(rl)))
+            out["carried"] = row[:rl.value].copy()
+        return out
 
     LBFGS_PASSES = ("push", "push_gram", "direction_gram", "direction_trial", "push_lite", "loop")
 
diff --git a/conjugategradientoptim.jl_amd/csrc/cgo_backend_cg.hip b/conjugategradientoptim.jl_amd/csrc/cgo_backend_cg.hip
--- a/conjugategradientoptim.jl_amd/csrc/cgo_backend_cg.hip
+++ b/conjugategradientoptim.jl_amd/csrc/cgo_backend_cg.hip
@@ -58,6 +58,19 @@
     return -1;
 }
 template <class Obj>
+static int launch_cg_carry(int mode, int nact, int ncarry, const RParams &P, const RDeep &Q, const RCarry &C, int grid, hipStream_t st) {
+#define ROW(MODE, NACT, NCARRY) if (mode == (MODE) && nact == (NACT) && ncarry == (NCARRY)) { k_cg_path<Obj, (MODE), (NACT), true, (NCARRY)><<<grid, BLOCK, 0, st>>>(P, Q, C); return 0; }
+    CGO_CG_CARRY_ROWS(ROW)
+#undef ROW
+    return -1;
+}
+static inline bool carry_row(int mode, int nact, int ncarry) {
+#define ROW(MODE, NACT, NCARRY) if (mode == (MODE) && nact == (NACT) && ncarry == (NCARRY)) return true;
+    CGO_CG_CARRY_ROWS(ROW)
+#undef ROW
+    return false;
+}
+template <class Obj>
 static int launch_cg_deep_t(int npts, const RParams &P, const RDeep &Q, int grid, hipStream_t st) {
 #define ROW(NPTS) if (npts == (NPTS)) { k_cg_trial_deep<Obj, (NPTS), true><<<grid, BLOCK, 0, st>>>(P, Q); return 0; }
     CGO_CG_DEEP_T_ROWS(ROW)
@@ -83,6 +96,11 @@
     if (!path_on_ || !path_objective(obj_->kind) || replay_depth_ < 2 || !lazy_eligible()) return false;
     const int mode_n = r_mode_of(KK_ACCEPT_TRIAL_NOSTORE), mode_s = R_REPLAY | R_ADT;
     return path_row(mode_n | lean_for(mode_n), MAXP) && path_row(mode_s | lean_for(mode_s), MAXP);
+}
+
+bool HipBackend::carry_row_for(int nact, int kc) const {
+    const int mode_n = r_mode_of(KK_ACCEPT_TRIAL_NOSTORE), mode_s = R_REPLAY | R_ADT;
+    return carry_row(mode_n | lean_for(mode_n), nact, kc) && carry_row(mode_s | lean_for(mode_s), nact, kc);
 }
 
 static inline bool lean_row(int mode) {
@@ -116,6 +134,7 @@
                          double *sums) {
     if (int rc = pipe_drain()) return rc;
     pipe_streak_ = 0;
+    carry_drop();
     if (u_lag_ && !(mode & R_ULAG)) {
         if (r_reads_u(mode)) { if (int rc = materialize_u()) return rc; }
         else if (mode & (R_INIT | R_RESET)) u_lag_ = false;
@@ -154,6 +173,11 @@
         }
         if (probe_ && fetch) { std::memcpy(probe_row_, sums, sizeof(double) * rows_for(npts)); probe_len_ = rows_for(npts); }
     }
+    if (carry_n_ && path_nact_) {
+        carry_valid_ = true; carry_k_ = carry_n_; carry_grid_ = grid;
+        for (int j = 0; j < carry_n_; ++j) carry_a_[j] = carry_req_[j];
+        cstats_.launches++;
+    }
     if (prof_on_) prof_commit(kk, plan.bytes);
     return CGO_OK;
 }
@@ -224,14 +248,14 @@
         if (rep_n_ < replay_depth_ - 1 && rep_n_ < (path_nact_ ? RCAP : RMAX)) {
             const int mode_n = r_mode_of(KK_ACCEPT_TRIAL_NOSTORE);
             if (int rc = launch_r(KK_ACCEPT_TRIAL_NOSTORE, mode_n | lean_for(mode_n), a_acc, beta, a, k, true, s)) return rc;
-            if (path_nact_) { path_last_n_ = path_nact_; path_count_[path_nact_]++; }
+            if (path_nact_) { path_last_n_ = path_nact_; path_last_n_carry_ = carry_n_; path_count_[path_nact_]++; }
             rep_a_[rep_n_] = a_acc; rep_b_[rep_n_] = beta; rep_n_++;
             rstats_.n++;
             return CGO_OK;
         }
         const int mode_s = R_REPLAY | R_ADT;
         if (int rc = launch_r(KK_ACCEPT_DIR_TRIAL, mode_s | lean_for(mode_s), a_acc, beta, a, k, true, s)) return rc;
-        if (path_nact_) { path_last_s_ = path_nact_; path_count_[path_nact_]++; }
+        if (path_nact_) { path_last_s_ = path_nact_; path_last_s_carry_ = carry_n_; path_count_[path_nact_]++; }
         rep_n_ = 0;
         rstats_.s++;
         return CGO_OK;
@@ -245,7 +269,37 @@
     u_lag_ = false;
     return CGO_OK;
 }
+int HipBackend::trial_carried(int k, double *s) {
+    if (int rc = pipe_drain()) return rc;
+    pipe_streak_ = 0;
+    if (rep_n_ > 0 && lazy_eligible()) { rstats_.t++; if (rep_n_ > RMAX) rstats_.t_deep++; }
+    HIPCHK(hipSetDevice(ctx_->device));
+    const int ns = rows_for(npts_for(k));
+    total_launches_++;
+    if (int rc = prof_begin(KK_TRIAL_CARRIED)) return rc;
+    if (int rc = finalize_rows(ctx_, carry_grid_, ns, true, ctx_->carry_partials)) return rc;
+    if (int rc = prof_end()) return rc;
+    if (int rc = fetch_sums(ctx_, s, MERGE_SUM, ns)) return rc;
+    if (prof_on_) prof_commit(KK_TRIAL_CARRIED, 0.0);
+    carry_valid_ = false; carry_hit_ = true;
+    cstats_.served++;
+    return CGO_OK;
+}
+int HipBackend::probe_carried(const double *a, int k, double *row, int cap, int *len) {
+    *len = 0;
+    if (!probe_ || !carry_valid_ || k != carry_k_ || std::memcmp(a, carry_a_, sizeof(double) * k) != 0) { set_error("probe: no carried row for these points"); return CGO_EINVAL; }
+    double s[NR7];
+    if (int rc = trial_carried(k, s)) return rc;
+    carry_hit_ = false;
+    const int ns = rows_for(npts_for(k));
+    if (ns > cap) { set_error("probe: cap smaller than the carried row"); return CGO_EINVAL; }
+    std::memcpy(row, s, sizeof(double) * ns);
+    *len = ns;
+    return CGO_OK;
+}
+
 int HipBackend::trial_r(const double *a, int k, double *s) {
+    if (carry_valid_ && k == carry_k_ && std::memcmp(a, carry_a_, sizeof(double) * k) == 0) return trial_carried(k, s);
     if (rep_n_ > 0 && lazy_eligible()) {
         rstats_.t++;
         if (rep_n_ > RMAX) rstats_.t_deep++;
@@ -285,6 +339,9 @@
     const bool big = plan.big; const int grid = plan.grid;
     const bool deep_t = deep_trial(mode);
     last_mode_ = mode; last_npts_ = plan.npts; last_big_ = big; last_nact_ = deep_t ? -1 : path_nact_;
+    const int ncarry = path_nact_ ? carry_n_ : 0;
+    last_ncarry_ = ncarry;
+    if (ncarry && (!carry_row(mode, path_nact_, ncarry) || grid > GRID_BIG || tail_fused(grid) || !ctx_->carry_partials)) { set_error("internal: not a carrying path row"); return CGO_EINVAL; }
     if (path_nact_ && (chain() || !big || ctl || !path_row(mode, path_nact_) || !path_objective(obj_->kind))) { set_error("internal: not a path row"); return CGO_EINVAL; }
     if (chain()) {
         if (int rc = prof_begin(kk)) return rc;
@@ -326,7 +383,17 @@
     hipStream_t st = ctx_->stream;
     if (int rc = prof_begin(kk)) return rc;
     int r = -2;
-    if (path_nact_) {
+    if (ncarry) {
+        RCarry C;
+        C.partials = ctx_->carry_partials;
+        for (int j = 0; j < NCARRY_MAX; ++j) C.a[j] = j < ncarry ? carry_req_[j] : 0.0;
+        switch (obj_->kind) {
+#define ROW(KIND, T) case KIND: r = launch_cg_carry<T>(mode, path_nact_, ncarry, P, Q, C, grid, st); break;
+        CGO_OBJ_CURV_ROWS(ROW)
+#undef ROW
+        default: break;
+        }
+    } else if (path_nact_) {
         switch (obj_->kind) {
 #define ROW(KIND, T) case KIND: r = launch_cg_path<T>(mode, path_nact_, P, Q, grid, st); break;
         CGO_OBJ_CURV_ROWS(ROW)
@@ -391,10 +458,11 @@
     return CGO_OK;
 }
 
-std::string HipBackend::r_symbol(int mode, int npts, bool big, int nact) const {
+std::string HipBackend::r_symbol(int mode, int npts, bool big, int nact, int ncarry) const {
     char buf[160];
     if (chain()) snprintf(buf, sizeof buf, "k_chain<%d, %d, %s>", mode, npts, big ? "true" : "false");
     else if (nact < 0) snprintf(buf, sizeof buf, "k_cg_trial_deep<%s, %d, true>", obj_tname(), npts);
+    else if (nact && ncarry) snprintf(buf, sizeof buf, "k_cg_path<%s, %d, %d, true, %d>", obj_tname(), mode, nact, ncarry);
     else if (nact) snprintf(buf, sizeof buf, "k_cg_path<%s, %d, %d, true>", obj_tname(), mode, nact);
     else snprintf(buf, sizeof buf, "k_cg<%s, %d, %d, %s>", obj_tname(), mode, npts, big ? "true" : "false");
     return buf;
@@ -421,7 +489,7 @@
     if ((mode & R_REPLAY) && (mode & R_ACCEPT)) mode |= lean_for(mode);
     if ((mode & R_REPLAY) && (mode & R_ACCEPT) && path_rows()) {
         const int last = kk == KK_ACCEPT_TRIAL_NOSTORE ? path_last_n_ : path_last_s_;
-        return r_symbol(mode, plan.npts, plan.big, last ? last : MAXP);
+        return r_symbol(mode, plan.npts, plan.big, last ? last : MAXP, kk == KK_ACCEPT_TRIAL_NOSTORE ? path_last_n_carry_ : path_last_s_carry_);
     }
     if (kk == KK_TRIAL && deep_trial(mode)) return r_symbol(mode, plan.npts, plan.big, -1);
     return r_symbol(mode, plan.npts, plan.big);
@@ -770,6 +838,9 @@
     probe_nact_ = 0;
     const bool want_deep = probe_deep_t_;
     probe_deep_t_ = false;
+    const int want_carry = probe_carry_n_;
+    probe_carry_n_ = 0;
+    carry_drop();
     const bool lse = obj_->two_phase();
     if (k < 0 || k > MAXP || (k > 0 && !a)) { set_error("probe: 0 ≤ k ≤ 7 trial steps"); return CGO_EINVAL; }
     if (!rmode_ && !lse) return probe_launch_stored(kk, variant, a_acc, beta, a, k, x, u, aux, sums, sums_cap, sums_len, x_out, u_out, g_out, symbol);
@@ -849,12 +920,18 @@
             if (!path_row(mode, want_nact) || !path_objective(obj_->kind) || k > want_nact) { rep_n_ = 0; set_error("probe: not a path row of this solver, or more steps than it evaluates"); return CGO_EINVAL; }
             path_nact_ = want_nact;
         }
+        if (want_carry) {
+            if (!want_nact || !carry_row(mode, want_nact, want_carry)) { path_nact_ = 0; rep_n_ = 0; set_error("probe: not a carrying path row of this solver"); return CGO_EINVAL; }
+            carry_n_ = want_carry;
+            for (int j = 0; j < want_carry; ++j) carry_req_[j] = probe_carry_a_[j];
+        }
         rc = launch_r(kk, mode, a_acc, beta, a, k, true, s);
+        carry_n_ = 0;
         path_nact_ = 0;
         deep_t_ = false;
         rep_n_ = 0;
         if (rc) return rc;
-        symbol = r_symbol(last_mode_, last_npts_, last_big_, last_nact_);
+        symbol = r_symbol(last_mode_, last_npts_, last_big_, last_nact_, last_ncarry_);
     }
     HIPCHK(hipStreamSynchronize(st));
     if (x_out) HIPCHK(hipMemcpyAsync(x_out, xc_, nb, hipMemcpyDeviceToHost, st));
diff --git a/conjugategradientoptim.jl_amd/csrc/cgo_capi.hip b/conjugategradientoptim.jl_amd/csrc/cgo_capi.hip
--- a/conjugategradientoptim.jl_amd/csrc/cgo_capi.hip
+++ b/conjugategradientoptim.jl_amd/csrc/cgo_capi.hip
@@ -500,6 +500,12 @@
     if (pol.resident >= 0) s->be->set_resident(pol.resident != 0);
     if (int prc = s->be->prepare_controller()) { delete s; obj_unref(obj); return prc; }
     s->sv = ls ? new Solver(s->be, *cfg, *ls) : new Solver(s->be, *cfg, *lss);
+    {
+        const int forced = env_tri("CGO_PATH_CARRY");
+        const bool carry = forced >= 0 ? forced != 0 : true;
+        s->be->set_path_carry(carry);
+        s->sv->set_path_carry(carry);
+    }
     *out = s;
     return CGO_OK;
 }
@@ -760,6 +766,45 @@
     if (tree) *tree = t;
     if (misses) *misses = m;
     return CGO_OK;
+    API_GUARD_END
+}
+
+int cgo_solver_set_path_carry(cgo_solver *s, int32_t on) {
+    API_GUARD_BEGIN
+    REQUIRE(s && s->sv, "null argument");
+    s->be->set_path_carry(on != 0);
+    s->sv->set_path_carry(on != 0);
+    return CGO_OK;
+    API_GUARD_END
+}
+
+int cgo_solver_path_carry_stats(cgo_solver *s, int64_t *launches, int64_t *served, int64_t *unused) {
+    API_GUARD_BEGIN
+    REQUIRE(s, "null argument");
+    const HipBackend::CarryStats &c = s->be->carry_stats();
+    if (launches) *launches = c.launches;
+    if (served) *served = c.served;
+    if (unused) *unused = c.unused;
+    return CGO_OK;
+    API_GUARD_END
+}
+
+int cgo_solver_probe_set_carry(cgo_solver *s, int32_t kc, const double *a) {
+    API_GUARD_BEGIN
+    REQUIRE(s, "null argument");
+    REQUIRE(kc >= 0 && kc <= 3 && (kc == 0 || a), "probe carried request: 0 … 3 steps");
+    s->be->set_probe_carry(kc, a);
+    return CGO_OK;
+    API_GUARD_END
+}
+
+int cgo_solver_probe_carried(cgo_solver *s, const double *a, int32_t k, double *row, int32_t cap, int32_t *len) {
+    API_GUARD_BEGIN
+    REQUIRE(s && a && row && len && k >= 1 && k <= 3, "null argument, or not 1 … 3 steps");
+    int n = 0;
+    const int rc = s->be->probe_carried(a, k, row, cap, &n);
+    *len = n;
+    return rc;
     API_GUARD_END
 }
 
diff --git a/conjugategradientoptim.jl_amd/csrc/cgo_engine.cpp b/conjugategradientoptim.jl_amd/csrc/cgo_engine.cpp
--- a/conjugategradientoptim.jl_amd/csrc/cgo_engine.cpp
+++ b/conjugategradientoptim.jl_amd/csrc/cgo_engine.cpp
@@ -36,7 +36,7 @@
     "init", "trial", "accept_dir_trial", "accept_dir", "accept_only",
     "reset_dir", "upg_norm", "lbfgs_push", "lbfgs_loop", "lbfgs_final", "lse_stats", "lse_grad",
     "scaled_norm", "dir_trial", "sys_project", "resident", "accept_trial_nostore", "materialize_xu",
-    "accept_trial_lazy", "materialize_u",
+    "trial_carried", "accept_trial_lazy", "materialize_u",
 };
 
 const char *kernel_kind_name(int k) { return (k >= 0 && k < KK_COUNT) ? kKernelNames[k] : "unknown"; }
@@ -158,7 +158,7 @@
     qn_trial_done_ = false;
     res_fail_streak_ = 0; res_backoff_ = 0;
     tr_f_.clear(); tr_g_.clear(); tr_a_.clear(); tr_e_.clear(); log_.clear();
-    path_part_ = false; path_reset_ = false;
+    path_part_ = false; path_reset_ = false; ncarry_ = 0;
     path_pred_ = 0; path_tree_ = 0; path_miss_ = 0;
     return CGO_OK;
 }
@@ -205,15 +205,9 @@
         path_part_ = false;
         path_miss_++;
     } else {
-        double pts[7] = {a, 0, 0, 0, 0, 0, 0};
-        int k = 1;
         const int mp = sys_ ? be_->max_points() : std::min(be_->max_points(), 3);
-        for (int q = 0; q < nh && k < mp; ++q) {
-            const double h = hs[q];
-            bool ok = std::isfinite(h) && h > 0.0;
-            for (int j = 0; ok && j < k; ++j) ok = (h != pts[j]);
-            if (ok) pts[k++] = h;
-        }
+        double pts[7];
+        const int k = ls_trial_request(a, hs, nh, mp, pts);
         Scal out[7];
         if (int rc = be_->trial(pts, k, out)) return rc;
         ncache_ = k;
@@ -545,7 +539,8 @@
                 rc = be_->accept_dir_trial_ctl(cc, cs, budget, out);
             } else if (be_->path_rows() && k >= 6) {
                 k = path_points(a_xp, beta, pts, k);
-                rc = be_->accept_dir_trial_path(a_xp, beta, pts, k, out);
+                rc = ncarry_ ? be_->accept_dir_trial_path_carry(a_xp, beta, pts, k, carry_, ncarry_, out)
+                             : be_->accept_dir_trial_path(a_xp, beta, pts, k, out);
             } else {
                 rc = be_->accept_dir_trial(a_xp, beta, pts, k, out);
             }
@@ -564,15 +559,16 @@
     ntree_ = k;
     for (int j = 0; j < 7; ++j) tree_[j] = pts[j];
     path_part_ = false;
+    ncarry_ = 0;
     int kp = 0;
-    double pp[7] = {0, 0, 0, 0, 0, 0, 0};
+    double pp[7] = {0, 0, 0, 0, 0, 0, 0}, hh[7][4] = {};
     if (cfg_.beta.kind == CGO_BETA_POLAK_RIBIERE && !path_reset_ && std::isfinite(last_.curv) && std::isfinite(beta) &&
         std::isfinite(a_xp) && a_xp > 0.0 && std::isfinite(dphi0_) && std::isfinite(last_.gtu) && std::isfinite(last_.gtgt) &&
         std::isfinite(last_.ygt) && std::isfinite(f_x_)) {
         const double c_k = (last_.gtu - dphi0_) / a_xp;
         const double d1 = -last_.gtgt + beta * last_.gtu;
         const double c1 = (last_.curv - 2.0 * beta * last_.ygt / a_xp + beta * beta * c_k) * path_skew_;
-        kp = ls_predicted_path(ls_, f_x_, d1, c1, a_initial_, pp);
+        kp = ls_predicted_path_hints(ls_, f_x_, d1, c1, a_initial_, pp, hh);
     }
     int ka = 0;
     for (int j = 0; j < kp; ++j) {
@@ -582,6 +578,7 @@
         pp[ka++] = pp[j];
     }
     if (ka == 0 || std::memcmp(&pp[0], &tree_[0], sizeof(double)) != 0) { path_tree_++; return k; }
+    if (path_carry_ && !sys_) ncarry_ = ls_predicted_carry(pp, hh, kp, ka, std::min(be_->max_points(), 3), carry_);
     for (int j = 0; j < 7; ++j) pts[j] = j < ka ? pp[j] : 0.0;
     path_part_ = ka < k;
     path_pred_++;
diff --git a/conjugategradientoptim.jl_amd/csrc/cgo_engine.hpp b/conjugategradientoptim.jl_amd/csrc/cgo_engine.hpp
--- a/conjugategradientoptim.jl_amd/csrc/cgo_engine.hpp
+++ b/conjugategradientoptim.jl_amd/csrc/cgo_engine.hpp
@@ -45,6 +45,7 @@
     KK_RESIDENT,
     KK_ACCEPT_TRIAL_NOSTORE,
     KK_MATERIALIZE_XU,
+    KK_TRIAL_CARRIED,
     KK_ACCEPT_TRIAL_LAZY,
     KK_MATERIALIZE_U,
     KK_COUNT
@@ -74,6 +75,9 @@
     virtual int accept_dir_trial(double a_acc, double beta, const double *a, int k, Scal *out) = 0;
     virtual bool path_rows() const { return false; }
     virtual int accept_dir_trial_path(double a_acc, double beta, const double *a, int k, Scal *out) { return accept_dir_trial(a_acc, beta, a, k, out); }
+    virtual int accept_dir_trial_path_carry(double a_acc, double beta, const double *a, int k, const double * , int , Scal *out) {
+        return accept_dir_trial_path(a_acc, beta, a, k, out);
+    }
     virtual int ctl_depth() const { return 0; }
     virtual int accept_dir_trial_ctl(const CtlConfig &, const CtlState &s, int64_t , Scal *out) {
         return accept_dir_trial(s.a_acc, s.beta, s.a, s.npts, out);
@@ -156,6 +160,8 @@
     const cgo_ls_config &linesearch() const { return ls_; }
     bool is_sys() const { return sys_; }
     void path_stats(int64_t &predicted, int64_t &tree, int64_t &misses) const { predicted = path_pred_; tree = path_tree_; misses = path_miss_; }
+    void set_path_carry(bool on) { path_carry_ = on; }
+    bool path_carry() const { return path_carry_; }
     void set_path_skew(double f) { path_skew_ = f; }
     void resume(double f_x0, int64_t evals, const ResState &s, const ResRecord *recs);
 
@@ -217,6 +223,9 @@
     double path_skew_ = 1.0;
     int64_t path_pred_ = 0, path_tree_ = 0, path_miss_ = 0;
     int path_points(double a_xp, double beta, double (&pts)[7], int k);
+    bool path_carry_ = false;
+    double carry_[7] = {};
+    int ncarry_ = 0;
 };
 
 struct BatchRun {
diff --git a/conjugategradientoptim.jl_amd/csrc/cgo_hip_backend.hip b/conjugategradientoptim.jl_amd/csrc/cgo_hip_backend.hip
--- a/conjugategradientoptim.jl_amd/csrc/cgo_hip_backend.hip
+++ b/conjugategradientoptim.jl_amd/csrc/cgo_hip_backend.hip
@@ -58,6 +58,7 @@
     HIPCHK(hipStreamCreateWithFlags(&stream, hipStreamNonBlocking));
     HIPCHK(hipMalloc((void **)&partials, sizeof(double) * MAX_GRID * NG));
     HIPCHK(hipMalloc((void **)&partials2, sizeof(double) * (MAX_GRID / 64) * NG));
+    HIPCHK(hipMalloc((void **)&carry_partials, sizeof(double) * GRID_BIG * NR));
     HIPCHK(hipMalloc((void **)&out_dev, sizeof(double) * NG));
     HIPCHK(hipMalloc((void **)&tickets, sizeof(unsigned int) * (TAIL_GROUP + 2)));
     HIPCHK(hipMemset(tickets, 0, sizeof(unsigned int) * (TAIL_GROUP + 2)));
@@ -103,6 +104,7 @@
     if (stream) (void)hipStreamSynchronize(stream);
     if (partials) (void)hipFree(partials);
     if (partials2) (void)hipFree(partials2);
+    if (carry_partials) (void)hipFree(carry_partials);
     if (out_dev) (void)hipFree(out_dev);
     if (tickets) (void)hipFree(tickets);
     if (partials_f) (void)hipFree(partials_f);
@@ -431,8 +433,9 @@
     return rows * ns * 8 > thr;
 }
 
-int finalize_rows(HipCtx *ctx, int rows, int ns, bool canon) {
+int finalize_rows(HipCtx *ctx, int rows, int ns, bool canon, const double *partials) {
     hipStream_t st = ctx->stream;
+    if (!partials) partials = ctx->partials;
     ctx->seq++;
     double *hp; unsigned long long *hs;
     ctx->pub_target(&hp, &hs);
@@ -442,18 +445,18 @@
         t.host_out = hp; t.host_seq = hs; t.seq = ctx->seq; t.strict = ctx->tail_strict ? 1 : 0;
         ctx->pub_checked = (hp != nullptr) && !ctx->tail_strict;
         const int nb = (rows + TAIL_GROUP - 1) / TAIL_GROUP;
-        const bool ok = with_width<NG, NR, NR5, NR7, NRC3, NS>(ns, false, [&](auto w) { k_finalize_one<decltype(w)::value><<<nb, BLOCK, 0, st>>>(ctx->partials, rows, t); });
+        const bool ok = with_width<NG, NR, NR5, NR7, NRC3, NS>(ns, false, [&](auto w) { k_finalize_one<decltype(w)::value><<<nb, BLOCK, 0, st>>>(partials, rows, t); });
         if (!ok) { set_error("internal: no single-launch reduction for this row width"); return CGO_EINVAL; }
         HIPCHK(hipGetLastError());
         return CGO_OK;
     }
-    const double *src = ctx->partials;
+    const double *src = partials;
     int nrows = rows;
     if (canon) {
         if (rows > TAIL_GROUP * TAIL_GROUP) { set_error("internal: more partial rows than two levels of 64 reduce"); return CGO_EINVAL; }
         if (rows > TAIL_GROUP) {
             const int nb = (rows + TAIL_GROUP - 1) / TAIL_GROUP;
-            with_width<NR, NR5, NR7, NRC3, NS>(ns, true, [&](auto w) { k_finalize_t<decltype(w)::value, BLOCK><<<nb, BLOCK, 0, st>>>(ctx->partials, TAIL_GROUP, rows, ctx->partials2, nullptr, nullptr, 0); });
+            with_width<NR, NR5, NR7, NRC3, NS>(ns, true, [&](auto w) { k_finalize_t<decltype(w)::value, BLOCK><<<nb, BLOCK, 0, st>>>(partials, TAIL_GROUP, rows, ctx->partials2, nullptr, nullptr, 0); });
             HIPCHK(hipGetLastError());
             src = ctx->partials2;
             nrows = nb;
@@ -464,7 +467,7 @@
     }
     if (two_stage_rows(rows, ns)) {
         const int nb = (rows + 63) / 64;
-        with_width<NG, NS>(ns, true, [&](auto w) { constexpr int N = decltype(w)::value, T = N == NG ? 768 : BLOCK; k_finalize_t<N, T><<<nb, T, 0, st>>>(ctx->partials, 64, rows, ctx->partials2, nullptr, nullptr, 0); });
+        with_width<NG, NS>(ns, true, [&](auto w) { constexpr int N = decltype(w)::value, T = N == NG ? 768 : BLOCK; k_finalize_t<N, T><<<nb, T, 0, st>>>(partials, 64, rows, ctx->partials2, nullptr, nullptr, 0); });
         HIPCHK(hipGetLastError());
         src = ctx->partials2;
         nrows = nb;
@@ -581,6 +584,7 @@
     discard_pending();
     u_lag_ = false;
     rep_n_ = 0;
+    carry_drop();
     HIPCHK(hipSetDevice(ctx_->device));
     xc_ = x_.p; xn_ = gb_.p;
     if (pingpong_ == 1) xalt_ = x2_.p;
@@ -594,6 +598,7 @@
     discard_pending();
     u_lag_ = false;
     rep_n_ = 0;
+    carry_drop();
     HIPCHK(hipSetDevice(ctx_->device));
     xc_ = x_.p; xn_ = gb_.p;
     if (pingpong_ == 1) xalt_ = x2_.p;
@@ -617,6 +622,7 @@
     discard_pending();
     u_lag_ = false;
     rep_n_ = 0;
+    carry_drop();
     xc_ = x_.p; xn_ = gb_.p;
     if (pingpong_ == 1) xalt_ = x2_.p;
     return fill_device(ctx_, xc_, obj_->n_local, obj_->offset, kind, seed, lo, hi);
@@ -762,6 +768,8 @@
         double s[NR7];
         if (int rc = trial_r(a, k, s)) return rc;
         unpack_r(s, k, out, false);
+        if (carry_hit_) { for (int j = 0; j < k; ++j) out[j].curv = carry_curv_[j]; }
+        carry_hit_ = false;
         return CGO_OK;
     }
     if (obj_->host_closure()) return host_trial(a[0], false, out[0]);
@@ -805,6 +813,23 @@
     if (rc) return rc;
     unpack_r(s, k, out, true, MAXP);
     for (int j = 0; j < k; ++j) { out[j].curv = out[j].yy; out[j].yy = 0.0; }
+    return CGO_OK;
+}
+
+int HipBackend::accept_dir_trial_path_carry(double a_acc, double beta, const double *a, int k, const double *ca, int kc, Scal *out) {
+    const int nact = k <= 5 ? std::max(k, 1) : MAXP;
+    if (!carry_on_ || !path_rows() || !ctx_->single() || !carry_row_for(nact, kc)) return accept_dir_trial_path(a_acc, beta, a, k, out);
+    double s[NR7];
+    path_nact_ = nact;
+    carry_n_ = kc;
+    for (int j = 0; j < kc; ++j) carry_req_[j] = ca[j];
+    const int rc = accept_dir_trial_r(a_acc, beta, a, k, s);
+    path_nact_ = 0;
+    carry_n_ = 0;
+    if (rc) return rc;
+    unpack_r(s, k, out, true, MAXP);
+    for (int j = 0; j < k; ++j) { out[j].curv = out[j].yy; out[j].yy = 0.0; }
+    if (carry_valid_) for (int j = 0; j < kc; ++j) carry_curv_[j] = s[RS_PER_POINT * (nact + j) + RS_YY];
     return CGO_OK;
 }
 
diff --git a/conjugategradientoptim.jl_amd/csrc/cgo_hip_backend.hpp b/conjugategradientoptim.jl_amd/csrc/cgo_hip_backend.hpp
--- a/conjugategradientoptim.jl_amd/csrc/cgo_hip_backend.hpp
+++ b/conjugategradientoptim.jl_amd/csrc/cgo_hip_backend.hpp
@@ -38,6 +38,7 @@
     std::unique_ptr<Comm> comm;
     double *partials = nullptr;
     double *partials2 = nullptr;
+    double *carry_partials = nullptr;
     double *out_dev = nullptr;
     unsigned int *tickets = nullptr;
     double *partials_f = nullptr;
@@ -235,6 +236,13 @@
     int accept_dir_trial_path(double a_acc, double beta, const double *a, int k, Scal *out) override;
     int64_t path_launches(int nact) const { return (nact >= 1 && nact <= 7) ? path_count_[nact] : 0; }
     void set_probe_path(int nact) { probe_nact_ = nact; }
+    void set_path_carry(bool on) { carry_on_ = on; }
+    bool path_carry() const { return carry_on_; }
+    int accept_dir_trial_path_carry(double a_acc, double beta, const double *a, int k, const double *ca, int kc, Scal *out) override;
+    struct CarryStats { int64_t launches = 0, served = 0, unused = 0; };
+    const CarryStats &carry_stats() const { return cstats_; }
+    void set_probe_carry(int kc, const double *ca) { probe_carry_n_ = std::max(0, std::min(kc, 3)); for (int j = 0; j < probe_carry_n_; ++j) probe_carry_a_[j] = ca[j]; }
+    int probe_carried(const double *a, int k, double *row, int cap, int *len);
     std::string kernel_symbol(int kernel_kind) const;
     int probe_launch(int kernel_kind, int variant, double a_acc, double beta, const double *a, int k, const double *x,
                      const double *u, const double *aux, double *sums, int sums_cap, int *sums_len, double *x_out,
@@ -284,7 +292,7 @@
     bool last_big_ = false;
     int probe_prepare();
     int probe_slack_intact();
-    std::string r_symbol(int mode, int npts, bool big, int nact = 0) const;
+    std::string r_symbol(int mode, int npts, bool big, int nact = 0, int ncarry = 0) const;
     std::string probe_syms_;
     void probe_note(const double *row, int len, const char *fmt, ...);
     int probe_ring_slack_intact();
@@ -335,6 +343,15 @@
     int path_nact_ = 0, last_nact_ = 0, probe_nact_ = 0;
     int path_last_n_ = 0, path_last_s_ = 0;
     int64_t path_count_[8] = {};
+    bool carry_on_ = false, carry_valid_ = false, carry_hit_ = false;
+    int carry_n_ = 0, last_ncarry_ = 0, path_last_n_carry_ = 0, path_last_s_carry_ = 0, probe_carry_n_ = 0;
+    double carry_req_[3] = {}, probe_carry_a_[3] = {};
+    int carry_k_ = 0, carry_grid_ = 0;
+    double carry_a_[3] = {}, carry_curv_[3] = {};
+    CarryStats cstats_;
+    bool carry_row_for(int nact, int kc) const;
+    void carry_drop() { if (carry_valid_) { cstats_.unused++; carry_valid_ = false; } }
+    int trial_carried(int k, double *s);
     int accept_dir_trial_r(double a_acc, double beta, const double *a, int k, double *s);
     int trial_r(const double *a, int k, double *s);
     int launch_r_kernel(int kk, int mode, double a_acc, double beta, const double *a, int k, int npts,
@@ -469,7 +486,7 @@
 enum MergeKind { MERGE_SUM = 0, MERGE_LSE = 1, MERGE_MAX0 = 2 };
 int fetch_sums(HipCtx *ctx, double *sums, int merge = MERGE_SUM, int ns = 10, double *raw = nullptr);
 int finalize_launch(HipCtx *ctx, int grid, bool lse);
-int finalize_rows(HipCtx *ctx, int rows, int ns, bool canon = false);
+int finalize_rows(HipCtx *ctx, int rows, int ns, bool canon = false, const double *partials = nullptr);
 int fill_device(HipCtx *ctx, double *v, int64_t n, int64_t offset, int kind, uint64_t seed, double lo,
                 double hi);
 
diff --git a/conjugategradientoptim.jl_amd/csrc/cgo_kernels_cg_path.hip.hpp b/conjugategradientoptim.jl_amd/csrc/cgo_kernels_cg_path.hip.hpp
--- a/conjugategradientoptim.jl_amd/csrc/cgo_kernels_cg_path.hip.hpp
+++ b/conjugategradientoptim.jl_amd/csrc/cgo_kernels_cg_path.hip.hpp
@@ -268,5 +268,122 @@
     store_partials_n<W, false>(acc, P.partials, P.tail);
 }
 
-}
-}
+constexpr int NCARRY_MAX = 3;
+struct RCarry {
+    double *partials;
+    double a[NCARRY_MAX];
+};
+
+template <class Obj, int NACT, int NCARRY>
+__device__ inline void cg_carry_points2(const RParams &P, const RCarry &C, const d2 &x, const d2 &u, const PV<Obj> &p, double (&acc)[RW<MAXP>::W],
+                                        double (&car)[RW<NCARRY>::W]) {
+    d2 g;
+    double f0 = 0.0;
+    obj_eval2<Obj>(x, p, P.s0, f0, g);
+#pragma unroll
+    for (int j = 0; j < NCARRY; ++j) {
+        const int b = RS_PER_POINT * j;
+        d2 xp, gt;
+        xp.x = x.x + C.a[j] * u.x;
+        xp.y = x.y + C.a[j] * u.y;
+        obj_term2<Obj, false>(xp, p, P.s0, car[b + RS_F], gt);
+        const double y0 = gt.x - g.x, y1 = gt.y - g.y;
+        car[b + RS_GTU] = dsum(car[b + RS_GTU], gt.x, u.x);   car[b + RS_GTU] = dsum(car[b + RS_GTU], gt.y, u.y);
+        car[b + RS_GTGT] = dsum(car[b + RS_GTGT], gt.x, gt.x); car[b + RS_GTGT] = dsum(car[b + RS_GTGT], gt.y, gt.y);
+        car[b + RS_GTG] = dsum(car[b + RS_GTG], gt.x, g.x);   car[b + RS_GTG] = dsum(car[b + RS_GTG], gt.y, g.y);
+        car[b + RS_YY] = dsum(car[b + RS_YY], y0, y0);       car[b + RS_YY] = dsum(car[b + RS_YY], y1, y1);
+        car[b + RS_UY] = dsum(car[b + RS_UY], u.x, y0);      car[b + RS_UY] = dsum(car[b + RS_UY], u.y, y1);
+        car[b + RS_YGT] = dsum(car[b + RS_YGT], y0, gt.x);    car[b + RS_YGT] = dsum(car[b + RS_YGT], y1, gt.y);
+        const int c = RS_PER_POINT * (NACT + j) + RS_YY;
+        const d2 hg = ObjCurv<Obj>::apply2(gt, p);
+        acc[c] = dsum(acc[c], gt.x, hg.x); acc[c] = dsum(acc[c], gt.y, hg.y);
+    }
+}
+
+template <class Obj, int NACT, int NCARRY>
+__device__ inline void cg_carry_single(const RParams &P, const RDeep &Q, const RDeepLds &L, const RCarry &C, long long i, double (&acc)[RW<MAXP>::W],
+                                       double (&car)[RW<NCARRY>::W]) {
+    double x = P.x[i];
+    double u = P.u[i];
+    const PS<Obj> p = ps_load<Obj>(P, i);
+    replay_single<Obj>(P, Q, L, x, u, p);
+    x = x + P.a_acc * u;
+    double g = 0.0, f0 = 0.0;
+    obj_eval1<Obj>(x, p, P.s0, f0, g);
+    u = -g + P.beta * u;
+#pragma unroll
+    for (int j = 0; j < NCARRY; ++j) {
+        const int b = RS_PER_POINT * j;
+        const double xp = x + C.a[j] * u;
+        double gt;
+        obj_term1<Obj, false>(xp, p, P.s0, car[b + RS_F], gt);
+        const double y = gt - g;
+        car[b + RS_GTU] = dsum(car[b + RS_GTU], gt, u); car[b + RS_GTGT] = dsum(car[b + RS_GTGT], gt, gt);
+        car[b + RS_GTG] = dsum(car[b + RS_GTG], gt, g);
+        car[b + RS_YY] = dsum(car[b + RS_YY], y, y);
+        car[b + RS_UY] = dsum(car[b + RS_UY], u, y);
+        car[b + RS_YGT] = dsum(car[b + RS_YGT], y, gt);
+        const int c = RS_PER_POINT * (NACT + j) + RS_YY;
+        acc[c] = dsum(acc[c], gt, ObjCurv<Obj>::apply1(gt, p));
+    }
+}
+
+template <class Obj, int MODE, int NACT, bool BIG, int NCARRY>
+__global__ __launch_bounds__(BLOCK) void k_cg_path(const RParams P, const RDeep Q, const RCarry C) {
+    static_assert(BIG, "path launches exist as pure-HBM streams only");
+    static_assert(path_mode(MODE), "a path row is launch N or S of the replay cycle in a lean form that leaves the y·y slot free");
+    static_assert(ObjCurv<Obj>::declared, "a carried point's curvature sum needs the constant Hessian");
+    static_assert(NCARRY >= 1 && NCARRY <= NCARRY_MAX && npts_for(NCARRY) == NCARRY, "a trial launch's point count");
+    static_assert(NACT >= 1 && NACT + NCARRY <= MAXP, "the carried curvature sums take the y·y slots of point blocks NACT … NACT + NCARRY − 1");
+    constexpr int W = RW<MAXP>::W, WC = RW<NCARRY>::W;
+    double acc[W], car[WC];
+#pragma unroll
+    for (int s = 0; s < W; ++s) acc[s] = 0.0;
+#pragma unroll
+    for (int s = 0; s < WC; ++s) car[s] = 0.0;
+    __shared__ RDeepLds L;
+    rdeep_stage(Q, L);
+    const long long n2 = P.n >> 1;
+    const long long per = big_chunk_pairs(n2, gridDim.x);
+    long long i = per * blockIdx.x + threadIdx.x;
+    const long long hi = (per * blockIdx.x + per < n2) ? per * blockIdx.x + per : n2;
+    const long long step = BLOCK;
+    for (; i + step < hi; i += 2 * step) {
+        d2 xa = ldg2<true>(P.x, i), xb = ldg2<true>(P.x, i + step);
+        d2 ua = ldg2<true>(P.u, i), ub = ldg2<true>(P.u, i + step);
+        const PV<Obj> pa = pv_load<Obj, true>(P, i), pb = pv_load<Obj, true>(P, i + step);
+        bool wxa = false, wua = false, wxb = false, wub = false;
+        cg_path_pair<Obj, MODE, NACT>(P, Q, L, xa, ua, pa, acc, wxa, wua);
+        cg_carry_points2<Obj, NACT, NCARRY>(P, C, xa, ua, pa, acc, car);
+        cg_path_pair<Obj, MODE, NACT>(P, Q, L, xb, ub, pb, acc, wxb, wub);
+        cg_carry_points2<Obj, NACT, NCARRY>(P, C, xb, ub, pb, acc, car);
+        if (wxa) stg2<true>(P.xo, i, xa);
+        if (wua) stg2<true>(P.uo, i, ua);
+        if (wxb) stg2<true>(P.xo, i + step, xb);
+        if (wub) stg2<true>(P.uo, i + step, ub);
+    }
+    if (i < hi) {
+        d2 xa = ldg2<true>(P.x, i);
+        d2 ua = ldg2<true>(P.u, i);
+        const PV<Obj> pa = pv_load<Obj, true>(P, i);
+        bool wxa = false, wua = false;
+        cg_path_pair<Obj, MODE, NACT>(P, Q, L, xa, ua, pa, acc, wxa, wua);
+        cg_carry_points2<Obj, NACT, NCARRY>(P, C, xa, ua, pa, acc, car);
+        if (wxa) stg2<true>(P.xo, i, xa);
+        if (wua) stg2<true>(P.uo, i, ua);
+    }
+    if ((P.n & 1) && blockIdx.x == 0 && threadIdx.x == 0) {
+        cg_carry_single<Obj, NACT, NCARRY>(P, Q, L, C, P.n - 1, acc, car);
+        cg_path_single<Obj, MODE, NACT>(P, Q, L, P.n - 1, acc);
+    }
+    if constexpr (LateF<Obj, MODE>::on) {
+#pragma unroll
+        for (int j = 0; j < NACT; ++j) acc[RS_PER_POINT * j + RS_F] *= ObjFScale<Obj>::scale;
+    }
+    store_partials_n<W, false>(acc, P.partials, P.tail);
+    const double own = wg_reduce_n<WC>(car);
+    if (threadIdx.x < WC) C.partials[(size_t)blockIdx.x * WC + threadIdx.x] = own;
+}
+
+}
+}
diff --git a/conjugategradientoptim.jl_amd/csrc/cgo_path.hpp b/conjugategradientoptim.jl_amd/csrc/cgo_path.hpp
--- a/conjugategradientoptim.jl_amd/csrc/cgo_path.hpp
+++ b/conjugategradientoptim.jl_amd/csrc/cgo_path.hpp
@@ -22,15 +22,40 @@
     }
 };
 
-CGO_HD inline int ls_predicted_path(const cgo_ls_config &ls, double f, double dphi0, double c, double a_initial, double (&pts)[7]) {
+struct PathModelEvalHints {
+    PathModelEval m;
+    double h[CTL_MAXP][4];
+    CGO_HD int operator()(double step, double &phi, double &dphi, double h1, double h2, double h3, double h4) {
+        const int before = m.n;
+        const int rc = m(step, phi, dphi, h1, h2, h3, h4);
+        if (m.n > before)
+            for (int j = 0; j < CTL_MAXP; ++j) if (j == before) { h[j][0] = h1; h[j][1] = h2; h[j][2] = h3; h[j][3] = h4; }
+        return rc;
+    }
+};
+
+CGO_HD inline int ls_trial_request(double a, const double *hs, int nh, int mp, double (&pts)[7]) {
     for (int j = 0; j < 7; ++j) pts[j] = 0.0;
-    if (!(hd_isfinite(f) && hd_isfinite(dphi0) && hd_isfinite(c))) return 0;
-    if (!(c > 0.0) || !(dphi0 < 0.0)) return 0;
-    if (ls.kind != CGO_LS_STRONG_WOLFE_BISECTION && ls.kind != CGO_LS_WOLFE_BISECTION) return 0;
-    if (ls.kind == CGO_LS_WOLFE_BISECTION && ls.cond_kind != CGO_COND_WOLFE) return 0;
-    PathModelEval ev;
-    ev.f = f; ev.d0 = dphi0; ev.c = c; ev.n = 0; ev.over = false;
-    for (int j = 0; j < CTL_MAXP; ++j) ev.a[j] = 0.0;
+    pts[0] = a;
+    int k = 1;
+    for (int q = 0; q < nh && k < mp && k < 7; ++q) {
+        const double h = hs[q];
+        bool ok = hd_isfinite(h) && h > 0.0;
+        for (int j = 0; ok && j < k; ++j) ok = (h != pts[j]);
+        if (ok) pts[k++] = h;
+    }
+    return k;
+}
+
+CGO_HD inline bool ls_path_predictable(const cgo_ls_config &ls, double f, double dphi0, double c) {
+    if (!(hd_isfinite(f) && hd_isfinite(dphi0) && hd_isfinite(c))) return false;
+    if (!(c > 0.0) || !(dphi0 < 0.0)) return false;
+    if (ls.kind != CGO_LS_STRONG_WOLFE_BISECTION && ls.kind != CGO_LS_WOLFE_BISECTION) return false;
+    if (ls.kind == CGO_LS_WOLFE_BISECTION && ls.cond_kind != CGO_COND_WOLFE) return false;
+    return true;
+}
+template <class Ev>
+CGO_HD inline void ls_path_run(const cgo_ls_config &ls, double f, double dphi0, double a_initial, Ev &ev) {
     LSOut o = ls_out(0.0, 0.0, 0, CGO_INCOMPLETE);
     if (ls.kind == CGO_LS_STRONG_WOLFE_BISECTION) {
         (void)ls_strong_wolfe_t(ls, f, dphi0, a_initial, ev, o);
@@ -39,9 +64,39 @@
         double uu = 0.0;
         (void)ls_wolfe_bisection_t(ls, f, dphi0, uu, a_initial, ev, bk, o);
     }
+}
+
+CGO_HD inline int ls_predicted_path(const cgo_ls_config &ls, double f, double dphi0, double c, double a_initial, double (&pts)[7]) {
+    for (int j = 0; j < 7; ++j) pts[j] = 0.0;
+    if (!ls_path_predictable(ls, f, dphi0, c)) return 0;
+    PathModelEval ev;
+    ev.f = f; ev.d0 = dphi0; ev.c = c; ev.n = 0; ev.over = false;
+    for (int j = 0; j < CTL_MAXP; ++j) ev.a[j] = 0.0;
+    ls_path_run(ls, f, dphi0, a_initial, ev);
     for (int j = 0; j < 7; ++j) pts[j] = ev.a[j];
     for (int j = 0; j < 7; ++j) if (j < ev.n && !(hd_isfinite(pts[j]) && pts[j] > 0.0)) return 0;
     return ev.n;
 }
 
+CGO_HD inline int ls_predicted_path_hints(const cgo_ls_config &ls, double f, double dphi0, double c, double a_initial, double (&pts)[7],
+                                          double (&hints)[7][4]) {
+    for (int j = 0; j < 7; ++j) { pts[j] = 0.0; for (int q = 0; q < 4; ++q) hints[j][q] = 0.0; }
+    if (!ls_path_predictable(ls, f, dphi0, c)) return 0;
+    PathModelEvalHints ev;
+    ev.m.f = f; ev.m.d0 = dphi0; ev.m.c = c; ev.m.n = 0; ev.m.over = false;
+    for (int j = 0; j < CTL_MAXP; ++j) { ev.m.a[j] = 0.0; for (int q = 0; q < 4; ++q) ev.h[j][q] = 0.0; }
+    ls_path_run(ls, f, dphi0, a_initial, ev);
+    for (int j = 0; j < 7; ++j) { pts[j] = ev.m.a[j]; for (int q = 0; q < 4; ++q) hints[j][q] = ev.h[j][q]; }
+    for (int j = 0; j < 7; ++j) if (j < ev.m.n && !(hd_isfinite(pts[j]) && pts[j] > 0.0)) return 0;
+    return ev.m.n;
 }
+
+CGO_HD inline int ls_predicted_carry(const double (&pts)[7], const double (&hints)[7][4], int npath, int held, int mp, double (&cp)[7]) {
+    for (int j = 0; j < 7; ++j) cp[j] = 0.0;
+    if (held < 1 || held >= npath || held >= 7) return 0;
+    double a = 0.0, hs[4] = {0.0, 0.0, 0.0, 0.0};
+    for (int j = 0; j < 7; ++j) if (j == held) { a = pts[j]; for (int q = 0; q < 4; ++q) hs[q] = hints[j][q]; }
+    return ls_trial_request(a, hs, 4, mp, cp);
+}
+
+}
diff --git a/include/cgo.h b/include/cgo.h
--- a/include/cgo.h
+++ b/include/cgo.h
@@ -376,6 +376,10 @@
 int cgo_solver_path_stats(cgo_solver *s, int64_t *by_nact, int64_t *predicted, int64_t *tree, int64_t *misses);
 int cgo_solver_probe_set_path(cgo_solver *s, int32_t nact);
 int cgo_solver_debug_set_path_skew(cgo_solver *s, double factor);
+int cgo_solver_set_path_carry(cgo_solver *s, int32_t on);
+int cgo_solver_path_carry_stats(cgo_solver *s, int64_t *launches, int64_t *served, int64_t *unused);
+int cgo_solver_probe_set_carry(cgo_solver *s, int32_t kc, const double *a);
+int cgo_solver_probe_carried(cgo_solver *s, const double *a, int32_t k, double *row, int32_t cap, int32_t *len);
 int32_t cgo_stop_status(int64_t it, int64_t max_iters, double f_x, double grad_norm, double eps, double f_x0, int64_t *iters_ran);
 
 int cgo_kernel_dir(cgo_ctx *ctx, double *u, const double *g, double beta, int64_t n,
```

New measurement: 2324. -1.4%, worse.
